# trungnt13/sisua

Hardware: AMD Instinct MI355X
Metric: cells/sec VAE training (pbmc8k_ly, batch=128) (higher is better)
Workload: dtype f32

## Files before the change

include/sisua_hip.h:

```cpp
#ifndef SISUA_HIP_H_
#define SISUA_HIP_H_

#include <stdint.h>

#ifdef __cplusplus
extern "C" {
#endif

#define SMX_ABI_VERSION 18
#define SMX_MAX_LAYERS 8
#define SMX_MAX_LABELS 4

typedef enum {
  SMX_OK = 0,
  SMX_ERR_INVALID = -1,
  SMX_ERR_HIP = -2,
  SMX_ERR_NOMEM = -3,
  SMX_ERR_COMM = -4,
  SMX_ERR_NAN = -5
} smx_status;

typedef enum { SMX_MODEL_VAE = 0, SMX_MODEL_DCA = 1, SMX_MODEL_SCVI = 2, SMX_MODEL_SISUA = 3, SMX_MODEL_SCALE = 4,
               SMX_MODEL_FVAE = 5,
               SMX_MODEL_SCALE_TRIL = 6 ,
// ... 116 lines not shown
                        float* l_samples, float* x_params, float* const* y_params);

int smx_predict(smx_model* m, const float* host_x, const float* host_library, int64_t n_cells, int32_t batch,
                int32_t n_samples, float* z_mean, float* z_scale, float* z_samples, float* l_mean, float* l_scale,
                float* l_samples, float* x_params, float* const* y_params);

int smx_predict_stat(smx_model* m, const float* host_x, const float* host_library, int64_t n_cells, int32_t batch, int32_t n_samples,
                     int32_t stat, int32_t count_only, const float* target, float* out);

int smx_predict_csr(smx_model* m, const int64_t* indptr, const int32_t* cols, const float* vals, const float* host_library,
                    int64_t n_cells, int32_t batch, int32_t n_samples, float* z_mean, float* z_scale, float* z_samples,
                    float* l_mean, float* l_scale, float* l_samples, float* x_params, float* const* y_params);
int smx_predict_stat_csr(smx_model* m, const int64_t* indptr, const int32_t* cols, const float* vals, const float* host_library,
                         int64_t n_cells, int32_t batch, int32_t n_samples, int32_t stat, int32_t count_only, const float* target,
                         const int64_t* t_indptr, const int32_t* t_cols, const float* t_vals, float* out);

int smx_predict_sample(smx_model* m, const float* host_x, const float* host_library, int64_t n_cells, int32_t batch, int32_t n_samples,
                       int32_t count_only, uint64_t seed, int32_t n_k, float* out);
int smx_predict_sample_csr(smx_model* m, const int64_t* indptr, const int32_t* cols, const float* vals, const float* host_library,
                           int64_t n_cells, int32_t batch, int32_t n_samples, int32_t count_only, uint64_t seed, int32_t n_k, float* out);

int smx_predict_stat_cols(smx_model* m, const float* host_x, const float* host_library, int64_t n_cells, int32_t batch, int32_t n_samples,
                          int32_t count_only, const int32_t* genes, int32_t n_sel, float* out);
int smx_predict_stat_cols_csr(smx_model* m, const int64_t* indptr, const int32_t* cols, const float* vals, const float* host_library,
                              int64_t n_cells, int32_t batch, int32_t n_samples, int32_t count_only, const int32_t* genes, int32_t n_sel,
                              float* out);

int smx_predict_impute(smx_model* m, const float* host_x, const float* host_library, int64_t n_cells, int32_t batch, int32_t n_samples,
                       int32_t count_only, const float* original, float* cell_median, int32_t* cell_changed, float* global_lohi);
int smx_predict_impute_csr(smx_model* m, const float* host_x, const int64_t* indptr, const int32_t* cols, const float* vals,
                           const float* host_library, int64_t n_cells, int32_t batch, int32_t n_samples, int32_t count_only,
                           const float* original, const int64_t* o_indptr, const int32_t* o_cols, const float* o_vals, float* cell_median,
                           int32_t* cell_changed, float* global_lohi);

int smx_predict_correlate(smx_model* m, const float* host_x, const float* host_library, int64_t n_cells, int32_t batch, int32_t n_samples,
                          int32_t count_only, const int32_t* genes, int32_t n_sel, const int32_t* prot_rank2, const double* prot_unit, int32_t P,
                          int64_t* sp_Sa, int64_t* sp_Saa, int64_t* sp_Sab, double* pe_mean, double* pe_Sxx, double* pe_Sxy, int32_t* nonfinite);
int smx_predict_correlate_csr(smx_model* m, const int64_t* indptr, const int32_t* cols, const float* vals, const float* host_library,
                              int64_t n_cells, int32_t batch, int32_t n_samples, int32_t count_only, const int32_t* genes, int32_t n_sel,
                              const int32_t* prot_rank2, const double* prot_unit, int32_t P, int64_t* sp_Sa, int64_t* sp_Saa, int64_t* sp_Sab,
                              double* pe_mean, double* pe_Sxx, double* pe_Sxy, int32_t* nonfinite);

int smx_decode(smx_model* m, const float* z, const float* l, int32_t batch, float* x_params, float* const* y_params);

int smx_marginal_llk(smx_model* m, const int32_t* row_ids, const float* host_x, const float* host_library, int32_t batch,
                     int32_t n_samples, float* mllk, float* llk_mean);
int smx_marginal_llk_csr(smx_model* m, const int64_t* indptr, const int32_t* cols, const float* vals, const float* host_library,
                         int32_t batch, int32_t n_samples, float* mllk, float* llk_mean);

int smx_score_llk(smx_model* m, const int32_t* row_ids, const float* host_x, const float* host_library,
                  const float* const* targets, int32_t n_targets, int32_t batch, int32_t n_samples, float* out);

int smx_set_noise(smx_model* m, int32_t stream, const float* data, int32_t batch, int32_t width);
int smx_clear_noise(smx_model* m);

int smx_comm_unique_id(uint8_t id[128]);
int smx_comm_init(smx_model* m, int rank, int world, const uint8_t id[128]);
int smx_comm_world(const smx_model* m);
int smx_comm_rank(const smx_model* m);
int smx_comm_form(const smx_model* m);
int smx_comm_set_form(smx_model* m, int form);
int smx_opt_gather(smx_model* m);
int smx_comm_p2p_export(smx_model* m, int world, uint8_t handles[128]);
int smx_comm_p2p_init(smx_model* m, int rank, int world, const uint8_t* all_handles);
int smx_comm_p2p_error(smx_model* m, int32_t* error);
int smx_comm_time_allreduce(smx_model* m, int iters, float* us_per_call, int64_t* floats);
int smx_comm_library(char* rccl_path, int rccl_cap, char* hip_path, int hip_cap, int32_t* rccl_version);
int smx_comm_set_sync_bn(smx_model* m, int on);
int smx_comm_init_local(smx_model* const* models, int n);

int smx_shuffle_order(int32_t n_obs, int32_t buffer, const int64_t* picks, int32_t* out);

int smx_set_tuning(const char* name, double value);
int smx_clear_tuning(const char* name);

int smx_set_flag(smx_model* m, const char* name, int value);

int smx_timing_enable(smx_model* m, const char* kernel);
int smx_timing_read(smx_model* m, double* total_ms, int64_t* launches);
int64_t smx_loss_bytes_per_cell(const smx_model* m);
int64_t smx_head_fused_bytes(const smx_model* m, int32_t batch);
int32_t smx_head_dw_late(const smx_model* m);
int32_t smx_lazy_adam_steps(const smx_model* m);

int smx_k_count_llk(int likelihood, int direct, const float* x, const float* planes, int32_t B, int32_t G,
                    float* llk, float* grads);
int smx_k_adam(int32_t n_tensors, const int32_t* sizes, float* params, const float* grads, float* m, float* v,
               int32_t step, float lr, float beta1, float beta2, float eps, float clipnorm, float* norms);
int smx_k_opt(int32_t rule, const float* hp, int32_t n_hp, int32_t n_tensors, const int32_t* sizes, float* params, const float* grads,
              float* m, float* v, int32_t step, float lr, float clipnorm, float* norms);
typedef enum { SMX_CARRIER_LAUNCH = 0, SMX_CARRIER_SWEEP = 1, SMX_CARRIER_SHARD = 2, SMX_CARRIER_BODY512 = 3 } smx_opt_carrier;
int smx_k_opt_carrier(const int32_t* ip, const float* fp, const float* hp, int32_t n_hp, const int32_t* sizes, const float* params,
                      const float* grads, const float* m, const float* v, const int32_t* sq_first, const int32_t* sq_count, const float* sq_slots,
                      float* params_out, float* m_out, float* v_out, float* norms, float* lr_t, int32_t* guards_ok, int32_t* unused_ok);
int smx_k_gemm(int transA, int transB, const float* A, const float* B, int32_t M, int32_t N, int32_t K,
               int32_t split_k, int32_t tile_cfg, float* C);
int smx_k_head_fused(int likelihood, int u16, const float* x, const float* d, const float* W, const float* bias, int32_t B, int32_t G,
                     float grad_scale, int32_t reps, float* llk, float* dW, float* db, float* dd, float* sumsq, float* us);
int smx_k_head_fused_stress(int likelihood, int u16, const float* x, const float* d, const float* W, const float* bias, int32_t B, int32_t G,
                            float grad_scale, int32_t launches, int32_t* n_differ, int64_t* first_word);
int smx_k_hiprand(uint64_t seed, int32_t n, const uint32_t* counters, uint32_t* ours, uint32_t* hiprand_words);
int smx_k_noise(uint64_t seed, int32_t stream, int32_t step, int32_t sample, const int64_t* cell_ids, int32_t B,
                int32_t width, float dropout_p, float* dropout_mult, float* normal);
int smx_k_bn_fwd(const int32_t* ip, const float* fp, const float* pre, const float* gamma, const float* beta, const float* bias,
                 const float* moving_mean, const float* moving_var, const float* mask, const int32_t* rows, uint64_t seed, float* out,
                 float* xhat, float* inv_std, float* batch_mean, float* batch_var, float* moving_mean_out, float* moving_var_out,
                 int32_t* guards_ok);
int smx_k_bn_bwd(const int32_t* ip, const float* fp, const float* dout, const float* out, const float* xhat, const float* inv_std,
                 const float* gamma, const float* beta, const float* mask, const int32_t* rows, uint64_t seed, float* dpre, float* dgamma,
                 float* dbeta, float* dbias, int32_t* guards_ok);
int smx_k_scvi_head_train(const int32_t* ip, const float* fp, const float* raw, const void* x, const float* hl, const float* Wl, const float* bl,
                          const float* library, const int32_t* rows, const float* eps_in, uint64_t seed, float* draw, float* llk_part, float* l,
                          float* sig, float* eps, float* kl, float* latl, float* dlatl, float* dl, int32_t* guards_ok);
int smx_k_scvi_head_fwd(const int32_t* ip, const float* fp, const float* raw, const float* l, float* planes, float* rho_raw, int32_t* guards_ok);
int smx_k_scvi_head_bwd(const int32_t* ip, const float* fp, const float* planes, const float* dplanes, const float* rho_raw, const float* l,
                        float* draw, float* dl, int32_t* guards_ok);
int smx_k_plane_sample(int likelihood, int direct, int count_only, const float* planes, int32_t rows, int32_t G, uint64_t seed,
                       int32_t n_k, float* out);
int smx_k_row_select(const float* rows, int32_t n_rows, int32_t G, int32_t ld, float* lo, float* hi);
int smx_k_col_rank2(const float* cols, int32_t n_cols, int64_t n_cells, int32_t* rank2, int32_t* nonfinite);
int smx_k_col_correlate(const float* cols, int32_t n_cols, int64_t n_cells, const int32_t* prot_rank2, const double* prot_unit, int32_t P,
                        int64_t* sp_Sa, int64_t* sp_Saa, int64_t* sp_Sab, double* pe_mean, double* pe_Sxx, double* pe_Sxy, int32_t* nonfinite);

int smx_cluster_silhouette(const float* Z, int64_t n_cells, int32_t D, const int32_t* labels, int32_t n_labels, double* a, double* b);
int smx_cluster_kmeans(const float* Z, int64_t n_cells, int32_t D, int32_t K, const int32_t* init_idx, int32_t n_init, int32_t max_iter,
                       int32_t* labels_best, double* centres_best, double* inertia, int32_t* n_iter, int32_t* best, int32_t* labels_all);

int smx_gmm1d_fit(const float* X, int64_t n_cells, int32_t C, int32_t K, const float* init_raw, int32_t R, int32_t max_iter, double tol,
                  double reg_covar, int32_t remove_zeros, int32_t log_norm, double* lower_bound, int32_t* n_iter, int32_t* converged,
                  int32_t* best, double* weights, double* means, double* variances, int64_t* n_train, double* col_sum, double* params_all,
                  double* stats);
int smx_gmm1d_predict(const float* X, int64_t n_cells, int32_t C, int32_t K, const double* weights, const double* means, const double* variances,
                      const int32_t* order, int32_t positive_component, const double* threshold, int32_t log_norm, double* prob, float* bin,
                      double* score);

int smx_gmm_full_fit(const float* Z, int64_t n_cells, int32_t D, int32_t K, const int32_t* init_labels, int32_t R, int32_t max_iter, double tol,
                     double reg_covar, double* lower_bound, int32_t* n_iter, int32_t* converged, int32_t* status, int32_t* best,
                     double* weights, double* means, double* covariances, double* chol_inv, int32_t* labels, double* params_all);
int smx_gmm_full_predict(const float* Z, int64_t n_cells, int32_t D, int32_t K, const double* weights, const double* means, const double* chol_inv,
                         int32_t* labels, double* resp, double* score);

int smx_prep_stats(const float* x, const int64_t* indptr, const int32_t* cols, const float* vals, int64_t n_cells, int32_t n_genes,
                   int32_t block_rows, int32_t func, const float* row_div, const uint8_t* col_mask, const float* row_thresh,
                   double* cell_total, int32_t* cell_n_genes, double* gene_sum, double* gene_sumsq, int64_t* gene_n_cells,
                   int64_t* gene_n_above);
int smx_prep_apply(const float* x, const int64_t* indptr, const int32_t* cols, const float* vals, int64_t n_cells, int32_t n_genes,
                   int32_t block_rows, int32_t func, const float* row_div, const float* mean, const float* sd, int32_t clip,
                   float max_value, float* out_dense, float* out_vals);

int smx_pca_cov(const float* x, const int64_t* indptr, const int32_t* cols, const float* vals, int64_t n_cells, int32_t n_genes,
                int32_t block_rows, double* mean, double* cov);
int smx_pca_project(const float* x, const int64_t* indptr, const int32_t* cols, const float* vals, int64_t n_cells, int32_t n_genes,
                    int32_t block_rows, const double* mean, const double* components, int32_t n_components, float* out);

int smx_knn(const float* Z, int64_t n_cells, int32_t D, int32_t k, int32_t* idx, double* dist);
int smx_knn_umap(const int32_t* idx, const double* dist, int64_t n_cells, int32_t K, double* rho, double* sigma, double* weight);

int smx_tsne_affinities(const int32_t* idx, const double* dist, int64_t n_cells, int32_t k, double perplexity, double* cond_p, double* beta);
int smx_tsne_gradient(const int64_t* indptr, const int32_t* cols, const double* p, int64_t n_cells, int32_t n_components, const double* Y,
                      double exaggeration, double* grad, double* kl, double* Z);
int smx_tsne_fit(const int64_t* indptr, const int32_t* cols, const double* p, int64_t n_cells, int32_t n_components, const double* Y0,
                 int32_t max_iter, double early_exaggeration, double learning_rate, double min_grad_norm, int32_t n_iter_without_progress,
                 double* Y, double* kl_trace, int32_t* n_iter, double* update_out, double* gains_out);

int smx_mutual_info(const double* xcols, const uint8_t* x_discrete, const double* ycols, const uint8_t* y_discrete, int64_t n_cells,
                    int32_t n_genes, int32_t n_proteins, int32_t n_neighbors, int32_t gene_chunk, const double* psi, const double* logn,
// ... 43 lines not shown
```

sisua_amd/_hip.py:

```python
from __future__ import annotations

import ctypes as C
import os

_HERE = os.path.dirname(os.path.abspath(__file__))
LIB_PATH = os.path.join(_HERE, "libsisua_hip.so")

SMX_ABI_VERSION = 18
SMX_MAX_LAYERS = 8
SMX_MAX_LABELS = 4

MODEL_KINDS = {"vae": 0, "dca": 1, "scvi": 2, "sisua": 3, "scale": 4, "fvae": 5, "scale_tril": 6, "scale_post": 7}
LIKELIHOODS = {"nb": 0, "zinb": 1, "nbd": 2, "zinbd": 3, "mse": 4, "bernoulli": 5, "normal": 6}
LABEL_LIKELIHOODS = {"nb": 0, "onehot": 1, "mixnb": 2, "mixgauss": 3, "mixtril": 4, "mixzinb": 5, "nbd": 6, "zinb": 7, "zinbd": 8,
                     "bernoulli": 9, "normal": 10}
SCVI_PLANE_OPTIONS = {"full": 0, "share": 1, "single": 2}
ACTIVATIONS = {"relu": 0, "linear": 1}
SMX_ACT_RELU, SMX_ACT_LINEAR, SMX_ACT_LEAKY_RELU, SMX_ACT_ELU, SMX_ACT_SELU, SMX_ACT_TANH, SMX_ACT_SIGMOID, SMX_ACT_SOFTPLUS = range(8)
HIDDEN_ACTIVATIONS = {"relu": SMX_ACT_RELU, "linear": SMX_ACT_LINEAR, "leaky_relu": SMX_ACT_LEAKY_RELU, "elu": SMX_ACT_ELU,
                      "selu": SMX_ACT_SELU, "tanh": SMX_ACT_TANH, "sigmoid": SMX_ACT_SIGMOID, "softplus": SMX_ACT_SOFTPLUS}
SMX_NET_ENCODER, SMX_NET_DECODER, SMX_NET_LIBRARY_ENCODER = range(3)


class SmxError(RuntimeError):
# ... 53 lines not shown
    "smx_set_bn": (C.c_int, [_VP, C.c_int, C.c_int, _FP]),
    "smx_get_step": (C.c_int, [_VP, _IP]),
    "smx_set_step": (C.c_int, [_VP, C.c_int32]),
    "smx_dataset_upload": (C.c_int, [_VP, _FP, C.c_int64, C.POINTER(_FP), _FP, C.POINTER(C.c_uint8), C.c_int64]),
    "smx_dataset_upload_u16": (C.c_int, [_VP, C.POINTER(C.c_uint16), C.c_int64, C.POINTER(_FP), _FP, C.POINTER(C.c_uint8), C.c_int64]),
    "smx_dataset_upload_csr": (C.c_int, [_VP, C.POINTER(C.c_int64), C.POINTER(C.c_int32), _FP, C.c_int64, C.POINTER(_FP), _FP,
                                         C.POINTER(C.c_uint8), C.c_int64]),
    "smx_dataset_upload_csr_dense": (C.c_int, [_VP, _LP, _IP, _FP, C.c_int64, C.POINTER(_FP), _FP, C.POINTER(C.c_uint8), C.c_int64,
                                               C.c_int32]),
    "smx_dataset_size": (C.c_int64, [_VP]),
    "smx_dataset_generate_lognormal": (C.c_int, [_VP, C.c_uint64, C.c_int32, C.c_int64, C.c_int32, C.c_double]),
    "smx_train_step": (C.c_int, [_VP, _IP, C.c_int32, C.POINTER(smx_metrics)]),
    "smx_train_step_graph": (C.c_int, [_VP, _IP, C.c_int32, C.POINTER(smx_metrics)]),
    "smx_train_steps": (C.c_int, [_VP, _IP, C.c_int32, C.c_int32, C.c_int, C.POINTER(smx_metrics)]),
    "smx_train_stage": (C.c_int, [_VP, _IP, C.c_int32, C.c_int32]),
    "smx_metrics_history": (C.c_int, [_VP, C.c_int32, _FP]),
    "smx_eval_step": (C.c_int, [_VP, _IP, C.c_int32, C.POINTER(smx_metrics)]),
    "smx_set_train_draws": (C.c_int, [_VP, C.c_int32]),
    "smx_set_optimizer": (C.c_int, [_VP, C.c_int32, _FP, C.c_int32]),
    "smx_set_schedule": (C.c_int, [_VP, C.c_int32, C.c_int32, C.POINTER(C.c_double), C.c_int32]),
    "smx_get_schedule": (C.c_int, [_VP, C.c_int32, _IP, C.POINTER(C.c_double), C.c_int32, _IP]),
    "smx_schedule_eval": (C.c_int, [C.c_int32, C.POINTER(C.c_double), C.c_int32, C.c_int64, C.c_int32, _FP]),
    "smx_get_optimizer": (C.c_int, [_VP, _IP, _FP, _IP]),
    "smx_set_activation": (C.c_int, [_VP, C.c_int32, C.c_int32]),
    "smx_forward": (C.c_int, [_VP, _IP, _FP, _FP, C.c_int32, C.c_int32, C.c_int32, _FP, _FP, _FP, _FP, _FP, _FP, _FP,
                              C.POINTER(_FP)]),
    "smx_forward_samples": (C.c_int, [_VP, _IP, _FP, _FP, C.c_int32, C.c_int32, _FP, _FP, _FP, _FP, _FP, _FP, _FP,
                                      C.POINTER(_FP)]),
    "smx_shuffle_order": (C.c_int, [C.c_int32, C.c_int32, C.POINTER(C.c_int64), C.POINTER(C.c_int32)]),
    "smx_predict": (C.c_int, [_VP, _FP, _FP, C.c_int64, C.c_int32, C.c_int32, _FP, _FP, _FP, _FP, _FP, _FP, _FP,
                              C.POINTER(_FP)]),
    "smx_predict_stat": (C.c_int, [_VP, _FP, _FP, C.c_int64, C.c_int32, C.c_int32, C.c_int32, C.c_int32, _FP, _FP]),
    "smx_predict_csr": (C.c_int, [_VP, _LP, _IP, _FP, _FP, C.c_int64, C.c_int32, C.c_int32, _FP, _FP, _FP, _FP, _FP, _FP, _FP,
                                  C.POINTER(_FP)]),
    "smx_predict_stat_csr": (C.c_int, [_VP, _LP, _IP, _FP, _FP, C.c_int64, C.c_int32, C.c_int32, C.c_int32, C.c_int32, _FP,
                                       _LP, _IP, _FP, _FP]),
    "smx_predict_sample": (C.c_int, [_VP, _FP, _FP, C.c_int64, C.c_int32, C.c_int32, C.c_int32, C.c_uint64, C.c_int32, _FP]),
    "smx_predict_sample_csr": (C.c_int, [_VP, _LP, _IP, _FP, _FP, C.c_int64, C.c_int32, C.c_int32, C.c_int32, C.c_uint64, C.c_int32, _FP]),
    "smx_predict_stat_cols": (C.c_int, [_VP, _FP, _FP, C.c_int64, C.c_int32, C.c_int32, C.c_int32, _IP, C.c_int32, _FP]),
    "smx_predict_stat_cols_csr": (C.c_int, [_VP, _LP, _IP, _FP, _FP, C.c_int64, C.c_int32, C.c_int32, C.c_int32, _IP, C.c_int32, _FP]),
    "smx_predict_impute": (C.c_int, [_VP, _FP, _FP, C.c_int64, C.c_int32, C.c_int32, C.c_int32, _FP, _FP, _IP, _FP]),
    "smx_predict_impute_csr": (C.c_int, [_VP, _FP, _LP, _IP, _FP, _FP, C.c_int64, C.c_int32, C.c_int32, C.c_int32, _FP, _LP, _IP, _FP,
                                         _FP, _IP, _FP]),
    "smx_predict_correlate": (C.c_int, [_VP, _FP, _FP, C.c_int64, C.c_int32, C.c_int32, C.c_int32, _IP, C.c_int32, _IP, _DP, C.c_int32,
                                        _LP, _LP, _LP, _DP, _DP, _DP, _IP]),
    "smx_predict_correlate_csr": (C.c_int, [_VP, _LP, _IP, _FP, _FP, C.c_int64, C.c_int32, C.c_int32, C.c_int32, _IP, C.c_int32, _IP, _DP,
                                            C.c_int32, _LP, _LP, _LP, _DP, _DP, _DP, _IP]),
    "smx_decode": (C.c_int, [_VP, _FP, _FP, C.c_int32, _FP, C.POINTER(_FP)]),
    "smx_dataset_library": (C.c_int, [_VP, _FP]),
    "smx_dataset_corrupt": (C.c_int, [_VP, C.c_double, C.c_double, C.c_uint64, C.POINTER(C.c_int64)]),
    "smx_dataset_read": (C.c_int, [_VP, C.c_int64, C.c_int64, _FP, _FP, _FP]),
    "smx_marginal_llk": (C.c_int, [_VP, _IP, _FP, _FP, C.c_int32, C.c_int32, _FP, _FP]),
    "smx_marginal_llk_csr": (C.c_int, [_VP, _LP, _IP, _FP, _FP, C.c_int32, C.c_int32, _FP, _FP]),
    "smx_score_llk": (C.c_int, [_VP, _IP, _FP, _FP, C.POINTER(_FP), C.c_int32, C.c_int32, C.c_int32, _FP]),
    "smx_set_noise": (C.c_int, [_VP, C.c_int32, _FP, C.c_int32, C.c_int32]),
    "smx_clear_noise": (C.c_int, [_VP]),
    "smx_comm_unique_id": (C.c_int, [C.POINTER(C.c_uint8)]),
    "smx_comm_init": (C.c_int, [_VP, C.c_int, C.c_int, C.POINTER(C.c_uint8)]),
    "smx_comm_p2p_export": (C.c_int, [_VP, C.c_int, C.POINTER(C.c_uint8)]),
    "smx_comm_p2p_init": (C.c_int, [_VP, C.c_int, C.c_int, C.POINTER(C.c_uint8)]),
    "smx_comm_p2p_error": (C.c_int, [_VP, C.POINTER(C.c_int32)]),
    "smx_comm_time_allreduce": (C.c_int, [_VP, C.c_int, C.POINTER(C.c_float), C.POINTER(C.c_int64)]),
    "smx_comm_world": (C.c_int, [_VP]),
    "smx_comm_rank": (C.c_int, [_VP]),
    "smx_comm_form": (C.c_int, [_VP]),
    "smx_comm_set_form": (C.c_int, [_VP, C.c_int]),
    "smx_opt_gather": (C.c_int, [_VP]),
    "smx_comm_library": (C.c_int, [C.c_char_p, C.c_int, C.c_char_p, C.c_int, _IP]),
    "smx_comm_set_sync_bn": (C.c_int, [_VP, C.c_int]),
    "smx_comm_init_local": (C.c_int, [C.POINTER(_VP), C.c_int]),
    "smx_k_adam": (C.c_int, [C.c_int32, _IP, _FP, _FP, _FP, _FP, C.c_int32, C.c_float, C.c_float, C.c_float, C.c_float,
                             C.c_float, _FP]),
    "smx_k_opt": (C.c_int, [C.c_int32, _FP, C.c_int32, C.c_int32, _IP, _FP, _FP, _FP, _FP, C.c_int32, C.c_float, C.c_float, _FP]),
    "smx_k_opt_carrier": (C.c_int, [_IP, _FP, _FP, C.c_int32, _IP, _FP, _FP, _FP, _FP, _IP, _IP, _FP, _FP, _FP, _FP, _FP, _FP, _IP, _IP]),
    "smx_set_flag": (C.c_int, [_VP, C.c_char_p, C.c_int]),
    "smx_set_tuning": (C.c_int, [C.c_char_p, C.c_double]),
    "smx_clear_tuning": (C.c_int, [C.c_char_p]),
    "smx_timing_enable": (C.c_int, [_VP, C.c_char_p]),
    "smx_timing_read": (C.c_int, [_VP, C.POINTER(C.c_double), C.POINTER(C.c_int64)]),
    "smx_loss_bytes_per_cell": (C.c_int64, [_VP]),
    "smx_head_fused_bytes": (C.c_int64, [_VP, C.c_int32]),
    "smx_head_dw_late": (C.c_int32, [_VP]),
    "smx_lazy_adam_steps": (C.c_int32, [_VP]),
    "smx_k_count_llk": (C.c_int, [C.c_int, C.c_int, _FP, _FP, C.c_int32, C.c_int32, _FP, _FP]),
    "smx_k_head_fused": (C.c_int, [C.c_int, C.c_int, _FP, _FP, _FP, _FP, C.c_int32, C.c_int32, C.c_float, C.c_int32, _FP, _FP, _FP, _FP, _FP,
                                   _FP]),
    "smx_k_head_fused_stress": (C.c_int, [C.c_int, C.c_int, _FP, _FP, _FP, _FP, C.c_int32, C.c_int32, C.c_float, C.c_int32, C.POINTER(C.c_int32),
                                          C.POINTER(C.c_int64)]),
    "smx_k_gemm": (C.c_int, [C.c_int, C.c_int, _FP, _FP, C.c_int32, C.c_int32, C.c_int32, C.c_int32, C.c_int32, _FP]),
    "smx_k_hiprand": (C.c_int, [C.c_uint64, C.c_int32, C.POINTER(C.c_uint32), C.POINTER(C.c_uint32), C.POINTER(C.c_uint32)]),
    "smx_k_noise": (C.c_int, [C.c_uint64, C.c_int32, C.c_int32, C.c_int32, C.POINTER(C.c_int64), C.c_int32, C.c_int32,
                              C.c_float, _FP, _FP]),
    "smx_k_bn_fwd": (C.c_int, [_IP, _FP, _FP, _FP, _FP, _FP, _FP, _FP, _FP, _IP, C.c_uint64, _FP, _FP, _FP, _FP, _FP, _FP, _FP, _IP]),
    "smx_k_bn_bwd": (C.c_int, [_IP, _FP, _FP, _FP, _FP, _FP, _FP, _FP, _FP, _IP, C.c_uint64, _FP, _FP, _FP, _FP, _IP]),
    "smx_k_scvi_head_train": (C.c_int, [_IP, _FP, _FP, _VP, _FP, _FP, _FP, _FP, _IP, _FP, C.c_uint64, _FP, _FP, _FP, _FP, _FP, _FP, _FP, _FP, _FP, _IP]),
    "smx_k_scvi_head_fwd": (C.c_int, [_IP, _FP, _FP, _FP, _FP, _FP, _IP]),
    "smx_k_scvi_head_bwd": (C.c_int, [_IP, _FP, _FP, _FP, _FP, _FP, _FP, _FP, _IP]),
    "smx_k_plane_sample": (C.c_int, [C.c_int, C.c_int, C.c_int, _FP, C.c_int32, C.c_int32, C.c_uint64, C.c_int32, _FP]),
    "smx_k_row_select": (C.c_int, [_FP, C.c_int32, C.c_int32, C.c_int32, _FP, _FP]),
    "smx_k_col_rank2": (C.c_int, [_FP, C.c_int32, C.c_int64, _IP, _IP]),
    "smx_k_col_correlate": (C.c_int, [_FP, C.c_int32, C.c_int64, _IP, _DP, C.c_int32, _LP, _LP, _LP, _DP, _DP, _DP, _IP]),
    "smx_cluster_silhouette": (C.c_int, [_FP, C.c_int64, C.c_int32, _IP, C.c_int32, _DP, _DP]),
    "smx_cluster_kmeans": (C.c_int, [_FP, C.c_int64, C.c_int32, C.c_int32, _IP, C.c_int32, C.c_int32, _IP, _DP, _DP, _IP, _IP, _IP]),
    "smx_gmm1d_fit": (C.c_int, [_FP, C.c_int64, C.c_int32, C.c_int32, _FP, C.c_int32, C.c_int32, C.c_double, C.c_double, C.c_int32, C.c_int32, _DP, _IP,
                            _IP, _IP, _DP, _DP, _DP, _LP, _DP, _DP, _DP]),
    "smx_gmm1d_predict": (C.c_int, [_FP, C.c_int64, C.c_int32, C.c_int32, _DP, _DP, _DP, _IP, C.c_int32, _DP, C.c_int32, _DP, _FP, _DP]),
    "smx_gmm_full_fit": (C.c_int, [_FP, C.c_int64, C.c_int32, C.c_int32, _IP, C.c_int32, C.c_int32, C.c_double, C.c_double, _DP, _IP, _IP, _IP, _IP,
                               _DP, _DP, _DP, _DP, _IP, _DP]),
    "smx_gmm_full_predict": (C.c_int, [_FP, C.c_int64, C.c_int32, C.c_int32, _DP, _DP, _DP, _IP, _DP, _DP]),
    "smx_prep_stats": (C.c_int, [_FP, _LP, _IP, _FP, C.c_int64, C.c_int32, C.c_int32, C.c_int32, _FP, C.POINTER(C.c_uint8), _FP, _DP, _IP, _DP, _DP,
                                 _LP, _LP]),
    "smx_prep_apply": (C.c_int, [_FP, _LP, _IP, _FP, C.c_int64, C.c_int32, C.c_int32, C.c_int32, _FP, _FP, _FP, C.c_int32, C.c_float, _FP, _FP]),
    "smx_pca_cov": (C.c_int, [_FP, _LP, _IP, _FP, C.c_int64, C.c_int32, C.c_int32, _DP, _DP]),
    "smx_pca_project": (C.c_int, [_FP, _LP, _IP, _FP, C.c_int64, C.c_int32, C.c_int32, _DP, _DP, C.c_int32, _FP]),
    "smx_knn": (C.c_int, [_FP, C.c_int64, C.c_int32, C.c_int32, _IP, _DP]),
    "smx_knn_umap": (C.c_int, [_IP, _DP, C.c_int64, C.c_int32, _DP, _DP, _DP]),
    "smx_tsne_affinities": (C.c_int, [_IP, _DP, C.c_int64, C.c_int32, C.c_double, _DP, _DP]),
    "smx_tsne_gradient": (C.c_int, [_LP, _IP, _DP, C.c_int64, C.c_int32, _DP, C.c_double, _DP, _DP, _DP]),
    "smx_tsne_fit": (C.c_int, [_LP, _IP, _DP, C.c_int64, C.c_int32, _DP, C.c_int32, C.c_double, C.c_double, C.c_double, C.c_int32, _DP, _DP, _IP,
                               _DP, _DP]),
    "smx_mutual_info": (C.c_int, [_DP, C.POINTER(C.c_uint8), _DP, C.POINTER(C.c_uint8), C.c_int64, C.c_int32, C.c_int32, C.c_int32, C.c_int32, _DP,
                                  _DP, _DP]),
    "smx_k_mi_cells": (C.c_int, [_DP, C.c_int32, _DP, C.c_int32, C.c_int64, C.c_int32, _DP, _DP, _IP, _DP, _DP]),
    "smx_group_moments": (C.c_int, [_FP, _LP, _IP, _FP, C.c_int64, C.c_int32, C.c_int32, _IP, C.c_int32, _LP, _DP, _DP, _LP]),
    "smx_group_ranksums": (C.c_int, [_FP, C.c_int32, C.c_int64, _IP, C.c_int32, C.c_int32, _LP, _LP]),
    "smx_mbkmeans_seed": (C.c_int, [_FP, _LP, _IP, _FP, C.c_int64, C.c_int32, C.c_int32, C.c_int32, C.c_int64, _DP, _IP, _DP, _DP]),
    "smx_mbkmeans_step": (C.c_int, [_FP, _LP, _IP, _FP, C.c_int64, C.c_int32, C.c_int32, _DP, _DP, _IP, _DP]),
    "smx_mbkmeans_predict": (C.c_int, [_FP, _LP, _IP, _FP, C.c_int64, C.c_int32, C.c_int32, C.c_int32, _DP, _IP, _DP]),
    "smx_louvain": (C.c_int, [_LP, _IP, _DP, C.c_int64, C.c_double, C.c_double, C.c_int32, C.c_int32, _IP, _IP, _IP, _DP, _LP, _IP, _IP]),
    "smx_louvain_modularity": (C.c_int, [_LP, _IP, _DP, C.c_int64, _IP, C.c_double, _DP]),
    "smx_louvain_table_degree": (C.c_int32, []),
    "smx_logreg_eval": (C.c_int, [_FP, _LP, _IP, _FP, C.c_int64, C.c_int32, _IP, C.c_int32, C.c_int32, C.c_double, C.c_int32, _DP, _DP, _DP, _DP,
                                  _DP]),
    "smx_logreg_fit": (C.c_int, [_FP, _LP, _IP, _FP, C.c_int64, C.c_int32, _IP, C.c_int32, C.c_int32, C.c_double, C.c_int32, C.c_double, C.c_int32,
                                 _DP, _DP, _DP, _DP, _DP, _DP, _IP, _IP, _IP]),
    "smx_logreg_decision": (C.c_int, [_FP, _LP, _IP, _FP, C.c_int64, C.c_int32, C.c_int32, C.c_int32, C.c_int32, _DP, _DP, _DP]),
    "smx_pad_audit": (C.c_int, [_VP, C.c_int32, _LP, _IP, _LP, C.c_char_p, C.c_int32]),
    "smx_pad_poke": (C.c_int, [_VP, C.c_int32, C.c_int32, C.c_float]),
}

_lib = None


def load():
  global _lib
  if _lib is not None:
    return _lib
  if not os.path.exists(LIB_PATH):
    raise SmxError(f"{LIB_PATH} is missing: build it with `python -m sisua_amd.build` "
                   "(hipcc --offload-arch=gfx950). sisua_amd has no CPU fallback.")
  try:
    lib = C.CDLL(LIB_PATH, mode=C.RTLD_GLOBAL)
  except OSError as e:
    raise SmxError(f"cannot load {LIB_PATH}: {e}") from e
  for name, (res, args) in SIGNATURES.items():
    try:
      fn = getattr(lib, name)
    except AttributeError as e:
      raise SmxError(f"{LIB_PATH} does not export {name}") from e
    fn.restype = res
    fn.argtypes = args
  if lib.smx_abi_version() != SMX_ABI_VERSION:
    raise SmxError("libsisua_hip.so ABI version mismatch; rebuild")
  if int(os.environ.get("WORLD_SIZE", "1")) > 1:
    for cand in ("/opt/rocm/lib/librccl.so.1", "/opt/rocm/lib/librccl.so"):
      if os.path.exists(cand):
# ... 33 lines not shown
```

sisua_amd/build.py:

```python
import os
import subprocess
import sys
from concurrent.futures import ThreadPoolExecutor

HERE = os.path.dirname(os.path.abspath(__file__))
CSRC = os.path.join(HERE, "csrc")
LIB = os.path.join(HERE, "libsisua_hip.so")
SOURCES = ["smx_gemm.hip", "smx_dgemm.hip", "smx_bn.hip", "smx_latent.hip", "smx_adam.hip", "smx_loss.hip", "smx_data.hip", "smx_headloss.hip", "smx_headbwd.hip", "smx_headfused.hip", "smx_bigk.hip", "smx_factor.hip", "smx_scvi.hip", "smx_score.hip", "smx_model.hip", "smx_dataset.hip", "smx_comm.hip", "smx_p2p.hip", "smx_forward.hip", "smx_backward.hip", "smx_step.hip", "smx_predict.hip", "smx_sample.hip", "smx_impute.hip", "smx_correlate.hip", "smx_cluster.hip", "smx_gmm.hip", "smx_gmm_full.hip", "smx_prep.hip", "smx_pca.hip", "smx_knn.hip", "smx_tsne.hip", "smx_mi.hip", "smx_rankgroups.hip", "smx_mbkmeans.hip", "smx_louvain.hip", "smx_logreg.hip", "smx_scoring.hip", "smx_schedule.hip", "smx_kapi.hip"]
HEADERS = ["smx_device.h", "smx_act.h", "smx_internal.h", "smx_loss.h", "smx_model.h", "smx_panel.h", "smx_dgemm.h", "smx_adam.h", "smx_headdw.h", "smx_dist.h", "smx_block.h", "smx_prep.h", os.path.join("..", "..", "include", "sisua_hip.h")]
FLAGS = ["--offload-arch=gfx950", "-O3", "-std=c++17", "-fPIC", "-fno-slp-vectorize", "-Wall", "-Wno-unused-function", "-Wno-unused-value", "-Wno-unused-result"]


def _hipcc():
  for c in (os.environ.get("HIPCC"), "/opt/rocm/bin/hipcc", "hipcc"):
    if c and (os.path.isabs(c) and os.path.exists(c) or not os.path.isabs(c)):
      return c
  raise RuntimeError("hipcc not found")


def _stale(target, deps):
  if not os.path.exists(target):
    return True
  t = os.path.getmtime(target)
  return any(os.path.getmtime(d) > t for d in deps)


def build(force: bool = False, verbose: bool = True) -> str:
  hipcc = _hipcc()
  hdrs = [os.path.normpath(os.path.join(CSRC, h)) for h in HEADERS]
  stamp, flags = os.path.join(CSRC, ".flags"), " ".join(FLAGS)
  if not os.path.exists(stamp) or open(stamp).read() != flags:
    force = True
  objs, jobs = [], []
  for s in SOURCES:
    src = os.path.join(CSRC, s)
    obj = os.path.join(CSRC, s.replace(".hip", ".o"))
    objs.append(obj)
    if force or _stale(obj, [src] + hdrs):
      jobs.append([hipcc] + FLAGS + ["-c", src, "-o", obj])

  def run(cmd):
    if verbose:
      print(" ".join(cmd), flush=True)
    r = subprocess.run(cmd, capture_output=True, text=True)
    if r.returncode != 0:
      raise RuntimeError("build failed:\n" + " ".join(cmd) + "\n" + r.stdout + r.stderr)
    return r.stderr

  with ThreadPoolExecutor(max_workers=7) as ex:
    for err in ex.map(run, jobs):
      if verbose and err.strip():
        print(err)
  with open(stamp, "w") as f:
    f.write(flags)
  if force or jobs or _stale(LIB, objs):
    isa_lint(objs)
    run([hipcc, "--offload-arch=gfx950", "-shared", "-fPIC", "-o", LIB] + objs + ["-ldl"])
  return LIB


def isa_lint(objs):
  tools = os.path.join(os.path.dirname(HERE), "tools")
  if not os.path.exists(os.path.join(tools, "isa_lint.py")) or os.environ.get("SMX_NO_ISA_LINT"):
    return
  sys.path.insert(0, tools)
  try:
    import isa_lint as lint
  finally:
    sys.path.pop(0)
  found = lint.lint_files(objs)
  if found:
    raise RuntimeError("isa_lint: the build contains instruction forms that are wrong on gfx950 (tools/isa_lint.py):\n" +
                       "\n".join("  %s %s: %s" % f for f in found[:20]))


if __name__ == "__main__":
  print(build(force="--force" in sys.argv))
```

sisua_amd/csrc/smx_backward.hip:

```cpp
#include "smx_model.h"

namespace smx {

static void fill_rider_adam(smx_model* m, AdamArgs& a) {
  fill_adam_args(m, a);
  a.use_sq = 1;
  for (size_t t = 0; t < m->tensors.size(); ++t) {
    a.sq_first[t] = m->sq_first[t]; a.sq_count[t] = m->sq_count[t];
    if (m->sq_reduced[t]) { a.sq_first[t] = m->sq_total_first + (int)t * SMX_SQR_PER_TENSOR; a.sq_count[t] = m->sq_reduced[t]; }
  }
  a.master = nullptr; a.with_metrics = 0;
}

static void take_adam_riders(smx_model* m, GemmArgs& h, AdamArgs& store) {
  const int n = std::min(m->adam_ride_b, m->adam_rest_to - m->adam_rest_from);
  m->adam_ride_b = 0;
  if (n <= 0) return;
  fill_rider_adam(m, store);
  h.ride_adam = &store; h.ride_first = m->adam_rest_from; h.ride_count = n;
  if (m->adam_early_from < 0) m->adam_early_from = m->adam_rest_from;
  m->adam_rest_from += n;
  m->adam_early_to = m->adam_rest_from;
}

// ... 77 lines not shown
    if (m->sq_count[t] == 0 && m->tensors[t].count > SMX_SQ_SMALL_TENSOR) return false;
  return true;
}
int head_sweep_prepare(smx_model* m) {
  const int mode = (dp_active(m) || tuning_on("event_system_fence")) ? 1 : 0;
  if (m->st_side && m->ev_mode == mode) return SMX_OK;
  if (!m->st_side) {
    int lo = 0, hi = 0;
    SMX_HIP(hipDeviceGetStreamPriorityRange(&lo, &hi));
    SMX_HIP(hipStreamCreateWithPriority(&m->st_side, hipStreamNonBlocking, lo));
  }
  if (m->ev_sweep) { hipEventDestroy(m->ev_sweep); m->ev_sweep = nullptr; }
  if (m->ev_hf) { hipEventDestroy(m->ev_hf); m->ev_hf = nullptr; }
  const unsigned fl = hipEventDisableTiming | (mode ? 0u : (unsigned)hipEventDisableSystemFence);
  SMX_HIP(hipEventCreateWithFlags(&m->ev_sweep, fl));
  SMX_HIP(hipEventCreateWithFlags(&m->ev_hf, fl));
  m->ev_mode = mode;
  return SMX_OK;
}
static int head_sweep_start(smx_model* m) {
  AdamArgs a;
  fill_rider_adam(m, a);
  static const bool skip = tuning_on("skip_head_adam");
  if (!skip) {
    SMX_HIP(hipStreamWaitEvent(m->st_side, m->ev_hf, 0));
    SMX_CHECK(launch_adam_sweep(m->st_side, a, m->chunk_first_head, head_sweep_end(m) - m->chunk_first_head, head_sweep_wgs(m)));
    SMX_HIP(hipEventRecord(m->ev_sweep, m->st_side));
    m->sweep_pending = true;
  }
  m->adam_early_from = m->chunk_first_head; m->adam_early_to = head_sweep_end(m);
  m->adam_early_pending = false; m->adam_rest_from = m->adam_rest_to = 0; m->adam_ride_b = 0;
  return SMX_OK;
}

int dp_chain_start(smx_model* m) {
  if (m->chain_started) return SMX_OK;
  SMX_CHECK(head_sweep_prepare(m));
  SMX_HIP(hipEventRecord(m->ev_hf, m->st));
  SMX_HIP(hipStreamWaitEvent(m->st_comm, m->ev_hf, 0));
  AdamArgs a;
  fill_adam_args(m, a);
  a.use_sq = 0; a.master = nullptr; a.with_metrics = 0;
  const int first = m->chunk_first_head, count = m->n_chunks - m->chunk_first_head;
  const int forced = (int)tuning("adam_sweep_wgs", 0);
  const int wgs = forced > 0 ? forced : std::min(std::max(count / SMX_HEAD_SWEEP_CHUNKS_PER_WG, 64), 256);
  if (m->flags.opt_shard && (m->world > 1 || m->dp_force) && dp_shard_available(m)) {
    const size_t slice = (((size_t)m->bucket1_count + m->world - 1) / m->world + 63) / 64 * 64;
    SMX_REQUIRE((size_t)m->world * slice <= (size_t)m->bucket1_count + SMX_SHARD_SLACK, "opt_shard: too many ranks for the buffers' slack");
    SMX_CHECK(dp_reduce_scatter(m, m->grads + m->bucket1_off, slice, m->st_comm, true));
    a.partial = m->shard_partial;
    a.shard_lo = (long)(m->bucket1_off + (size_t)m->rank * slice);
    a.shard_hi = (long)std::min(m->bucket1_off + ((size_t)m->rank + 1) * slice, m->bucket1_off + (size_t)m->bucket1_count);
    SMX_CHECK(launch_grad_sqsum_shard(m->st_comm, a, first, count));
    SMX_CHECK(dp_allreduce_buf(m, m->shard_partial + first, (size_t)count, m->st_comm, true));
    SMX_CHECK(launch_head_norms(m->st_comm, a, first, count));
    if (a.shard_hi > a.shard_lo) SMX_CHECK(launch_adam_shard(m->st_comm, a, first, count, wgs));
    SMX_CHECK(dp_all_gather(m, m->params + m->bucket1_off, slice, m->st_comm, true));
    m->opt_stale = true;
  } else {
    SMX_CHECK(dp_allreduce(m, m->bucket1_off, m->bucket1_count, m->st_comm, true));
    SMX_CHECK(launch_grad_sqsum_range(m->st_comm, a, first, count));
    SMX_CHECK(launch_adam_sweep(m->st_comm, a, first, count, wgs));
  }
  SMX_HIP(hipEventRecord(m->ev_sweep, m->st_comm));
  m->sweep_pending = true;
  m->chain_started = true;
  m->adam_early_from = m->chunk_first_head; m->adam_early_to = m->n_chunks;
  m->adam_rest_from = m->adam_rest_to = 0; m->adam_ride_b = 0;
  return SMX_OK;
}

struct MlpBwdOpts {
  bool skip_input_grad = false;
  int* out_slabs = nullptr;
  const char* label = "";
  const EpiLatentBwd* lat_epi = nullptr;
  GemmArgs* defer_dw0 = nullptr;
  const BnBwdArgs* front = nullptr;
  std::vector<GemmArgs>* defer = nullptr;
  std::vector<MlpLayer>* twin = nullptr; const BnBwdArgs* twin_front = nullptr; bool* twin_done = nullptr;
  bool last_bn_done = false;
  const HeadBwdArgs* head_dw = nullptr;
};
static int mlp_backward(smx_model* m, std::vector<MlpLayer>& mlp, const Pass& ps, Mat in0, bool in_is_x, int n_slabs, const MlpBwdOpts& o) {
  auto make_b = [&](MlpLayer& L, int slabs, const BnBwdArgs* front) {
    BnBwdArgs b;
    b.dout = m->slab; b.n_slabs = slabs; b.slab_stride = (long)ps.B * L.out_p; b.ld = L.out_p;
    b.out = L.out_buf; b.xhat = L.xhat; b.inv_std = L.inv_std;
    b.B = ps.B; b.H = L.out; b.Hp = L.out_p; b.batchnorm = L.bn >= 0; b.training = ps.training; b.leak = L.leak;
    b.drop_scale = (ps.training && L.drop_p > 0.f) ? 1.f / (1.f - L.drop_p) : 1.f;
    b.dpre = L.dpre;
    if (L.bn >= 0) { b.gamma = P_(m, L.tGamma); b.dgamma = G_(m, L.tGamma); b.dbeta = G_(m, L.tBeta); }
    else b.dbias = G_(m, L.tBias);
    if (L.act != SMX_ACT_RELU) {
      b.act = L.act;
      if (L.bn >= 0) b.beta = P_(m, L.tBeta);
      b.drop_p = ps.training ? L.drop_p : 0.f;
      b.nk = make_key(m, L.stream, ps.sample, true);
      if (&mlp == &m->dec) b.nk.draw_rows = (uint32_t)ps.draw_rows;
      b.rows = ps.rows; b.cell_base = ps.cell_base;
      if (const Injected* ij = inj(m, L.stream)) { b.inj_mask = ij->d; b.inj_ld = ij->ld; }
    }
    if (front) {
      b.front = 1; b.fD = front->fD; b.fld = front->fld; b.fW = front->fW; b.fldw = front->fldw; b.fK = front->fK;
      b.fold_dz = front->fold_dz; b.zD = front->zD; b.zld = front->zld; b.zW = front->zW; b.zldw = front->zldw; b.zlb = front->zlb;
    }
    if (&mlp == &m->dec && &L == &mlp.back() && m->wide_dd_slabs > 0 && !front) {
      b.dout = m->wide_dd_src; b.n_slabs = m->wide_dd_slabs; b.slab_stride = m->wide_dd_stride; b.wide = 1;
    }
    return b;
  };
  if (o.twin_done) *o.twin_done = false;
  BnBwdArgs carried;
  bool have_carried = false;
  bool dw_carried = false;
  bool dpre_done = false;
  for (int i = (int)mlp.size() - 1; i >= 0; --i) {
    MlpLayer& L = mlp[i];
    const TensorInfo& tw = m->tensors[L.tW];
    const bool last = (i == (int)mlp.size() - 1);
    BnBwdArgs b = make_b(L, n_slabs, (o.front && last) ? o.front : (have_carried ? &carried : nullptr));
    have_carried = false;
    const bool dpre_ready = dpre_done;
    dpre_done = false;
    if ((last && o.last_bn_done) || dpre_ready) {
    } else if (sync_bn_on(m, ps.training) && L.bn >= 0) {
      Timed t(m, "bn_bwd");
      m->adam_early_pending = false;
      const BnSyncArgs y = sync_args(m);
      SMX_CHECK(launch_bn_sync_bwd(m->st, b, y, 0));
      SMX_CHECK(dp_allreduce_buf(m, m->sync_buf, (size_t)y.world * 2 * L.out_p, m->st));
      SMX_CHECK(launch_bn_sync_bwd(m->st, b, y, 1));
    } else {
      if (m->metrics_before_allreduce && m->have_pending_metrics) {
        b.metrics = m->pending_metrics; b.with_metrics = 1; m->have_pending_metrics = false;
      }
      const HeadBwdArgs* hd = (last && o.head_dw && bn_wide_bwd_dw_supported(b, *o.head_dw)) ? o.head_dw : nullptr;
      if (!hd) attach_early_adam(m, b);
      const bool w_rides = hd && b.adam_count == 0 && b.sqr_count == 0 && m->lazy_w_pending && !m->lazy_rest_pending;
      if (w_rides) { b.adam = m->lazy_args; b.adam_first = m->lazy_w_first; b.adam_count = m->lazy_w_n; }
      if (m->lazy_want && m->lazy_l1 && !m->lazy_closed && &mlp == &m->enc && m->have_pending_metrics) {
        b.metrics = m->pending_metrics; b.with_metrics = 1; m->have_pending_metrics = false;
        if (!b.adam.params) fill_adam_args(m, b.adam);
        fill_step_close(m, b.adam);
        b.close = 1; m->lazy_closed = true;
      }
      Timed t(m, "bn_bwd");
      const bool dual = last && b.front && b.fK <= 64 && o.twin && o.twin_front && o.twin_front->fK <= 64 && !o.twin->empty() && m->flags.twin && bn_dual_supported(ps.B) &&
                        bn_bwd_front_supported(ps.B, o.twin_front->fK) && o.twin->back().out_p % 8 == 0 &&
                        !(sync_bn_on(m, ps.training) && o.twin->back().bn >= 0);
      if (hd) {
        SMX_CHECK(launch_bn_wide_bwd_dw(m->st, b, *hd));
        dw_carried = true;
        if (w_rides) m->lazy_w_pending = false;
      } else if (dual) {
        const BnBwdArgs b2 = make_b(o.twin->back(), 0, o.twin_front);
        SMX_CHECK(launch_bn_act_bwd_dual(m->st, b, b2));
        if (o.twin_done) *o.twin_done = true;
      } else {
        SMX_CHECK(launch_bn_act_bwd(m->st, b));
      }
    }
    const bool first_x = (i == 0 && in_is_x);
    const Mat in = (i == 0) ? in0 : Mat{mlp[i - 1].out_buf, mlp[i - 1].out_p};
    GemmArgs g = dense_wgrad(m, in, {L.dpre, L.out_p}, L.tW, dpre_ready ? G_(m, L.tBias) : nullptr, L.in_p, L.out_p, ps.B);
    if (first_x) x_gather(m, ps, g);
    if (i == 0 && o.skip_input_grad) {
      if (o.defer_dw0) *o.defer_dw0 = g;
      else {
        Timed t(m, first_x ? o.label : "gemm_mlp_dw");
        SMX_CHECK(launch_gemm(m->st, g));
      }
      n_slabs = 0;
      break;
    }
    if (o.defer && i > 0 && !(i == 0 && o.lat_epi) && m->flags.bwd_front && (L.out_p == 32 || L.out_p == 64 || L.out_p == 128) && mlp[i - 1].act == SMX_ACT_RELU &&
        bn_bwd_front_supported(ps.B, L.out_p) && mlp[i - 1].out_p % 8 == 0 && (tw.ld % 4) == 0 && (L.out_p % 4) == 0 &&
        !(sync_bn_on(m, ps.training) && mlp[i - 1].bn >= 0)) {
      o.defer->push_back(g);
      carried = BnBwdArgs();
      carried.fD = L.dpre; carried.fld = L.out_p; carried.fW = P_(m, L.tW); carried.fldw = tw.ld; carried.fK = L.out_p;
      have_carried = true;
      n_slabs = 0;
      continue;
    }
    GemmArgs h = dense_dgrad({L.dpre, L.out_p}, {P_(m, L.tW), tw.ld}, m->slab, ps.B, L.in_p, L.out_p);
    h.split_k = suggest_split_k(ps.B, L.in_p, L.out_p);
    SMX_REQUIRE((size_t)h.split_k * (size_t)h.slab_stride <= m->slab_cap, "split-K slabs exceed the slab buffer");
    if (i == 0 && o.lat_epi) {
      h.epi = 2; h.lb = *o.lat_epi; h.split_k = 1; h.tile = TILE_32x32_K4;
    }
    if (i > 0 && m->flags.act_epilogue && mlp[i - 1].bn < 0 && !(ps.training && mlp[i - 1].drop_p > 0.f) && h.split_k <= 1 &&
        mlp[i - 1].act == SMX_ACT_RELU) {
      MlpLayer& Lo = mlp[i - 1];
      h.split_k = 1; h.act = 2; h.leak = Lo.leak; h.act_out = Lo.out_buf; h.act_ld = Lo.out_p;
      h.C = Lo.dpre; h.ldc = Lo.out_p; h.slab_stride = 0;
      dpre_done = true;
    }
    int effs[2] = {1, 1};
    if (o.defer && i == 0 && o.lat_epi && m->fold_dz_now) {
      o.defer->push_back(g);
    } else if (o.defer && i == 0 && o.lat_epi) {
      o.defer->push_back(g);
      AdamArgs riders;
      if (m->adam_ride_b > 0) take_adam_riders(m, h, riders);
      Timed t(m, "gemm_mlp_bwd");
      SMX_CHECK(launch_gemm_group(m->st, &h, 1, effs + 1));
    } else {
      GemmArgs pair[2] = {g, h};
      Timed t(m, "gemm_mlp_bwd");
      SMX_CHECK(launch_gemm_group(m->st, pair, 2, effs));
    }
    const int eff = effs[1];
    n_slabs = eff;
  }
  if (o.out_slabs) *o.out_slabs = n_slabs;
  SMX_REQUIRE(!o.head_dw || dw_carried, "the output head's dW found no launch to carry it");
  return SMX_OK;
}

static int disc_wgrad(smx_model* m, const GemmArgs& g, int rows, bool b3, const GemmArgs* beside = nullptr) {
  if (!(b3 && m->flags.wgrad && wgrad_supported(g, rows))) return launch_gemm(m->st, g);
  if (g.M >= 512 && g.N % 128 == 0 && g.N / 128 <= SMX_GROUP_MAX && g.N > 128 && !tuning_on("no_panel")) {
    GemmArgs part[SMX_GROUP_MAX];
    int counts[SMX_GROUP_MAX];
    const int ng = g.N / 128, per = ((g.M + 31) / 32) * 8;
    for (int k = 0; k < ng; ++k) {
      part[k] = g;
      part[k].B = g.B + 128 * k; part[k].C = g.C + 128 * k; part[k].N = 128; part[k].panel_hint = 1;
      if (g.colsum) part[k].colsum = g.colsum + 128 * k;
      if (g.sq_part) { part[k].sq_part = g.sq_part + (long)per * k; part[k].sq_count = &counts[k]; }
    }
    const int rc = launch_wgrad_group(m->st, part, ng, rows, 1, beside);
    if (rc == SMX_OK && g.sq_part && g.sq_count) *g.sq_count = per * ng;
    return rc;
  }
  return launch_wgrad_group(m->st, &g, 1, rows, 1, beside);
// ... 457 lines not shown
```

sisua_amd/csrc/smx_bn.hip:

```cpp
#include "smx_internal.h"
#include "smx_adam.h"

namespace smx {

SMX_STAMP_TABLE

}
#include "smx_headdw.h"
namespace smx {

#ifndef SMX_BN_COLS
#define SMX_BN_COLS 8
#endif
constexpr int BN_COLS = SMX_BN_COLS;
constexpr int BN_RL = 64;
constexpr int BN_RPT_DEFAULT = 2;
constexpr int BN_THREADS = BN_COLS * BN_RL;
constexpr int BN_WAVES = BN_THREADS / 64;

__device__ inline float bn_col_reduce(float v, float* sh ) {
  const int c = threadIdx.x % BN_COLS, w = threadIdx.x >> 6;
  static_assert(BN_COLS == 8, "bn_col_reduce: the lanes of a column are 8 apart");
  v += __int_as_float(__builtin_amdgcn_update_dpp(0, __float_as_int(v), 0x128, 0xF, 0xF, false));
  v = xor32_add(xor16_add(v));
  __syncthreads();
  if ((threadIdx.x & 63) < BN_COLS) sh[w * BN_COLS + c] = v;
  __syncthreads();
  float t = 0.f;
#pragma unroll
  for (int q = 0; q < BN_WAVES; q += 4)
    t += (sh[q * BN_COLS + c] + sh[(q + 1) * BN_COLS + c]) + (sh[(q + 2) * BN_COLS + c] + sh[(q + 3) * BN_COLS + c]);
  return t;
}

constexpr int SLAB_FLIGHT = 16;
template <int NR>
struct SlabBatch { float t[SLAB_FLIGHT][NR]; };
template <int NR>
__device__ inline void slab_issue(const float* base, int s0, int n_slabs, long slab_stride, int ld, int col, int r0, int rl, int B, SlabBatch<NR>& sb) {
#pragma unroll
  for (int q = 0; q < SLAB_FLIGHT; ++q) {
    const int s = min(s0 + q, n_slabs - 1);
#pragma unroll
    for (int i = 0; i < NR; ++i) {
      const int r = min(r0 + rl + BN_RL * i, B - 1);
      sb.t[q][i] = base[(long)s * slab_stride + (long)r * ld + col];
    }
  }
}
template <int NR>
__device__ inline void slab_accumulate(const SlabBatch<NR>& sb, int s0, int n_slabs, int r0, int rl, int B, float (&acc)[NR]) {
#pragma unroll
  for (int q = 0; q < SLAB_FLIGHT; ++q)
    if (s0 + q < n_slabs) {
#pragma unroll
      for (int i = 0; i < NR; ++i) acc[i] += (r0 + rl + BN_RL * i < B) ? sb.t[q][i] : 0.f;
    }
}
template <int BN_RPT>
__device__ inline void slab_sum(const float* base, int n_slabs, long slab_stride, int ld, int col, int r0, int rl,
                                int B, float (&acc)[BN_RPT]) {
#pragma unroll
  for (int i = 0; i < BN_RPT; ++i) acc[i] = 0.f;
  if (BN_RPT <= 2) {
    for (int s = 0; s < n_slabs; s += SLAB_FLIGHT) {
      SlabBatch<BN_RPT> sb;
      slab_issue<BN_RPT>(base, s, n_slabs, slab_stride, ld, col, r0, rl, B, sb);
      slab_accumulate<BN_RPT>(sb, s, n_slabs, r0, rl, B, acc);
    }
    return;
  }
  constexpr int SU = BN_RPT <= 4 ? 4 : 2;
  int s = 0;
  for (; s + SU <= n_slabs; s += SU) {
    float t[SU][BN_RPT];
#pragma unroll
    for (int q = 0; q < SU; ++q)
#pragma unroll
      for (int i = 0; i < BN_RPT; ++i) {
        const int r = r0 + rl + BN_RL * i;
        t[q][i] = r < B ? base[(long)(s + q) * slab_stride + (long)r * ld + col] : 0.f;
      }
#pragma unroll
    for (int q = 0; q < SU; ++q)
// ... 327 lines not shown

int launch_bn_act_fwd(hipStream_t st, const BnFwdArgs& a_in) {
  BnFwdArgs a = a_in;
  const bool gen = a.act != SMX_ACT_RELU;
  if (gen && (a.act < SMX_ACT_RELU || a.act > SMX_ACT_SOFTPLUS || a.front)) { set_error("bn_act_fwd: activations other than ReLU take no front"); return SMX_ERR_INVALID; }
  if (a.front) {
    if (!bn_front_supported(a.B, a.lat.Dp) || a.n_jobs || !a.W || (a.lat.ld % 4) || (a.lat.inj_eps && (a.lat.inj_ld % 4)) ||
        (a.lat.Dp > 32 && a.lat.Dp != 64 && a.lat.Dp != 128)) {
      set_error("bn_act_fwd: latent front not applicable");
      return SMX_ERR_INVALID;
    }
    if (a.Hp % BN_COLS) { set_error("bn_act_fwd: bad shapes"); return SMX_ERR_INVALID; }
    const size_t lds = ((size_t)a.B * (a.lat.Dp + 4) + (size_t)BN_COLS * (a.lat.Dp + 4)) * sizeof(float);
    static const bool big_ok = hipFuncSetAttribute(reinterpret_cast<const void*>(&bn_act_fwd_kernel<4, 1>),
                                                   hipFuncAttributeMaxDynamicSharedMemorySize, 96 * 1024) == hipSuccess;
    if (lds > 64 * 1024 && !big_ok) { set_error("bn_act_fwd: cannot reserve the dynamic LDS of the latent front"); return SMX_ERR_HIP; }
    if (a.lat.Dp == 128) {
      static const bool big2 = hipFuncSetAttribute(reinterpret_cast<const void*>(&bn_act_fwd_kernel<2, 2>),
                                                   hipFuncAttributeMaxDynamicSharedMemorySize, 96 * 1024) == hipSuccess;
      if (a.B > BN_RL * 2 || a.lat.stochastic || a.lat.relu || a.lat.z || (lds > 64 * 1024 && !big2)) {
        set_error("bn_act_fwd: 128-wide front not applicable");
        return SMX_ERR_INVALID;
      }
      hipLaunchKernelGGL((bn_act_fwd_kernel<2, 2>), dim3(a.Hp / BN_COLS), dim3(BN_THREADS), lds, st, a);
    } else if (a.B <= BN_RL * 2) hipLaunchKernelGGL((bn_act_fwd_kernel<2, 1>), dim3(a.Hp / BN_COLS + (a.lat.z ? 1 : 0)), dim3(BN_THREADS), lds, st, a);
    else hipLaunchKernelGGL((bn_act_fwd_kernel<4, 1>), dim3(a.Hp / BN_COLS + (a.lat.z ? 1 : 0)), dim3(BN_THREADS), lds, st, a);
    SMX_HIP(hipGetLastError());
    return SMX_OK;
  }
  if (a.Hp % BN_COLS || a.B <= 0) { set_error("bn_act_fwd: bad shapes"); return SMX_ERR_INVALID; }
  if (a.wide) {
    if (a.B > 128 || a.Hp > 128 || !a.pre || !a.xhat || a.slab_stride < (long)a.Hp * 128 || (a.slab_stride % 4)) { set_error("bn_act_fwd: wide slabs take at most 128 x 128"); return SMX_ERR_INVALID; }
    if (gen) hipLaunchKernelGGL(bn_wide_fwd_gen_kernel, dim3(a.Hp + a.n_jobs * SMX_NOISE_BLOCKS_PER_JOB), dim3(BN_THREADS), 0, st, a);
    else hipLaunchKernelGGL(bn_wide_fwd_kernel, dim3(a.Hp + a.n_jobs * SMX_NOISE_BLOCKS_PER_JOB), dim3(BN_THREADS), 0, st, a);
    SMX_HIP(hipGetLastError());
    return SMX_OK;
  }
  const int grid = a.Hp / BN_COLS + a.n_jobs * SMX_NOISE_BLOCKS_PER_JOB;
  if (gen) {
    if (a.B <= BN_RL * 2) hipLaunchKernelGGL(bn_act_fwd_gen_kernel<2>, dim3(grid), dim3(BN_THREADS), 0, st, a);
    else if (a.B <= BN_RL * 4) hipLaunchKernelGGL(bn_act_fwd_gen_kernel<4>, dim3(grid), dim3(BN_THREADS), 0, st, a);
    else if (a.B <= BN_RL * 8) hipLaunchKernelGGL(bn_act_fwd_gen_kernel<8>, dim3(grid), dim3(BN_THREADS), 0, st, a);
    else if (a.B <= BN_RL * 16) hipLaunchKernelGGL(bn_act_fwd_gen_kernel<16>, dim3(grid), dim3(BN_THREADS), 0, st, a);
    else hipLaunchKernelGGL(bn_act_fwd_gen_kernel<0>, dim3(grid), dim3(BN_THREADS), 0, st, a);
    SMX_HIP(hipGetLastError());
    return SMX_OK;
  }
  if (a.B <= BN_RL * 2) hipLaunchKernelGGL(bn_act_fwd_kernel<2>, dim3(grid), dim3(BN_THREADS), 0, st, a);
  else if (a.B <= BN_RL * 4) hipLaunchKernelGGL(bn_act_fwd_kernel<4>, dim3(grid), dim3(BN_THREADS), 0, st, a);
  else if (a.B <= BN_RL * 8) hipLaunchKernelGGL(bn_act_fwd_kernel<8>, dim3(grid), dim3(BN_THREADS), 0, st, a);
  else if (a.B <= BN_RL * 16) hipLaunchKernelGGL(bn_act_fwd_kernel<16>, dim3(grid), dim3(BN_THREADS), 0, st, a);
  else hipLaunchKernelGGL(bn_act_fwd_kernel<0>, dim3(grid), dim3(BN_THREADS), 0, st, a);
  SMX_HIP(hipGetLastError());
  return SMX_OK;
}

bool bn_dual_supported(int B) { return B > 0 && B <= BN_RL * 4; }
int launch_bn_act_fwd_dual(hipStream_t st, const BnFwdArgs& a, const BnFwdArgs& b) {
  if (a.front || b.front || b.n_jobs || a.B != b.B || !bn_dual_supported(a.B) || a.Hp % BN_COLS || b.Hp % BN_COLS || a.act != SMX_ACT_RELU ||
      b.act != SMX_ACT_RELU) {
    set_error("bn_act_fwd_dual: bad shapes (or an activation other than ReLU)");
    return SMX_ERR_INVALID;
  }
  const int na = a.Hp / BN_COLS + a.n_jobs * SMX_NOISE_BLOCKS_PER_JOB;
  const int grid = na + b.Hp / BN_COLS;
  if (a.B <= BN_RL * 2) hipLaunchKernelGGL(bn_act_fwd_dual_kernel<2>, dim3(grid), dim3(BN_THREADS), 0, st, a, b, na);
  else hipLaunchKernelGGL(bn_act_fwd_dual_kernel<4>, dim3(grid), dim3(BN_THREADS), 0, st, a, b, na);
  SMX_HIP(hipGetLastError());
  return SMX_OK;
}

typedef float bnf_f32x4 __attribute__((ext_vector_type(4)));
__device__ inline bnf_f32x4 bnf_mfma16x3(const Split8& a, const Split8& b, bnf_f32x4 acc) {
  acc = __builtin_amdgcn_mfma_f32_16x16x32_bf16(a.t2, b.t0, acc, 0, 0, 0);
  acc = __builtin_amdgcn_mfma_f32_16x16x32_bf16(a.t0, b.t2, acc, 0, 0, 0);
  acc = __builtin_amdgcn_mfma_f32_16x16x32_bf16(a.t1, b.t1, acc, 0, 0, 0);
  acc = __builtin_amdgcn_mfma_f32_16x16x32_bf16(a.t1, b.t0, acc, 0, 0, 0);
  acc = __builtin_amdgcn_mfma_f32_16x16x32_bf16(a.t0, b.t1, acc, 0, 0, 0);
  acc = __builtin_amdgcn_mfma_f32_16x16x32_bf16(a.t0, b.t0, acc, 0, 0, 0);
  return acc;
}
#define SMX_FOLD_WROW 136
#define SMX_FOLD_WIMG_BYTES (3 * 32 * SMX_FOLD_WROW * 2)
__device__ inline void fold_dz_tile(const BnBwdArgs& a, const int bid, float* tile, const int ldd, unsigned char* wimg) {
  const EpiLatentBwd& e = a.zlb;
  const int tid = threadIdx.x, lane = tid & 63, w = tid >> 6, li = lane & 15, kg = lane >> 4;
  float e_mu[2][4], e_sr[2][4], e_sg[2][4], e_ep[2][4];
  const float kls = kl_scale_of(e.klw);
#pragma unroll
  for (int nb = 0; nb < 2; ++nb)
#pragma unroll
    for (int r = 0; r < 4; ++r) {
      const long b = min(16 * w + 4 * kg + r, a.B - 1);
      const int d = 16 * nb + li;
      e_mu[nb][r] = e.lat[b * e.ld + d];
      e_sr[nb][r] = e.lat[b * e.ld + e.Dp + d];
      e_sg[nb][r] = e.sig[b * e.Dp + d];
      e_ep[nb][r] = e.eps[b * e.Dp + d];
    }
  {
    const int d = tid >> 4, k0 = (tid & 15) * 8;
    const float4 lo = *reinterpret_cast<const float4*>(a.zW + (long)d * a.zldw + k0), hi = *reinterpret_cast<const float4*>(a.zW + (long)d * a.zldw + k0 + 4);
    const float x[8] = {lo.x, lo.y, lo.z, lo.w, hi.x, hi.y, hi.z, hi.w};
    const Split8 sp = split3x8(x);
    smx_bf16x8* row = reinterpret_cast<smx_bf16x8*>(wimg + ((long)d * SMX_FOLD_WROW + k0) * 2);
    row[0] = sp.t0;
    row[(32 * SMX_FOLD_WROW * 2) / 16] = sp.t1;
    row[(2 * 32 * SMX_FOLD_WROW * 2) / 16] = sp.t2;
  }
  Split8 A[4];
  {
    const float* zr = a.zD + (long)min(16 * w + li, a.B - 1) * a.zld + 8 * kg;
    float4 v[8];
#pragma unroll
    for (int ks = 0; ks < 4; ++ks) { v[2 * ks] = *reinterpret_cast<const float4*>(zr + 32 * ks); v[2 * ks + 1] = *reinterpret_cast<const float4*>(zr + 32 * ks + 4); }
#pragma unroll
    for (int ks = 0; ks < 4; ++ks) {
      const float x[8] = {v[2 * ks].x, v[2 * ks].y, v[2 * ks].z, v[2 * ks].w, v[2 * ks + 1].x, v[2 * ks + 1].y, v[2 * ks + 1].z, v[2 * ks + 1].w};
      A[ks] = split3x8(x);
    }
  }
  __syncthreads();
  bnf_f32x4 acc[2] = {{0.f, 0.f, 0.f, 0.f}, {0.f, 0.f, 0.f, 0.f}};
#pragma unroll
  for (int ks = 0; ks < 4; ++ks)
#pragma unroll
    for (int nb = 0; nb < 2; ++nb) {
      const smx_bf16x8* row = reinterpret_cast<const smx_bf16x8*>(wimg + ((long)(16 * nb + li) * SMX_FOLD_WROW + 32 * ks + 8 * kg) * 2);
      Split8 Bq;
      Bq.t0 = row[0]; Bq.t1 = row[(32 * SMX_FOLD_WROW * 2) / 16]; Bq.t2 = row[(2 * 32 * SMX_FOLD_WROW * 2) / 16];
      acc[nb] = bnf_mfma16x3(A[ks], Bq, acc[nb]);
    }
#pragma unroll
  for (int nb = 0; nb < 2; ++nb)
#pragma unroll
    for (int r = 0; r < 4; ++r) {
      const int b = 16 * w + 4 * kg + r, d = 16 * nb + li;
      const bool live = d < e.D;
      const float dz = acc[nb][r];
      const float o0 = live ? dz + kls * e_mu[nb][r] : 0.f;
      const float o1 = live ? (dz * e_ep[nb][r] + kls * (e_sg[nb][r] - frcp(e_sg[nb][r]))) * sigmoidf(e_sr[nb][r] + SMX_SOFTPLUS_INV_1) : 0.f;
      if (b < a.B) {
        tile[b * ldd + d] = o0;
        tile[b * ldd + e.Dp + d] = o1;
        if (bid == 0) { e.dlat[(long)b * e.ld + d] = o0; e.dlat[(long)b * e.ld + e.Dp + d] = o1; }
      }
    }
}

__device__ inline float bn_keep(const BnBwdArgs& a, int r, int col) {
  if (!(a.drop_p > 0.f)) return a.drop_scale;
  if (a.inj_mask) return a.inj_mask[(long)r * a.inj_ld + col];
  const uint32_t cell = a.cell_base + (uint32_t)(a.rows ? a.rows[r] : r);
  return dropout_mult1(philox_row(a.nk, (uint32_t)r, cell, (uint32_t)(col >> 2)), col & 3, a.drop_p, a.drop_scale);
}
__device__ inline float bn_gen_dy(const BnBwdArgs& a, int r, int col, float dout, float xv, float gamma, float beta) {
  const float y = a.batchnorm ? __builtin_fmaf(gamma, xv, beta) : xv;
  return dout * bn_keep(a, r, col) * act_grad(a.act, act_fwd(a.act, y));
}

template <int RPT, int FRONT, bool GEN_ACT = false>
__device__ inline void bn_act_bwd_body(const BnBwdArgs& a, const int bid) {
  constexpr bool SMALL = RPT > 0;
  constexpr int BN_RPT = SMALL ? RPT : BN_RPT_DEFAULT;
  extern __shared__ __attribute__((aligned(16))) float ds[];
  {
    const int nb = a.Hp / BN_COLS, extra = bid - nb;
    if (extra >= 0) {
      const int e = extra - (a.with_metrics ? 1 : 0);
      if (e >= 0 && e < a.adam_count) { adam_chunk_body<BN_THREADS>(a.adam, a.adam_first + e); return; }
      if (threadIdx.x >= 256) return;
      if (e < 0) metrics_body(a.metrics);
      else {
        const int i = e - a.adam_count;
        if (i < a.sqr_count) sq_reduce_body(a.adam.sq_slots + a.sqr_first[i], a.sqr_n[i], a.sq_total + a.sqr_dst[i]);
        else step_close_body<false>(a.adam);
      }
      return;
    }
  }
  __shared__ float sh[BN_WAVES * BN_COLS];
  SMX_STAMP(FRONT ? 3 : 2, 0);
  if (FRONT) preload(a.fD, a.fld, a.fW, a.fldw, a.fK, a.diag, a.out, a.xhat, a.inv_std, a.gamma, a.B, a.H, a.Hp, a.batchnorm, a.training, a.drop_scale);
  else preload(a.dout, a.n_slabs, a.slab_stride, a.ld, a.out, a.xhat, a.inv_std, a.gamma, a.B, a.H, a.Hp, a.batchnorm, a.training, a.drop_scale, a.dpre, a.leak);
  const int c = threadIdx.x % BN_COLS, rl = threadIdx.x / BN_COLS;
  const int col = bid * BN_COLS + c;
  const bool live = col < a.H;
  constexpr int CH = BN_RL * BN_RPT;
  float dyreg[BN_RPT], xhreg[BN_RPT];
  float s1 = 0.f, s2 = 0.f;
  float outpre[BN_RPT], xhpre[BN_RPT];
  float gamma_pre = 0.f, inv_pre = 0.f;
  if (SMALL) {
#pragma unroll
    for (int i = 0; i < BN_RPT; ++i) {
      const long o = (long)min(rl + BN_RL * i, a.B - 1) * a.Hp + col;
      if constexpr (!GEN_ACT) outpre[i] = a.out[o];
      xhpre[i] = (GEN_ACT || a.batchnorm) ? a.xhat[o] : 0.f;
    }
    if (a.batchnorm) { gamma_pre = live ? a.gamma[col] : 0.f; inv_pre = a.inv_std[col]; }
  }
  float gamma_g = 0.f, beta_g = 0.f;
  if constexpr (GEN_ACT) {
    if (a.batchnorm && live) { gamma_g = a.gamma[col]; beta_g = a.beta[col]; }
  }
  constexpr int FK = FRONT == 2 ? 128 : 64;
  float wrow[FRONT ? FK : 1];
  if (FRONT) {
    const int ldd = a.fK + 4, kq = a.fK >> 2;
    const int ksh = __builtin_ctz((unsigned)kq), kmask = kq - 1;
    float* ws = ds + a.B * ldd;
    const int ldw_s = a.fK + 4;
    float4 wl = make_float4(0.f, 0.f, 0.f, 0.f);
    const bool wl_on = (int)threadIdx.x < BN_COLS * kq && !(a.diag & 64);
    if (wl_on) wl = *reinterpret_cast<const float4*>(a.fW + (long)(bid * BN_COLS + ((int)threadIdx.x >> ksh)) * a.fldw + ((int)threadIdx.x & kmask) * 4);
    if (FRONT == 1 && a.fold_dz) {
      fold_dz_tile(a, bid, ds, ldd, reinterpret_cast<unsigned char*>(ws + BN_COLS * ldw_s));
      if ((int)threadIdx.x < BN_COLS * kq) *reinterpret_cast<float4*>(&ws[((int)threadIdx.x >> ksh) * ldw_s + ((int)threadIdx.x & kmask) * 4]) = wl;
    } else
    {
      constexpr int MAXIT = BN_RPT * (FK / 32);
      float4 tl[MAXIT];
#pragma unroll
      for (int it = 0; it < MAXIT; ++it) {
        const int idx = threadIdx.x + it * BN_THREADS;
        tl[it] = (idx < a.B * kq && !(a.diag & 32)) ? *reinterpret_cast<const float4*>(a.fD + (long)(idx >> ksh) * a.fld + (idx & kmask) * 4)
                                  : make_float4(0.f, 0.f, 0.f, 0.f);
      }
#pragma unroll
      for (int it = 0; it < MAXIT; ++it) {
        const int idx = threadIdx.x + it * BN_THREADS;
        if (idx < a.B * kq) {
          *reinterpret_cast<float4*>(ds + (idx >> ksh) * ldd + (idx & kmask) * 4) = tl[it];
        }
      }
      if ((int)threadIdx.x < BN_COLS * kq) *reinterpret_cast<float4*>(&ws[((int)threadIdx.x >> ksh) * ldw_s + ((int)threadIdx.x & kmask) * 4]) = wl;
    }
    __syncthreads();
    SMX_STAMP(3, 1);
#pragma unroll
    for (int v = 0; v < FK / 4; ++v) {
      const float4 t = (4 * v < a.fK) ? *reinterpret_cast<const float4*>(&ws[c * ldw_s + 4 * v]) : make_float4(0.f, 0.f, 0.f, 0.f);
      wrow[4 * v] = t.x; wrow[4 * v + 1] = t.y; wrow[4 * v + 2] = t.z; wrow[4 * v + 3] = t.w;
    }
    SMX_STAMP(3, 2);
  }
  for (int r0 = 0; r0 < a.B; r0 += CH) {
    float acc[BN_RPT];
    if (FRONT) {
      const int ldd = a.fK + 4;
#pragma unroll
      for (int i = 0; i < BN_RPT; ++i) {
        const int r = min(r0 + rl + BN_RL * i, a.B - 1);
        const float4* d4 = reinterpret_cast<const float4*>(ds + r * ldd);
        float t = 0.f;
        auto dots = [&](auto nv) {
#pragma unroll
          for (int v = 0; v < decltype(nv)::value; ++v) {
            const float4 d = d4[v];
            t = fmaf(d.x, wrow[4 * v], t); t = fmaf(d.y, wrow[4 * v + 1], t); t = fmaf(d.z, wrow[4 * v + 2], t); t = fmaf(d.w, wrow[4 * v + 3], t);
          }
        };
        if (a.diag & 16) t = ds[r * ldd] + wrow[0] + wrow[63];
        else if (FRONT == 2) dots(std::integral_constant<int, FK / 4>());
        else if (a.fK <= 32) dots(std::integral_constant<int, 8>());
        else dots(std::integral_constant<int, 16>());
        acc[i] = t;
      }
    } else
    slab_sum(a.dout, a.n_slabs, a.slab_stride, a.ld, col, r0, rl, a.B, acc);
#pragma unroll
    for (int i = 0; i < BN_RPT; ++i) {
      const int r = r0 + rl + BN_RL * i;
      float dy = 0.f, xh = 0.f;
      if (r < a.B) {
        const long o = (long)r * a.Hp + col;
        if constexpr (GEN_ACT) {
          const float xv = SMALL ? xhpre[i] : a.xhat[o];
          dy = live ? bn_gen_dy(a, r, col, acc[i], xv, gamma_g, beta_g) : 0.f;
          if (a.batchnorm) xh = xv;
        } else {
        const float ov = SMALL ? outpre[i] : a.out[o];
        dy = (live && ov > 0.f) ? acc[i] * a.drop_scale : 0.f;
        if (a.leak != 0.f && live && !(ov > 0.f)) dy = acc[i] * a.leak;
        if (a.batchnorm) xh = SMALL ? xhpre[i] : a.xhat[o];
        }
        if (!SMALL) a.dpre[o] = dy;
        s1 += dy;
        {
#pragma clang fp contract(off)
          s2 += dy * xh;
        }
      }
      if (SMALL) { dyreg[i] = dy; xhreg[i] = xh; }
    }
  }
  SMX_STAMP(FRONT ? 3 : 2, 3);
  s1 = bn_col_reduce(s1, sh);
  SMX_STAMP(FRONT ? 3 : 2, 4);
// ... 166 lines not shown
          a.batch_mean, a.batch_var, a.moving_mean, a.moving_var, a.inv_std, a.update_moving, a.rows, a.leak);
  const int col = bid, r = (int)threadIdx.x;
  const bool live = col < a.H, rowt = r < 128, on = rowt && r < a.B;
  const float bias = (!a.batchnorm && a.bias && live) ? a.bias[col] : 0.f;
  const float gamma = (a.batchnorm && live) ? a.gamma[col] : 0.f, beta = (a.batchnorm && live) ? a.beta[col] : 0.f;
  const bool drop = a.training && a.drop_p > 0.f;
  float mpre = 0.f;
  if (drop && a.inj_mask && on) mpre = a.inj_mask[(long)r * a.inj_ld + col];
  float mm_pre = 0.f, mv_pre = 0.f;
  if (a.batchnorm && a.training && a.update_moving && live && r == 0) { mm_pre = a.moving_mean[col]; mv_pre = a.moving_var[col]; }
  SMX_STAMP(0, 0);
  wide_slab_column(a.pre, a.slab_stride, a.n_slabs, col, sh);
  SMX_STAMP(0, 3);
  __syncthreads();
  float v = 0.f;
  if (rowt) { v = wide_row_value(sh, r) + bias; vs[r] = v; }
  float mean = 0.f, inv = 1.f;
  if (a.batchnorm) {
    float var;
    if (a.training) {
      __syncthreads();
      if (r < 64) {
        const float v0 = vs[r], v1 = vs[r + 64];
        float s1 = 0.f;
        if (r < a.B) s1 += v0;
        if (r + 64 < a.B) s1 += v1;
        s1 = wide_tree64(s1);
        const float mu = s1 / (float)a.B;
        float s2 = 0.f;
        if (r < a.B) { const float d = v0 - mu; s2 = d * d; }
        if (r + 64 < a.B) { const float d = v1 - mu; s2 = __builtin_fmaf(d, d, s2); }
        s2 = wide_tree64(s2);
        if (r == 0) { st[0] = mu; st[1] = s2 / (float)a.B; }
      }
      __syncthreads();
      mean = st[0];
      var = st[1];
      if (r == 0) {
        if (a.batch_mean) { a.batch_mean[col] = mean; a.batch_var[col] = var; }
        if (a.update_moving && live) {
          a.moving_mean[col] = mm_pre * a.momentum + mean * (1.f - a.momentum);
          a.moving_var[col] = mv_pre * a.momentum + var * (1.f - a.momentum);
        }
      }
    } else {
      mean = live ? a.moving_mean[col] : 0.f;
      var = live ? a.moving_var[col] : 1.f;
    }
    inv = rsqrtf(var + a.eps);
    if (r == 0 && a.inv_std) a.inv_std[col] = inv;
  }
  SMX_STAMP(0, 5);
  if (!on) return;
  const float scale = drop ? 1.f / (1.f - a.drop_p) : 1.f;
  const long o = (long)r * a.Hp + col;
  float y = v;
  if (a.batchnorm) {
    v = (v - mean) * inv;
    y = __builtin_fmaf(gamma, v, beta);
  }
  a.xhat[o] = v;
  float h;
  if constexpr (GEN_ACT) h = act_fwd(a.act, y);
  else {
    h = fmaxf(y, 0.f);
    if (a.leak != 0.f) h += a.leak * fminf(y, 0.f);
  }
  if (drop) {
    float mult = mpre;
    if (!a.inj_mask) {
      const uint32_t cell = a.cell_base + (uint32_t)(a.rows ? a.rows[r] : r);
      const U4 w = philox_row(a.nk, (uint32_t)r, cell, (uint32_t)(col >> 2));
      mult = dropout_mult1(w, col & 3, a.drop_p, scale);
    }
    h *= mult;
  }
  a.out[o] = live ? h : 0.f;
  SMX_STAMP(0, 6);
}
__global__ __launch_bounds__(BN_THREADS) void bn_wide_fwd_kernel(BnFwdArgs a) { bn_wide_fwd_body<false>(a); }
__global__ __launch_bounds__(BN_THREADS) void bn_wide_fwd_gen_kernel(BnFwdArgs a) { bn_wide_fwd_body<true>(a); }

constexpr int BN_WIDE_BWD_SMEM_FLOATS = 16 * 128 + 128 + 128 + 4;
template <bool GEN_ACT>
__device__ inline void bn_wide_bwd_body(const BnBwdArgs& a, float* lds) {
#pragma clang fp contract(off)
  const int bid = (int)blockIdx.x;
  {
    const int extra = bid - a.Hp;
    if (extra >= 0) {
      const int e = extra - (a.with_metrics ? 1 : 0);
      if (e >= 0 && e < a.adam_count) { adam_chunk_body<BN_THREADS>(a.adam, a.adam_first + e); return; }
      if (threadIdx.x >= 256) return;
      if (e < 0) metrics_body(a.metrics);
      else {
        const int i = e - a.adam_count;
        if (i < a.sqr_count) sq_reduce_body(a.adam.sq_slots + a.sqr_first[i], a.sqr_n[i], a.sq_total + a.sqr_dst[i]);
        else step_close_body<false>(a.adam);
      }
      return;
    }
  }
  float* const sh = lds;
  float* const vs = lds + 16 * 128; float* const xs = vs + 128; float* const st = xs + 128;
  preload(a.dout, a.n_slabs, a.slab_stride, a.out, a.xhat, a.inv_std, a.gamma, a.B, a.H, a.Hp, a.batchnorm, a.training, a.drop_scale, a.dpre, a.dgamma, a.dbeta);
  const int col = bid, r = (int)threadIdx.x;
  const bool live = col < a.H, rowt = r < 128, on = rowt && r < a.B;
  float ov = 0.f, xh = 0.f, gamma = 0.f, inv = 0.f;
  float xv = 0.f, beta = 0.f;
  if (on) {
    const long o = (long)r * a.Hp + col;
    if constexpr (GEN_ACT) {
      xv = a.xhat[o];
      if (a.batchnorm) xh = xv;
    } else {
      ov = a.out[o];
      if (a.batchnorm) xh = a.xhat[o];
    }
  }
  if (a.batchnorm) { gamma = live ? a.gamma[col] : 0.f; inv = a.inv_std[col]; }
  if constexpr (GEN_ACT) {
    if (a.batchnorm && live) beta = a.beta[col];
  }
  SMX_STAMP(2, 0);
  wide_slab_column(a.dout, a.slab_stride, a.n_slabs, col, sh);
  SMX_STAMP(2, 3);
  __syncthreads();
  float dy = 0.f;
  if (on) {
    const float acc = wide_row_value(sh, r);
    if constexpr (GEN_ACT) dy = live ? bn_gen_dy(a, r, col, acc, xv, gamma, beta) : 0.f;
    else {
      dy = (live && ov > 0.f) ? acc * a.drop_scale : 0.f;
      if (a.leak != 0.f && live && !(ov > 0.f)) dy = acc * a.leak;
    }
  }
  if (rowt) { vs[r] = dy; xs[r] = xh; }
  __syncthreads();
  if (r < 64) {
    float s1 = 0.f, s2 = 0.f;
    if (r < a.B) { const float d0 = vs[r]; s1 += d0; s2 += d0 * xs[r]; }
    if (r + 64 < a.B) { const float d1 = vs[r + 64]; s1 += d1; s2 += d1 * xs[r + 64]; }
    s1 = wide_tree64(s1);
    if (a.batchnorm) s2 = wide_tree64(s2);
    if (r == 0) { st[0] = s1; st[1] = s2; }
  }
  __syncthreads();
  const float s1 = st[0], s2 = st[1];
  SMX_STAMP(2, 5);
  if (!a.batchnorm) {
    if (r == 0 && a.dbias && live) a.dbias[col] = s1;
    if (on) a.dpre[(long)r * a.Hp + col] = dy;
    return;
  }
  if (r == 0) { a.dgamma[col] = live ? s2 : 0.f; a.dbeta[col] = live ? s1 : 0.f; }
  if (!on) return;
  const float invB = 1.f / (float)a.B;
  float d;
  if (a.training) d = (gamma * inv) * __builtin_fmaf(-__builtin_fmaf(xh, s2, s1), invB, dy);
  else d = dy * gamma * inv;
  a.dpre[(long)r * a.Hp + col] = d;
  SMX_STAMP(2, 6);
}
__global__ __launch_bounds__(BN_THREADS) void bn_wide_bwd_kernel(BnBwdArgs a) {
  __shared__ __attribute__((aligned(16))) float lds[BN_WIDE_BWD_SMEM_FLOATS];
  bn_wide_bwd_body<false>(a, lds);
}
__global__ __launch_bounds__(BN_THREADS) void bn_wide_bwd_gen_kernel(BnBwdArgs a) {
  __shared__ __attribute__((aligned(16))) float lds[BN_WIDE_BWD_SMEM_FLOATS];
  bn_wide_bwd_body<true>(a, lds);
}

template <int NP>
__global__ __launch_bounds__(BN_THREADS) void bn_wide_bwd_dw_kernel(BnBwdArgs a, HeadBwdArgs h) {
  static_assert(SMX_HEAD_DW_SMEM_FLOATS >= BN_WIDE_BWD_SMEM_FLOATS && BN_THREADS == 512, "bn_wide_bwd_dw: role 0 is a 512-thread body with the larger LDS need");
  __shared__ __attribute__((aligned(16))) float lds[SMX_HEAD_DW_SMEM_FLOATS];
  const int first_dw = (int)gridDim.x - h.n_w;
  if ((int)blockIdx.x >= first_dw) {
    preload(h.D, h.ldd, h.dP, h.ldp, h.dW, h.ldw, h.db, h.B, h.Gp, h.sq_part, h.n_w, h.n_ht, h.n_gt, h.diag, h.Hp, h.n_planes);
    head_dw_body<NP, 0, 1>(h, (int)blockIdx.x - first_dw, lds);
    return;
  }
  bn_wide_bwd_body<false>(a, lds);
}

bool bn_wide_bwd_dw_supported(const BnBwdArgs& a, const HeadBwdArgs& h) {
  return a.wide && !a.front && a.act == SMX_ACT_RELU && a.Hp % BN_COLS == 0 && a.B > 0 && a.B <= 128 && a.Hp <= 128 &&
         !h.sep && h.bf16x3 && h.n_extra == 0 && (h.n_planes == 2 || h.n_planes == 3) && h.B == a.B && h.B > 0 && h.Hp % 32 == 0 && h.Gp % 32 == 0;
}
int launch_bn_wide_bwd_dw(hipStream_t st, const BnBwdArgs& a, const HeadBwdArgs& h_in) {
  HeadBwdArgs h = h_in;
  if (!bn_wide_bwd_dw_supported(a, h) || !a.dout || a.slab_stride < (long)a.Hp * 128 || (a.slab_stride % 4) || !h.D || !h.dP || !h.dW || !h.db || h.ldd < h.Hp ||
      h.ldp < (long)h.n_planes * h.Gp || h.ldw < (long)h.n_planes * h.Gp) {
    set_error("bn_wide_bwd_dw: bad shapes");
    return SMX_ERR_INVALID;
  }
  h.n_ht = h.Hp / 32; h.n_gt = h.Gp / 32; h.n_ct = (h.B + 31) / 32;
  h.n_w = h.n_ht * ((h.n_gt + 7) / 8 * 8);
  h.skip_dd = 1; h.skip_dw = 0; h.diag = 0;
  { static const int dg = (int)tuning("head_bwd_diag", 0); if (dg) h.diag = dg; }
  if (h.sq_count) *h.sq_count = h.n_ht * h.n_gt * 8;
  const dim3 grid((unsigned)(a.Hp + (a.with_metrics ? 1 : 0) + a.adam_count + a.sqr_count + (a.close ? 1 : 0) + h.n_w));
  if (h.n_planes == 3) hipLaunchKernelGGL(bn_wide_bwd_dw_kernel<3>, grid, dim3(BN_THREADS), 0, st, a, h);
  else hipLaunchKernelGGL(bn_wide_bwd_dw_kernel<2>, grid, dim3(BN_THREADS), 0, st, a, h);
  SMX_HIP(hipGetLastError());
  return SMX_OK;
}

bool bn_wide_supported(int B, int Hp, int n_slabs) { return B > 0 && B <= 128 && Hp > 0 && Hp <= 128 && n_slabs > 0 && !tuning_on("no_bn_wide"); }

__global__ __launch_bounds__(BN_THREADS) void bn_sync_stats_fwd_kernel(BnFwdArgs a, BnSyncArgs y) {
  __shared__ float sh[BN_WAVES * BN_COLS];
  const int c = threadIdx.x % BN_COLS, rl = threadIdx.x / BN_COLS;
  const int col = blockIdx.x * BN_COLS + c;
  float s1 = 0.f;
  for (int r0 = 0; r0 < a.B; r0 += BN_RL * 2) {
    float acc[2];
    slab_sum<2>(a.pre, a.n_slabs, a.slab_stride, a.ld, col, r0, rl, a.B, acc);
#pragma unroll
    for (int i = 0; i < 2; ++i) {
      const int r = r0 + rl + BN_RL * i;
      if (r < a.B) { a.xhat[(long)r * a.Hp + col] = acc[i]; s1 += acc[i]; }
    }
  }
  s1 = bn_col_reduce(s1, sh);
  const float mean = s1 / (float)a.B;
  float s2 = 0.f;
  for (int r = rl; r < a.B; r += BN_RL) { const float d = a.xhat[(long)r * a.Hp + col] - mean; s2 += d * d; }
  s2 = bn_col_reduce(s2, sh);
  if (rl == 0)
    for (int r = 0; r < y.world; ++r) {
      y.gather[((long)r * 2 + 0) * a.Hp + col] = r == y.rank ? mean : 0.f;
      y.gather[((long)r * 2 + 1) * a.Hp + col] = r == y.rank ? s2 : 0.f;
    }
}

template <bool GEN_ACT>
__device__ inline void bn_sync_apply_fwd_body(const BnFwdArgs& a, const BnSyncArgs& y) {
  const int c = threadIdx.x % BN_COLS, rl = threadIdx.x / BN_COLS;
  const int col = blockIdx.x * BN_COLS + c;
  const bool live = col < a.H;
  float mean = 0.f;
  for (int r = 0; r < y.world; ++r) mean += y.gather[((long)r * 2) * a.Hp + col];
  mean /= (float)y.world;
  float m2 = 0.f;
  for (int r = 0; r < y.world; ++r) {
    const float d = y.gather[((long)r * 2) * a.Hp + col] - mean;
    m2 += y.gather[((long)r * 2 + 1) * a.Hp + col] + (float)a.B * d * d;
  }
  const float var = m2 / ((float)a.B * (float)y.world);
  const float inv = rsqrtf(var + a.eps);
  const float gamma = live ? a.gamma[col] : 0.f, beta = live ? a.beta[col] : 0.f;
  if (rl == 0) {
    if (a.batch_mean) { a.batch_mean[col] = mean; a.batch_var[col] = var; }
    if (a.inv_std) a.inv_std[col] = inv;
  }
  const bool drop = a.training && a.drop_p > 0.f;
  const float scale = drop ? 1.f / (1.f - a.drop_p) : 1.f;
  for (int r = rl; r < a.B; r += BN_RL) {
    const long o = (long)r * a.Hp + col;
    const float v = (a.xhat[o] - mean) * inv;
    a.xhat[o] = v;
    float h;
    if constexpr (GEN_ACT) h = act_fwd(a.act, __builtin_fmaf(gamma, v, beta));
    else h = fmaxf(gamma * v + beta, 0.f);
    if (drop) {
      float mult;
      if (a.inj_mask) mult = a.inj_mask[(long)r * a.inj_ld + col];
      else {
        const uint32_t cell = a.cell_base + (uint32_t)(a.rows ? a.rows[r] : r);
        mult = dropout_mult1(philox_row(a.nk, (uint32_t)r, cell, (uint32_t)(col >> 2)), col & 3, a.drop_p, scale);
      }
      h *= mult;
    }
    a.out[o] = live ? h : 0.f;
  }
}
__global__ __launch_bounds__(BN_THREADS) void bn_sync_apply_fwd_kernel(BnFwdArgs a, BnSyncArgs y) { bn_sync_apply_fwd_body<false>(a, y); }
__global__ __launch_bounds__(BN_THREADS) void bn_sync_apply_fwd_gen_kernel(BnFwdArgs a, BnSyncArgs y) { bn_sync_apply_fwd_body<true>(a, y); }

template <bool GEN_ACT>
__device__ inline void bn_sync_stats_bwd_body(const BnBwdArgs& a, const BnSyncArgs& y) {
  __shared__ float sh[BN_WAVES * BN_COLS];
  const int c = threadIdx.x % BN_COLS, rl = threadIdx.x / BN_COLS;
  const int col = blockIdx.x * BN_COLS + c;
  const bool live = col < a.H;
  float gamma_g = 0.f, beta_g = 0.f;
// ... 81 lines not shown
```

sisua_amd/csrc/smx_internal.h:

```cpp
#pragma once
#include <hip/hip_runtime.h>
#include <stdint.h>

#include <string>

#include "smx_device.h"
#include "smx_act.h"
#include "../../include/sisua_hip.h"

namespace smx {

void set_error(const std::string& msg);
#define SMX_HIP(call)                                                                          \
  do {                                                                                         \
    hipError_t e_ = (call);                                                                    \
    if (e_ != hipSuccess) {                                                                    \
      smx::set_error(std::string(#call) + " failed: " + hipGetErrorString(e_) + " (" __FILE__ ":" + \
                     std::to_string(__LINE__) + ")");                                          \
      return SMX_ERR_HIP;                                                                      \
    }                                                                                          \
  } while (0)

inline int round_up(int v, int m) { return (v + m - 1) / m * m; }

enum GemmTile { TILE_AUTO = 0, TILE_128x32 = 1, TILE_64x64 = 2, TILE_32x128 = 3, TILE_32x32_K4 = 4, TILE_64x32_K2 = 5 };

struct AXform {
  const int32_t* rows = nullptr;
  int log1p = 0;
  float drop_p = 0.f, drop_scale = 1.f;
  NoiseKey nk{0, 0, 0, 0, nullptr};
  uint32_t cell_base = 0;
  const float* inj_mask = nullptr;
  int inj_ld = 0;
  int u16 = 0;
};

struct EpiLatentBwd {
  const float* lat = nullptr; int ld = 0;
  const float* sig = nullptr; const float* eps = nullptr;
  KlWeight klw{nullptr, 0.f, 0.f, 0}; int D = 0, Dp = 0, stochastic = 1, relu = 0;
  float* dlat = nullptr;
  const float* dklz = nullptr;
  const float* dz_add = nullptr;
};

struct AdamArgs;
struct GemmArgs {
  const float* A = nullptr; int lda = 0; int a_kmajor = 0;
  const float* B = nullptr; int ldb = 0; int b_nmajor = 0;
  float* C = nullptr; int ldc = 0; long slab_stride = 0;
  int M = 0, N = 0, K = 0;
  int split_k = 1;
  int k_chunk = 0;
  const float* bias = nullptr;
  float* colsum = nullptr;
  int use_xform = 0;
  AXform xf;
  int tile = TILE_AUTO;
  float* sq_part = nullptr; int sq_gx = 0; int* sq_count = nullptr;
  int wide_store = 0;
  int c_colmajor = 0;
  int epi = 0;
  EpiLatentBwd lb;
  int act = 0; float leak = 0.f; const float* act_out = nullptr; int act_ld = 0;
  int act_wrap = 0;
  int panel_hint = 0;
  const AdamArgs* ride_adam = nullptr; int ride_first = 0, ride_count = 0;
};
double tuning(const char* name, double dflt);
unsigned long long tuning_epoch();
inline bool tuning_on(const char* name) { return tuning(name, 0.0) != 0.0; }
struct GemmRide;
bool gemm_ride_tile_supported(const GemmArgs& g);
int launch_gemm(hipStream_t st, const GemmArgs& g, int* eff_split = nullptr, const GemmRide* ride = nullptr);
#define SMX_GROUP_MAX 8
int launch_gemm_group(hipStream_t st, const GemmArgs* list, int n, int* eff_splits = nullptr);
int launch_gemm_dual(hipStream_t st, const GemmArgs& g1, const GemmArgs& g2, int* eff_split = nullptr);
bool dgemm_supported(const GemmArgs& g);
int launch_dgemm(hipStream_t st, const GemmArgs& g);
int suggest_split_k(int M, int N, int K);

struct LossArgs {
  int likelihood = 0;
  int direct = 0;
  int backward = 1;
  const float* X = nullptr; int ldx = 0;
  int x_u16 = 0;
  const int32_t* rows = nullptr;
  const float* P = nullptr;
// ... 321 lines not shown
int launch_score_draws(hipStream_t st, const ScoreDrawArgs& a);
struct ScoreBnArgs {
  float* h = nullptr; long R = 0; int H = 0, Hp = 0;
  const float* gamma = nullptr; const float* beta = nullptr; const float* moving_mean = nullptr; const float* moving_var = nullptr;
  float eps = 1e-3f, leak = 0.f;
  float* out_t = nullptr; long ldt = 0;
  __bf16* out3 = nullptr;
  int act = SMX_ACT_RELU;
};
struct ScoreDec1Args {
  ScoreDrawArgs d;
  const float* W = nullptr; int ldw = 0;
  int H = 0, Hp = 0;
  const float* gamma = nullptr; const float* beta = nullptr; const float* moving_mean = nullptr; const float* moving_var = nullptr;
  float eps = 1e-3f, leak = 0.f;
  __bf16* out3 = nullptr;
};
bool score_decoder1_supported(int Dp, int Hp);
int launch_score_decoder1(hipStream_t st, const ScoreDec1Args& a);
struct ScoreSplitWArgs {
  const float* W = nullptr; int ldw = 0, Gp = 0;
  int n_gt = 0, nslab = 0, NP = 0;
  __bf16* img = nullptr;
};
int launch_score_split_w(hipStream_t st, const ScoreSplitWArgs& a);
int launch_score_bn_act(hipStream_t st, const ScoreBnArgs& a);
struct ScoreHeadArgs {
  const __bf16* A3 = nullptr;
  const __bf16* Wimg = nullptr;
  const float* bias = nullptr;
  const float* X = nullptr; int ldx = 0; const int32_t* rows = nullptr; int x_u16 = 0;
  float* llk_part = nullptr;
  int R = 0, row_mod = 0, G = 0, Gp = 0, Hp = 0, likelihood = 0;
  int n_rb = 0, n_gt = 0, rb_group = 0, gt_per_xcd = 0;
  int no_queue = 0;
  int n_split = 0, wg_per_xcd = 0;
};
bool score_head_supported(int Hp, int Gp);
int launch_score_head(hipStream_t st, const ScoreHeadArgs& a);
struct ScviScoreArgs {
  const float* raw = nullptr; long ld = 0; long plane_stride = 0;
  int R = 0, G = 0, Gp = 0, k = 2, likelihood = 0, row_mod = 0;
  const float* l = nullptr; float clip_library = 1e3f;
  const float* X = nullptr; int ldx = 0; const int32_t* rows = nullptr; int x_u16 = 0;
  float* llk = nullptr;
};
bool scvi_score_supported(int Gp);
int launch_scvi_score_rows(hipStream_t st, const ScviScoreArgs& a);
struct IwStackArgs {
  const float* llk_part = nullptr; int n_chunks = 0;
  const float* lw = nullptr;
  const float* lgx1 = nullptr; const int32_t* rows = nullptr;
  float* run_max = nullptr; float* run_sum = nullptr; float* llk_sum = nullptr;
  int B = 0, S = 0, first = 1;
};
int launch_iw_stack(hipStream_t st, const IwStackArgs& a);

struct HeadBwdArgs {
  const float* D = nullptr; int ldd = 0;
  const float* dP = nullptr; long ldp = 0;
  const float* W = nullptr; int ldw = 0;
  float* dW = nullptr; float* db = nullptr;
  float* slab = nullptr; long slab_stride = 0;
  int dd_colmajor = 0;
  int B = 0, Hp = 0, Gp = 0, n_planes = 0;
  int n_slices = 0, k_chunk = 0;
  float* sq_part = nullptr; int* sq_count = nullptr;
  int sep = 0; const float* Wp[3] = {nullptr, nullptr, nullptr}; float* dWp[3] = {nullptr, nullptr, nullptr};
  float* dbp[3] = {nullptr, nullptr, nullptr}; float* sqp[3] = {nullptr, nullptr, nullptr}; int* sq_countp[3] = {nullptr, nullptr, nullptr};
  int n_extra = 0; const float* xA[SMX_MAX_LABELS] = {nullptr, nullptr, nullptr, nullptr}; int xlda[SMX_MAX_LABELS] = {0, 0, 0, 0};
  const float* xW[SMX_MAX_LABELS] = {nullptr, nullptr, nullptr, nullptr}; int xldw[SMX_MAX_LABELS] = {0, 0, 0, 0}; int xK[SMX_MAX_LABELS] = {0, 0, 0, 0};
  int n_ht = 0, n_gt = 0, n_ct = 0, n_w = 0;
  int diag = 0;
  int bf16x3 = 0;
  int skip_dw = 0;
  int skip_dd = 0;
};
bool head_bwd_supported(int B, int Hp, int Gp);
int head_bwd_slices(long ldp, int max_slabs, int* k_chunk);
int launch_out_head_bwd(hipStream_t st, const HeadBwdArgs& a);
bool bn_wide_bwd_dw_supported(const BnBwdArgs& a, const HeadBwdArgs& h);
int launch_bn_wide_bwd_dw(hipStream_t st, const BnBwdArgs& a, const HeadBwdArgs& h);
#define SMX_ADAM_SPLIT_LATE_DEFAULT 1.0f

struct BigKArgs {
  const float* A = nullptr; long lda = 0;
  int a_u16 = 0, log1p = 0; const int32_t* rows = nullptr;
  const float* Bm = nullptr; long ldb = 0; int b_kmajor = 0;
  float* part = nullptr; long slab_stride = 0;
  float* out = nullptr; int ldc = 0;
  int M = 0, N = 0, K = 0;
  int n_slices = 0, k_chunk = 0;
  int stages = 0;
  int colmajor = 0;
};
#define SMX_BIGK_STAGES_DEFAULT 2
int bigk_slices(long K, int max_slices, int* k_chunk);
bool bigk_supported(const BigKArgs& a);
int launch_bigk(hipStream_t st, const BigKArgs& a);

int launch_grad_sqsum_shard(hipStream_t st, const AdamArgs& a, int first, int count);
int launch_head_norms(hipStream_t st, const AdamArgs& a, int first, int count);
int launch_adam_shard(hipStream_t st, const AdamArgs& a, int first, int count, int wgs);
int launch_bigk_reduce(hipStream_t st, const float* part, long slab_stride, int n_slices, long n4, float* out);

#define SMX_HEAD_FUSED_TAB_BYTES (8 * 12 * 64 * 16)
#define SMX_SHARD_SLACK 4096
#define SMX_DP_BUCKETS_MIN_BYTES 3000000
#define SMX_HEAD_FUSED_MIN_GENES 4096
int head_fused_min_genes();
#define SMX_HEAD_FUSED_MAX_CELLS 256
#define SMX_HEAD_SWEEP_MIN_CHUNKS 1536
#define SMX_HEAD_SWEEP_CHUNKS_PER_WG 18
struct HeadFusedArgs {
  const float* D = nullptr; int ldd = 0;
  const float* W = nullptr; long ldw = 0;
  const float* bias = nullptr;
  const void* X = nullptr; long ldx = 0; const int32_t* rows = nullptr; int x_u16 = 0;
  float* dW = nullptr; float* db = nullptr;
  float* part = nullptr; long slab_stride = 0;
  int part_colmajor = 0;
  float* llk_part = nullptr;
  float* sq_part = nullptr;
  void* dtab = nullptr;
  int B = 0, G = 0, Gp = 0, likelihood = 0;
  float grad_scale = 1.f;
  int n_gt = 0, per_wg = 0, n_chunks = 0;
  long long* dbg = nullptr;
};
bool head_fused_supported(int B, int Hp, int Gp, int k);
int head_fused_grid(int Gp);
int head_fused_chunks(int Gp);
int launch_head_fused(hipStream_t st, const HeadFusedArgs& a, int* n_slabs, int* n_sq, hipEvent_t stop = nullptr);
int launch_head_fused_reduce(hipStream_t st, const HeadFusedArgs& a, int n_slabs, float* dd_out);
long head_fused_bytes(int B, int G, int Gp, int k);
int head_fused_prepare();

struct WgradProblem {
  const float* A; int lda; int a_mode; int log1p;
  const int32_t* rows;
  const float* Bm; int ldb;
  float* C; int ldc; int M, N;
  float* colsum; float* sq_part;
  int start, n_mt, n_nt;
  int panel;
};
struct WgradGroup { int n; int B; int b3; int pad; int starts[SMX_GROUP_MAX]; WgradProblem p[SMX_GROUP_MAX]; };
bool wgrad_supported(const GemmArgs& g, int B);

#define SMX_PANEL_MIN_WIDE 4096
struct PanelProblem {
  const void* big = nullptr; long ld_big = 0;
  int big_mode = 0, log1p = 0; const int32_t* rows = nullptr;
  long sub_stride = 0; int n_sub = 1;
  const float* S = nullptr; int ldS = 0; int n_st = 0;
  float* out = nullptr; long ld_out = 0;
  float* big_colsum = nullptr;
  float* s_colsum = nullptr;
  float* sq_part = nullptr;
  int n_wt = 0; int B = 0;
};
int panel_grid(int units);
bool panel_dw_supported(const HeadBwdArgs& a);
int launch_panel_dw(hipStream_t st, const HeadBwdArgs& a);
int launch_wgrad_group(hipStream_t st, const GemmArgs* list, int n, int B, int bf16x3 = 0, const GemmArgs* beside = nullptr);

// ... 61 lines not shown
```

sisua_amd/csrc/smx_model.h:

```cpp
#pragma once
#include <dlfcn.h>
#include <limits.h>
#include <math.h>
#include <rccl/rccl.h>
#include <stdio.h>
#include <stdlib.h>
#include <string.h>
#include <unistd.h>

#include <algorithm>
#include <condition_variable>
#include <memory>
#include <mutex>
#include <chrono>
#include <map>
#include <string>
#include <vector>

#include "../../include/sisua_hip.h"
#include "smx_internal.h"

using namespace smx;

#define SMX_CHECK(expr)            \
// ... 156 lines not shown
  std::vector<TensorInfo> tensors;
  size_t flat_count = 0, tail_off_bn = 0, tail_off_metrics = 0, grads_count = 0;
  float *params = nullptr, *grads = nullptr, *adam_m = nullptr, *adam_v = nullptr;
  int opt_rule = 0; float opt_hp[4] = {0.f, 0.f, 0.f, 0.f}; uint32_t opt_t0 = 0;
  int sched_kind[2] = {0, 0}; std::vector<double> sched_p[2];
  std::vector<MlpLayer> enc, encl, dec;
  int t_latW = -1, t_latb = -1, t_latlW = -1, t_latlb = -1;
  int t_outW[3] = {-1, -1, -1}, t_outb[3] = {-1, -1, -1};
  int t_labW[SMX_MAX_LABELS], t_labb[SMX_MAX_LABELS];
  int lab_ky[SMX_MAX_LABELS], lab_Pp[SMX_MAX_LABELS];
  std::vector<int> bn_w, bn_wp;
  std::vector<size_t> bn_off;
  float* bn_moving = nullptr;
  size_t bn_total = 0;
  float* X = nullptr; int64_t N = 0; int64_t cell_base = 0;
  float* Y[SMX_MAX_LABELS] = {nullptr, nullptr, nullptr, nullptr};
  float* library = nullptr; uint8_t* mask = nullptr; float* lgx1 = nullptr;
  float* hostX = nullptr; float* hostLib = nullptr; float* hostLgx1 = nullptr;
  float* zero_rows = nullptr;
  int32_t* rows2[2] = {nullptr, nullptr}; int32_t* order = nullptr; size_t order_cap = 0;
  float2* sched_tab = nullptr; size_t sched_cap = 0;
  int32_t* order_pin = nullptr; size_t order_pin_cap = 0; hipEvent_t ev_order = nullptr; bool order_pin_busy = false;
  int32_t* pred_ids = nullptr; int pred_ids_batch = 0;
  char* csr_host = nullptr; size_t csr_host_bytes = 0;
  float* pred_target = nullptr; size_t pred_target_floats = 0;
  float* imp_d = nullptr; size_t imp_d_floats = 0;
  unsigned long long* imp_hist = nullptr;
  int32_t* pred_sel = nullptr; size_t pred_sel_n = 0;
  char* cor_keep = nullptr; size_t cor_keep_bytes = 0;
  char* cor_ops = nullptr; size_t cor_ops_bytes = 0;
  float* metrics_pin = nullptr;
  float* score_pin = nullptr; size_t score_pin_floats = 0;
  float* mhist = nullptr; size_t mhist_cap = 0; int32_t mhist_steps = 0;
  int32_t staged_steps = 0, staged_batch = 0, staged_draws = 1;
  StepState* state3 = nullptr;
  int par = 0; uint32_t h_next = 0;
  MetricsArgs pending_metrics; bool have_pending_metrics = false, metrics_before_allreduce = false;
  int seq_batch = 0, seq_prepare_next = 0;
  bool lazy_want = false;
  bool lazy_l1 = false;
  bool lazy_closed = false;
  bool lazy_rest_pending = false, lazy_w_pending = false;
  AdamArgs lazy_args;
  int lazy_w_first = 0, lazy_w_n = 0;
  int32_t lazy_steps = 0;
  bool ahead_front_eps = false, ahead_front_drop = false;
  bool scvi_fused = false;
  bool encl_twinned = false;
  float* noise_eps = nullptr;
  float *latbuf = nullptr, *dlat = nullptr, *z = nullptr, *sig = nullptr, *eps = nullptr, *kl = nullptr;
  float *latlbuf = nullptr, *dlatl = nullptr, *lsmp = nullptr, *lsig = nullptr, *leps = nullptr, *kl_l = nullptr, *dl = nullptr;
  float *P = nullptr, *dP = nullptr, *raw = nullptr, *draw = nullptr, *rho = nullptr, *llk_part = nullptr;
  float* laby_raw[SMX_MAX_LABELS] = {nullptr, nullptr, nullptr, nullptr};
  float* laby_draw[SMX_MAX_LABELS] = {nullptr, nullptr, nullptr, nullptr};
  float* llk_y = nullptr;
  float* llk_o = nullptr;
  int n_observed = 0;
  bool out_single[3] = {false, false, false};
  bool out_has_W[3] = {true, true, true};
  float* slab = nullptr; size_t slab_cap = 0; int max_feat_p = 0;
  void* hf_tab = nullptr;
  float* shard_partial = nullptr;
  bool opt_stale = false;
  unsigned long long params_epoch = 1, wimg_epoch = 0, wimg_tuning = 0; int wimg_key = 0;
  long wide_dd_stride = 0;
  const float* wide_dd_src = nullptr;
  int wide_dd_slabs = 0;
  bool head_fused = false; int head_fused_sq = 0;
  float* bigk_part = nullptr; size_t bigk_floats = 0;
  OptChunk* chunks = nullptr; int n_chunks = 0; int chunks_floats = 4096; float* partial = nullptr; float* tensor_norm = nullptr;
  std::map<int, Injected> injected; bool use_injected = false;
  ncclComm_t comm = nullptr; int rank = 0, world = 1;
  ncclComm_t comm2 = nullptr;
  std::shared_ptr<LocalGroup> local; float* local_scratch = nullptr; size_t local_scratch_cap = 0;
  std::shared_ptr<P2PState> p2p;
  bool sync_bn = false; float* sync_buf = nullptr; size_t sync_cap = 0;
  bool dp_force = false, dp_two_buckets = false;
  int dp_form = 0;
  hipStream_t st_comm = nullptr; hipEvent_t ev_c1 = nullptr, ev_c2 = nullptr, ev_c3 = nullptr;
  size_t bucket1_off = 0, bucket1_count = 0;
  bool bucket1_in_flight = false;
  bool fold_dz_now = false;
  bool dw_late_now = false;
  bool chain_started = false;
  int audit_rows = 0, audit_disc_rows = 0; AuditStacked audit_stk;
  std::map<int, hipGraphExec_t> graphs;
  bool capturing = false;
  bool graph_comm_failed = false;
  std::string timing_label; int timing_reps = SMX_LOSS_TIMING_REPEAT; std::vector<std::pair<hipEvent_t, hipEvent_t>> timing_events; size_t timing_used = 0;
};

namespace smx {

struct Timed {
  smx_model* m; hipEvent_t stop = nullptr;
  Timed(smx_model* m_, const char* label) : m(m_) {
    if (m->capturing || m->timing_label.empty() || m->timing_label != label) return;
    if (m->timing_used == m->timing_events.size()) {
      hipEvent_t a, b;
      if (hipEventCreate(&a) != hipSuccess || hipEventCreate(&b) != hipSuccess) return;
      m->timing_events.push_back({a, b});
    }
    auto& ev = m->timing_events[m->timing_used++];
    hipEventRecord(ev.first, m->st);
    stop = ev.second;
  }
  ~Timed() { if (stop) hipEventRecord(stop, m->st); }
};

template <typename T>
int dmalloc(T** p, size_t n) {
  if (n == 0) n = 1;
  hipError_t e = hipMalloc((void**)p, n * sizeof(T));
  if (e != hipSuccess) { set_error(std::string("hipMalloc failed: ") + hipGetErrorString(e)); return SMX_ERR_NOMEM; }
  e = hipMemset(*p, 0, n * sizeof(T));
  if (e != hipSuccess) { set_error(std::string("hipMemset failed: ") + hipGetErrorString(e)); return SMX_ERR_HIP; }
  return SMX_OK;
}
struct DeviceScratch {
  std::vector<void*> p;
  DeviceScratch() = default;
  DeviceScratch(const DeviceScratch&) = delete;
  DeviceScratch& operator=(const DeviceScratch&) = delete;
  ~DeviceScratch() { for (void* q : p) hipFree(q); }
  template <class T>
  int get(T** d, size_t n) {
    *d = nullptr;
    const int rc = dmalloc(d, n);
    if (*d) p.push_back(*d);
    return rc;
  }
  template <class T>
  int put(T** d, const T* host, size_t n) {
    *d = nullptr;
    if (!host) return SMX_OK;
    SMX_CHECK(get(d, n));
    SMX_HIP(hipMemcpy(*d, host, n * sizeof(T), hipMemcpyHostToDevice));
    return SMX_OK;
  }
};
template <typename T>
int dgrow(smx_model* m, T** p, size_t* cap, size_t need, size_t want = 0) {
  if (need <= *cap) return SMX_OK;
  if (*p) { SMX_HIP(hipStreamSynchronize(m->st)); hipFree(*p); }
  *p = nullptr; *cap = 0;
  SMX_CHECK(dmalloc(p, std::max(need, want)));
  *cap = std::max(need, want);
  return SMX_OK;
}
inline int hgrow(smx_model* m, float** p, size_t* cap, size_t need, size_t want = 0) {
  if (need <= *cap) return SMX_OK;
  if (*p) { SMX_HIP(hipStreamSynchronize(m->st)); hipHostFree(*p); }
  *p = nullptr; *cap = 0;
  SMX_HIP(hipHostMalloc((void**)p, std::max(need, want) * sizeof(float), hipHostMallocDefault));
  *cap = std::max(need, want);
  return SMX_OK;
}

inline int32_t* cur_rows(smx_model* m) { return m->rows2[m->par]; }
inline StepState* cur_state(smx_model* m) { return m->state3 + m->par; }
inline StepState* master_state(smx_model* m) { return m->state3 + 2; }
inline float* P_(smx_model* m, int t) { return m->params + m->tensors[t].offset; }
inline float* G_(smx_model* m, int t) { return m->grads + m->tensors[t].offset; }

struct Pass {
  int B = 0;
// ... 41 lines not shown
inline BnSyncArgs sync_args(smx_model* m) { BnSyncArgs y; y.gather = m->sync_buf; y.rank = m->rank; y.world = m->world; return y; }
inline KlWeight kl_weight(smx_model* m, const Pass& ps, float scale, int div) {
  KlWeight w{nullptr, 0.f, scale, div};
  if (ps.training) w.beta_ptr = &cur_state(m)->beta;
  else w.beta = sched_beta(m, m->h_next);
  return w;
}
inline NoiseKey draw_key(smx_model* m, int stream, const Pass& ps) {
  NoiseKey nk = make_key(m, stream, ps.sample, ps.training != 0);
  nk.draw_rows = (uint32_t)ps.draw_rows;
  return nk;
}
template <typename A>
inline void latent_noise(smx_model* m, const Pass& ps, A& a) {
  a.nk = draw_key(m, ST_EPS_Z, ps); a.rows = ps.rows; a.cell_base = ps.cell_base;
  if (const Injected* ij = inj(m, ST_EPS_Z)) { a.inj_eps = ij->d; a.inj_ld = ij->ld; }
}
inline bool b3_on(const smx_model* m, int B) {
  return m->flags.bf16x3 < 0 ? use_bf16x3((long)B * m->Gp * m->k) : m->flags.bf16x3 != 0;
}
inline float* sq_part_of(smx_model* m, int t) {
  return (m->sq_slots && !tuning_on("no_sq_partials")) ? m->sq_slots + m->sq_first[(size_t)t] : nullptr;
}
inline void want_sq(smx_model* m, GemmArgs& g, int t) {
  if (!(g.sq_part = sq_part_of(m, t))) return;
  g.sq_count = &m->sq_count[(size_t)t];
}
struct Mat { const float* p; int ld; Mat(const float* p_, long ld_) : p(p_), ld((int)ld_) {} };
inline GemmArgs dense_fwd(Mat H, Mat W, float* Y, int ldy, const float* bias, int M, int N, int K) {
  GemmArgs g;
  g.A = H.p; g.lda = H.ld; g.B = W.p; g.ldb = W.ld; g.C = Y; g.ldc = ldy; g.bias = bias; g.M = M; g.N = N; g.K = K;
  return g;
}
inline GemmArgs dense_wgrad(smx_model* m, Mat H, Mat dY, int tW, float* db, int M, int N, int K) {
  GemmArgs g;
  g.A = H.p; g.lda = H.ld; g.a_kmajor = 1; g.B = dY.p; g.ldb = dY.ld; g.C = G_(m, tW); g.ldc = m->tensors[tW].ld; g.colsum = db;
  g.M = M; g.N = N; g.K = K;
  want_sq(m, g, tW);
  return g;
}
inline GemmArgs dense_dgrad(Mat dY, Mat W, float* slabs, int M, int N, int K) {
  GemmArgs g;
  g.A = dY.p; g.lda = dY.ld; g.B = W.p; g.ldb = W.ld; g.b_nmajor = 1; g.C = slabs; g.ldc = N; g.slab_stride = (long)M * N;
  g.M = M; g.N = N; g.K = K;
  return g;
}
inline void x_gather(smx_model* m, const Pass& ps, GemmArgs& g) {
  g.use_xform = 1;
  g.xf.rows = ps.xrows; g.xf.u16 = ps.x_u16; g.xf.log1p = m->cfg.log_norm; g.xf.cell_base = ps.cell_base;
  if (ps.training && m->cfg.input_dropout > 0.f) {
    g.xf.drop_p = m->cfg.input_dropout; g.xf.drop_scale = 1.f / (1.f - m->cfg.input_dropout);
    g.xf.nk = make_key(m, ST_INPUT_DROPOUT, ps.sample, true);
    if (const Injected* ij = inj(m, ST_INPUT_DROPOUT)) { g.xf.inj_mask = ij->d; g.xf.inj_ld = ij->ld; }
  }
}
inline ScviHeadArgs scvi_head_args(smx_model* m, const Pass& ps) {
  ScviHeadArgs sh;
  sh.raw = m->raw; sh.planes = m->P; sh.ld = (long)m->k * m->Gp; sh.plane_stride = m->Gp; sh.B = ps.B; sh.G = m->G; sh.Gp = m->Gp;
  sh.k = m->k; sh.l = m->lsmp; sh.clip_library = m->cfg.clip_library; sh.rho_raw = m->rho;
  return sh;
}

enum class Fwd { Full, DecodeOnly, Resample, EncodeOnly, EncodeRaw };
enum class Loss { None, Eval, Train };
int forward_pass(smx_model* m, const Pass& ps, Loss loss, Fwd mode = Fwd::Full);
int factor_forward(smx_model* m, const Pass& ps, bool backward);
bool use_head_loss(const smx_model* m, int B);
int backward_pass(smx_model* m, const Pass& ps);
int factor_backward(smx_model* m, const Pass& ps);
bool head_sweep_ok(smx_model* m);
int head_sweep_prepare(smx_model* m);
int head_sweep_join(smx_model* m);
int dp_chain_start(smx_model* m);
void fill_adam_args(smx_model* m, AdamArgs& a);
void fill_step_close(smx_model* m, AdamArgs& a);
bool lazy_adam_wanted(smx_model* m, bool prepare_next);
int lazy_flush(smx_model* m);
bool lazy_ride_tile(smx_model* m, const GemmArgs& g, GemmRide& r);
bool lazy_ride_w(smx_model* m, GemmRide& r);
int optimizer_pass(smx_model* m);
int csr_stage(smx_model* m, Pass& ps);
int check_rows(smx_model* m, const int32_t* ids, size_t n);
int read_metrics(smx_model* m, smx_metrics* out);
struct CsrRows { const int64_t* indptr; const int32_t* cols; const float* vals; };
int check_csr_rows(const CsrRows& c, size_t n, int G);
int csr_host_rows(smx_model* m, const CsrRows& c, size_t r0, size_t n, void* out, float* lgx1, int u16 = 0);
struct CellSrc { const int32_t* row_ids; const float* host_x; const float* host_library; };
int setup_pass(smx_model* m, Pass& ps, const CellSrc& src, int32_t batch, int training, int sample, int draw_rows = 0);
bool stacked_scoring_ok(const smx_model* m);
bool head_fused_ok(const smx_model* m, int B);
int stacked_decoder(smx_model* m, const float* z, long rows, float* const* hb, int last_form, float* ht, const float** out, int* out_ld);
#define SMX_IMP_L1_BINS 2048
#define SMX_IMP_LN_BINS 1024
#define SMX_IMP_HIST_WORDS (SMX_IMP_L1_BINS + 2 * SMX_IMP_LN_BINS + 1)
struct ImputeRowArgs {
  const float* mean; long ldm;
  const float* orig; long ldo;
  const float* cor; long ldc;
  int G, d_only;
  float* d;
  float* median; int32_t* changed;
  unsigned long long* hist;
};
int launch_impute_rows(hipStream_t st, const ImputeRowArgs& a, int rows);
int launch_impute_level(hipStream_t st, const float* d, long n, const unsigned* prefix, unsigned mask, int shift, unsigned long long* hist);
int launch_gather_cols(hipStream_t st, const float* src, long ld, long rows, const int32_t* idx, int n_sel, float* dst);
#define SMX_COR_MAX_CELLS (1l << 20)
struct CorrelateArgs {
  const float* cols; const int32_t* rank2; int N, P;
  const int32_t* prot_rank2; const double* prot_unit;
  long long *sp_Sa, *sp_Saa, *sp_Sab;
  double *pe_mean, *pe_Sxx, *pe_Sxy;
};
struct CorrelateWork {
  float* cols; int32_t* rank2; unsigned *sortA, *sortB; const int32_t* prot_rank2; const double* prot_unit; char* sums;
};
struct CorrelateOut { long long *sp_Sa, *sp_Saa, *sp_Sab; double *pe_mean, *pe_Sxx, *pe_Sxy; int32_t* nonfinite; };
inline size_t correlate_sums_bytes(size_t n, size_t P) { return n * ((2 + P) * 16 + 4); }
int launch_keep_cols(hipStream_t st, const float* src, long ld, long rows, const int32_t* idx, int n_sel, float* dst, long N, long c0);
int launch_col_rank2(hipStream_t st, const float* cols, int n_cols, long N, unsigned* sortA, unsigned* sortB, int32_t* rank2, int32_t* nonfinite);
int launch_col_correlate(hipStream_t st, const CorrelateArgs& a, int n_cols);
int correlate_kept(hipStream_t st, const CorrelateWork& w, int n, long N, int P, const CorrelateOut& o);

}
```

sisua_amd/csrc/smx_model.hip:

```cpp
#include <atomic>
#include <cfloat>
#include "smx_model.h"

namespace smx {

static thread_local std::string g_err;
void set_error(const std::string& msg) { g_err = msg; }
const char* last_error_cstr() { return g_err.c_str(); }

int add_tensor(smx_model* m, const std::string& name, int rows, int cols, int chunks, bool vec) {
  TensorInfo t;
  t.name = name; t.rows = vec ? 1 : rows; t.cols = cols; t.chunks = chunks;
  t.chunk_w = cols / chunks; t.chunk_wp = round_up(t.chunk_w, 32);
  t.rows_p = vec ? 1 : round_up(rows, 32);
  t.ld = chunks * t.chunk_wp;
  t.offset = m->flat_count;
  t.count = (size_t)t.rows_p * t.ld;
  m->flat_count += (t.count + 63) / 64 * 64;
  m->tensors.push_back(t);
  return (int)m->tensors.size() - 1;
}

int build_mlp(smx_model* m, std::vector<MlpLayer>& mlp, const char* prefix, int n_in, int n, const int32_t* units,
              int stream0, float drop_p, bool batchnorm, float leak) {
// ... 445 lines not shown
    if ((rc = dmalloc(&m->zero_rows, B))) return fail(rc);
    if (hipMemset(m->zero_rows, 0, B * sizeof(float)) != hipSuccess) { set_error("zero_rows: hipMemset failed"); return fail(SMX_ERR_HIP); }
  }
  set_row_caps(m, B);
  std::vector<OptChunk> chunks;
  const int CH = 4096;
  for (size_t t = 0; t < m->tensors.size(); ++t) {
    const TensorInfo& ti = m->tensors[t];
    const int first = (int)chunks.size();
    const int n = (int)((ti.count + CH - 1) / CH);
    for (int i = 0; i < n; ++i) {
      OptChunk c;
      memset(&c, 0, sizeof(c));
      c.tensor = (int)t; c.offset = (int)(ti.offset + (size_t)i * CH);
      c.count = (int)((size_t)(i + 1) * CH <= ti.count ? CH : ti.count - (size_t)i * CH);
      c.first_chunk = first; c.n_chunks = n; c.tensor_count = (int32_t)ti.count;
      chunks.push_back(c);
    }
  }
  m->n_chunks = (int)chunks.size();
  m->chunks_floats = CH;
  m->chunk_first_head = m->n_chunks;
  for (size_t i = 0; i < chunks.size(); ++i)
    if (chunks[i].tensor == m->t_outW[0]) { m->chunk_first_head = (int)i; break; }
  m->chunk_first_label = m->n_chunks;
  if (m->n_heads > 0)
    for (size_t i = 0; i < chunks.size(); ++i)
      if (chunks[i].tensor == m->t_labW[0]) { m->chunk_first_label = (int)i; break; }
  if (m->tensors.size() <= SMX_MAX_TENSORS) {
    size_t total = 0;
    m->sq_first.assign(m->tensors.size(), 0);
    m->sq_count.assign(m->tensors.size(), 0);
    for (size_t t = 0; t < m->tensors.size(); ++t) {
      const TensorInfo& ti = m->tensors[t];
      m->sq_first[t] = (int)total;
      total += (size_t)((ti.rows_p + 31) / 32) * (size_t)((ti.ld + 31) / 32) * 8;
    }
    m->sq_total_first = (int)total;
    m->sq_reduced.assign(m->tensors.size(), 0);
    if ((rc = dmalloc(&m->sq_slots, total + m->tensors.size() * SMX_SQR_PER_TENSOR))) return fail(rc);
  }
  if ((rc = dmalloc(&m->chunks, chunks.size())) || (rc = dmalloc(&m->partial, chunks.size())) || (rc = dmalloc(&m->shard_partial, chunks.size())) ||
      (rc = dmalloc(&m->tensor_norm, m->tensors.size())))
    return fail(rc);
  if (hipMemcpy(m->chunks, chunks.data(), chunks.size() * sizeof(OptChunk), hipMemcpyHostToDevice) != hipSuccess) {
    set_error("chunk table copy failed"); return fail(SMX_ERR_HIP);
  }
  *out = m;
  return SMX_OK;
}

int smx_model_destroy(smx_model* m) {
  if (!m) return SMX_OK;
  if (m->st) hipStreamSynchronize(m->st);
  for (auto& kv : m->graphs) hipGraphExecDestroy(kv.second);
  for (auto& ev : m->timing_events) { hipEventDestroy(ev.first); hipEventDestroy(ev.second); }
  if (m->bigk_part) hipFree(m->bigk_part);
  if (m->hf_tab) hipFree(m->hf_tab);
  p2p_release(m);
  if (m->comm2 && g_rccl.CommDestroy) g_rccl.CommDestroy(m->comm2);
  m->comm2 = nullptr;
  if (m->comm && g_rccl.CommDestroy) g_rccl.CommDestroy(m->comm);
  m->comm = nullptr;
  m->local.reset();
  auto fr = [](void* p) { if (p) hipFree(p); };
  fr(m->local_scratch); fr(m->sync_buf);
  fr(m->params); fr(m->grads); fr(m->adam_m); fr(m->adam_v); fr(m->bn_moving);
  for (auto* mlp : {&m->enc, &m->encl, &m->dec})
    for (auto& L : *mlp) { fr(L.xhat); fr(L.out_buf); fr(L.dpre); fr(L.inv_std); fr(L.noise); }
  release_dataset(m);
  fr(m->hostX); fr(m->hostLib); fr(m->hostLgx1); fr(m->zero_rows);
  for (int j = 0; j < SMX_MAX_LABELS; ++j) { fr(m->laby_raw[j]); fr(m->laby_draw[j]); }
  fr(m->rows2[0]); fr(m->rows2[1]); fr(m->order); fr(m->sched_tab); fr(m->state3); fr(m->mhist);
  fr(m->resp); fr(m->dklz); fr(m->zmean); fr(m->zpick); fr(m->tril_part); fr(m->ltril);
  for (auto& L : m->disc) { fr(L.xhat); fr(L.out_buf); fr(L.dpre); }
  fr(m->zz); fr(m->u_d); fr(m->tc_cell); fr(m->dl_cell); fr(m->dz_tc); fr(m->disc_dpre); fr(m->disc_db);
  fr(m->noise_eps); fr(m->latbuf); fr(m->dlat); fr(m->z); fr(m->sig); fr(m->eps); fr(m->kl);
  fr(m->latlbuf); fr(m->dlatl); fr(m->lsmp); fr(m->lsig); fr(m->leps); fr(m->kl_l); fr(m->dl);
  fr(m->P); fr(m->dP); fr(m->raw); fr(m->draw); fr(m->rho); fr(m->llk_part); fr(m->llk_y); fr(m->llk_o); fr(m->slab);
  fr(m->chunks); fr(m->partial); fr(m->shard_partial); fr(m->tensor_norm); fr(m->sq_slots);
  if (m->pinned) hipHostFree(m->pinned);
  if (m->order_pin) hipHostFree(m->order_pin);
  if (m->metrics_pin) hipHostFree(m->metrics_pin);
  if (m->score_pin) hipHostFree(m->score_pin);
  if (m->ev_order) hipEventDestroy(m->ev_order);
  if (m->pred_stage) hipFree(m->pred_stage);
  if (m->pred_target) hipFree(m->pred_target);
  if (m->csr_host) hipFree(m->csr_host);
  if (m->pred_ids) hipFree(m->pred_ids);
  if (m->imp_d) hipFree(m->imp_d);
  if (m->imp_hist) hipFree(m->imp_hist);
  if (m->pred_sel) hipFree(m->pred_sel);
  if (m->cor_keep) hipFree(m->cor_keep);
  if (m->cor_ops) hipFree(m->cor_ops);
  if (m->score_buf) hipFree(m->score_buf);
  if (m->score_wimg) hipFree(m->score_wimg);
  if (m->score_aux) hipFree(m->score_aux);
  for (auto& kv : m->injected) fr(kv.second.d);
  if (m->st_comm) { hipStreamSynchronize(m->st_comm); hipStreamDestroy(m->st_comm); }
  if (m->st_side) { hipStreamSynchronize(m->st_side); hipStreamDestroy(m->st_side); }
  if (m->ev_hf) hipEventDestroy(m->ev_hf);
  if (m->ev_sweep) hipEventDestroy(m->ev_sweep);
  if (m->ev_c1) hipEventDestroy(m->ev_c1);
  if (m->ev_c2) hipEventDestroy(m->ev_c2);
  if (m->ev_c3) hipEventDestroy(m->ev_c3);
  if (m->st) hipStreamDestroy(m->st);
  delete m;
  return SMX_OK;
}

int smx_num_tensors(const smx_model* m) { return m ? (int)m->tensors.size() : 0; }

int smx_tensor_info(const smx_model* m, int index, char* name, int name_cap, int32_t* rows, int32_t* cols) {
  SMX_REQUIRE(m && index >= 0 && index < (int)m->tensors.size(), "tensor index out of range");
  const TensorInfo& t = m->tensors[index];
  if (name && name_cap > 0) { strncpy(name, t.name.c_str(), name_cap - 1); name[name_cap - 1] = 0; }
  if (rows) *rows = t.rows;
  if (cols) *cols = t.cols;
  return SMX_OK;
}

static float* which_buf(smx_model* m, int which) {
  switch (which) { case 0: return m->params; case 1: return m->grads; case 2: return m->adam_m; case 3: return m->adam_v; }
  return nullptr;
}

int smx_get_tensor(smx_model* m, int which, int index, float* host) {
  SMX_REQUIRE(m && host && index >= 0 && index < (int)m->tensors.size(), "bad tensor index");
  float* base = which_buf(m, which);
  SMX_REQUIRE(base, "which must be 0..3");
  const TensorInfo& t = m->tensors[index];
  SMX_REQUIRE(!(m->opt_stale && (which == 2 || which == 3) && t.offset >= m->bucket1_off),
              "the heads' Adam moments are sharded over the ranks (flag opt_shard): call smx_opt_gather on every rank first");
  std::vector<float> dev(t.count);
  SMX_HIP(hipStreamSynchronize(m->st));
  SMX_HIP(hipMemcpy(dev.data(), base + t.offset, t.count * sizeof(float), hipMemcpyDeviceToHost));
  unpack(t, dev, host, 1.f);
  return SMX_OK;
}

int smx_set_tensor(smx_model* m, int which, int index, const float* host) {
  SMX_REQUIRE(m && host && index >= 0 && index < (int)m->tensors.size(), "bad tensor index");
  float* base = which_buf(m, which);
  SMX_REQUIRE(base, "which must be 0..3");
  const TensorInfo& t = m->tensors[index];
  std::vector<float> dev;
  pack(t, host, dev);
  SMX_HIP(hipStreamSynchronize(m->st));
  SMX_HIP(hipMemcpy(base + t.offset, dev.data(), t.count * sizeof(float), hipMemcpyHostToDevice));
  if (which == 0) ++m->params_epoch;
  return SMX_OK;
}

namespace smx {
struct AuditBuf { std::string name; const void* p = nullptr; long rows = 0; int ld = 0, width = 0, wp = 0, form = 0; };
static inline bool pad_nonzero(float v) { uint32_t b; memcpy(&b, &v, 4); return (b & 0x7fffffffu) != 0u; }
static inline bool pad_element(const TensorInfo& t, size_t i) {
  const size_t r = i / (size_t)t.ld, c = i % (size_t)t.ld;
  return (int)r >= t.rows || (int)(c % (size_t)t.chunk_wp) >= t.chunk_w;
}
struct PadTally {
  int64_t n_bad = 0, first_offset = -1; int first = -1; std::string first_name;
  void hit(int index, const std::string& name, int64_t off) {
    if (n_bad++ == 0) { first = index; first_name = name; first_offset = off; }
  }
};
// ... 155 lines not shown
  SMX_HIP(hipMemset(ij.d, 0, (size_t)m->Bmax * ld * sizeof(float)));
  SMX_HIP(hipMemcpy2D(ij.d, (size_t)ld * sizeof(float), data, (size_t)width * sizeof(float), (size_t)width * sizeof(float),
                      (size_t)batch, hipMemcpyHostToDevice));
  m->use_injected = true;
  return SMX_OK;
}

int smx_clear_noise(smx_model* m) {
  SMX_REQUIRE(m, "null model");
  SMX_HIP(hipStreamSynchronize(m->st));
  for (auto& kv : m->injected) if (kv.second.d) hipFree(kv.second.d);
  m->injected.clear();
  m->use_injected = false;
  return SMX_OK;
}

int smx_set_flag(smx_model* m, const char* name, int value) {
  SMX_REQUIRE(m && name, "null argument");
  SMX_HIP(hipStreamSynchronize(m->st));
  const std::string n(name);
  int* f = n == "head_loss" ? &m->flags.head_loss : n == "head_fused" ? &m->flags.head_fused : n == "head_sweep" ? &m->flags.head_sweep : n == "front" ? &m->flags.front : n == "bwd_front" ? &m->flags.bwd_front
         : n == "head_bwd" ? &m->flags.head_bwd : n == "wgrad" ? &m->flags.wgrad : n == "scvi_fused" ? &m->flags.scvi_fused
         : n == "twin" ? &m->flags.twin : n == "label_ride" ? &m->flags.label_ride : n == "act_epilogue" ? &m->flags.act_epilogue
         : n == "stacked_scoring" ? &m->flags.stacked_scoring : n == "bf16x3" ? &m->flags.bf16x3 : n == "opt_shard" ? &m->flags.opt_shard
         : n == "tie_mixtures" ? &m->flags.tie_mixtures : n == "tie_loc" ? &m->flags.tie_loc : n == "tie_scale" ? &m->flags.tie_scale : nullptr;
  SMX_REQUIRE(f, "unknown flag (head_loss, head_fused, head_sweep, front, bwd_front, head_bwd, wgrad, scvi_fused, twin, label_ride, act_epilogue, stacked_scoring, bf16x3, opt_shard; SCALE: tie_mixtures, tie_loc, tie_scale)");
  *f = (f == &m->flags.bf16x3 && value < 0) ? -1 : (value ? 1 : 0);
  drop_graphs(m);
  return SMX_OK;
}

int smx_set_activation(smx_model* m, int32_t net, int32_t act) {
  SMX_REQUIRE(m, "null model");
  SMX_REQUIRE(act >= SMX_ACT_RELU && act <= SMX_ACT_SOFTPLUS, "smx_set_activation: unknown activation");
  std::vector<MlpLayer>* mlp = net == SMX_NET_ENCODER ? &m->enc : net == SMX_NET_DECODER ? &m->dec : net == SMX_NET_LIBRARY_ENCODER ? &m->encl : nullptr;
  SMX_REQUIRE(mlp, "smx_set_activation: unknown network (encoder 0, decoder 1, library encoder 2)");
  SMX_REQUIRE(net != SMX_NET_LIBRARY_ENCODER || !m->encl.empty(), "smx_set_activation: the model has no library encoder");
  SMX_HIP(hipStreamSynchronize(m->st));
  for (auto& L : *mlp) L.act = act;
  drop_graphs(m);
  return SMX_OK;
}

int smx_timing_enable(smx_model* m, const char* kernel) {
  SMX_REQUIRE(m, "null model");
  SMX_HIP(hipStreamSynchronize(m->st));
  m->timing_label = kernel ? kernel : "";
  m->timing_reps = SMX_LOSS_TIMING_REPEAT;
  const size_t at = m->timing_label.find('@');
  if (at != std::string::npos) {
    m->timing_reps = std::max(1, atoi(m->timing_label.c_str() + at + 1));
    m->timing_label.resize(at);
  }
  m->timing_used = 0;
  return SMX_OK;
}

int smx_timing_read(smx_model* m, double* total_ms, int64_t* launches) {
  SMX_REQUIRE(m && total_ms && launches, "null argument");
  SMX_HIP(hipStreamSynchronize(m->st));
  double tot = 0.0;
  for (size_t i = 0; i < m->timing_used; ++i) {
    float ms = 0.f;
    SMX_HIP(hipEventElapsedTime(&ms, m->timing_events[i].first, m->timing_events[i].second));
    tot += ms;
  }
  *total_ms = tot; *launches = (int64_t)m->timing_used;
  m->timing_used = 0;
  return SMX_OK;
}

int64_t smx_loss_bytes_per_cell(const smx_model* m) {
  if (!m) return 0;
  return (int64_t)(4 + 8 * m->k) * m->G + 16 * (int64_t)m->D + 4;
}

int64_t smx_head_fused_bytes(const smx_model* m, int32_t batch) {
  if (!m || batch <= 0 || m->dec.empty()) return 0;
  return head_fused_ok(m, batch) ? (int64_t)head_fused_bytes(batch, m->G, m->Gp, m->k) : 0;
}

int32_t smx_head_dw_late(const smx_model* m) { return (m && m->dw_late_now) ? 1 : 0; }
int32_t smx_lazy_adam_steps(const smx_model* m) { return m ? m->lazy_steps : 0; }

}
```

sisua_amd/csrc/smx_step.hip:

```cpp
#include "smx_model.h"

namespace smx {

__global__ void bn_moving_update_kernel(float* moving, const float* batch_sum, int n, float inv_world, float momentum) {
  const int i = blockIdx.x * blockDim.x + threadIdx.x;
  if (i < n) moving[i] = moving[i] * momentum + batch_sum[i] * inv_world * (1.f - momentum);
}

void fill_adam_args(smx_model* m, AdamArgs& a) {
  const smx_config& c = m->cfg;
  a.params = m->params; a.grads = m->grads; a.m = m->adam_m; a.v = m->adam_v;
  a.chunks = m->chunks; a.n_chunks = m->n_chunks; a.n_launch = m->n_chunks; a.gap_from = m->n_chunks; a.gap_len = 0;
  a.partial = m->partial; a.tensor_norm = m->tensor_norm;
  a.use_sq = (m->sq_slots != nullptr && !dp_active(m) && !tuning_on("no_sq_partials")) ? 1 : 0;
  for (size_t t = 0; t < m->tensors.size() && a.use_sq; ++t) {
    a.sq_first[t] = m->sq_first[t]; a.sq_count[t] = m->sq_count[t];
    if (m->sq_count[t] == 0 && m->tensors[t].count > SMX_SQ_SMALL_TENSOR) a.use_sq = 0;
    if (m->sq_reduced[t]) { a.sq_first[t] = m->sq_total_first + (int)t * SMX_SQR_PER_TENSOR; a.sq_count[t] = m->sq_reduced[t]; }
  }
  a.sq_slots = m->sq_slots;
  a.state = cur_state(m); a.clipnorm = c.clipnorm;
  opt_scalars(m->opt_rule, m->opt_hp, a); a.t0 = m->opt_t0;
  a.grad_scale = 1.f;
  if (m->scale && (m->flags.tie_loc || m->flags.tie_scale)) {
// ... 74 lines not shown
    SMX_CHECK(launch_metrics(m->st, m->pending_metrics));
    m->have_pending_metrics = false;
  }
  const bool chain = dp_chain_ok(m);
  if (chain) {
    Timed t(m, "allreduce");
    SMX_CHECK(dp_chain_start(m));
    SMX_CHECK(dp_allreduce(m, 0, m->bucket1_off, m->st));
  } else if (dp_active(m)) {
    Timed t(m, "allreduce");
    if (m->bucket1_in_flight) {
      SMX_HIP(hipEventRecord(m->ev_c2, m->st));
      SMX_HIP(hipStreamWaitEvent(m->st_comm, m->ev_c2, 0));
      SMX_CHECK(dp_allreduce(m, 0, m->bucket1_off, m->st_comm));
      SMX_HIP(hipEventRecord(m->ev_c3, m->st_comm));
      SMX_HIP(hipStreamWaitEvent(m->st, m->ev_c3, 0));
      m->bucket1_in_flight = false;
    } else {
      SMX_CHECK(dp_allreduce(m, 0, m->grads_count, m->st));
    }
  }
  AdamArgs a;
  fill_adam_args(m, a);
  if (chain) a.sq_chunks = m->chunk_first_head;
  m->chain_started = false;
  if (dp_active(m) && m->bn_total && m->world > 1) {
    if (!a.use_sq) {
      a.bn_moving = m->bn_moving; a.bn_batch = m->grads + m->tail_off_bn; a.bn_total = (int)m->bn_total;
      a.bn_inv_world = 1.f / (float)m->world; a.bn_momentum = c.bn_momentum;
    } else {
      hipLaunchKernelGGL(bn_moving_update_kernel, dim3((unsigned)((m->bn_total + 255) / 256)), dim3(256), 0, m->st,
                         m->bn_moving, m->grads + m->tail_off_bn, (int)m->bn_total, 1.f / (float)m->world,
                         c.bn_momentum);
    }
  }
  if (m->adam_early_from >= 0) {
    a.gap_from = m->adam_early_from; a.gap_len = m->adam_early_to - m->adam_early_from;
    a.n_launch = m->n_chunks - a.gap_len;
  } else {
    a.gap_from = m->n_chunks; a.gap_len = 0; a.n_launch = m->n_chunks;
  }
  m->adam_early_from = -1;
  if (m->have_pending_metrics) { a.metrics = m->pending_metrics; a.with_metrics = 1; m->have_pending_metrics = false; }
  fill_step_close(m, a);
  if (m->lazy_closed) a.master = nullptr;
  if (lazy_defer(m, a)) return SMX_OK;
  Timed t(m, "adam");
  SMX_CHECK(launch_adam(m->st, a));
  return SMX_OK;
}

int csr_stage(smx_model* m, Pass& ps) {
  if (!m->x_csr || ps.Xsrc != m->X) return SMX_OK;
  SMX_REQUIRE(ps.rows != nullptr && ps.B <= m->Rmax, "sparse store: resident rows only");
  SMX_REQUIRE(!(ps.training && m->cfg.input_dropout > 0.f), "sparse store: input dropout is keyed by the dense store's rows (use the float32 / uint16 store)");
  SMX_CHECK(launch_csr_expand(m->st, m->csr_indptr, m->csr_cols, m->csr_vals, ps.rows, 0, ps.B, m->Gp, m->xbatch));
  ps.Xsrc = m->xbatch; ps.xrows = nullptr; ps.x_u16 = 0;
  return SMX_OK;
}

int train_sequence(smx_model* m, int B, bool with_begin, bool begin_from_master, uint32_t cursor, bool prepare_next) {
  Pass ps;
  ps.B = B; ps.rows = cur_rows(m); ps.xrows = ps.rows; ps.Xsrc = m->X; ps.x_u16 = m->x_u16; ps.lib = m->library; ps.lgx1 = m->lgx1;
  ps.cell_base = (uint32_t)m->cell_base; ps.training = 1; ps.sample = 0; ps.global_batch = B * m->world;
  ps.draw_rows = m->train_draws > 1 ? B / m->train_draws : 0;
  m->seq_batch = B; m->seq_prepare_next = prepare_next ? 1 : 0;
  m->lazy_want = lazy_adam_wanted(m, prepare_next); m->lazy_l1 = false; m->lazy_closed = false;
  Timed t(m, "step");
  if (with_begin) {
    AdamArgs o;
    opt_scalars(m->opt_rule, m->opt_hp, o);
    SMX_CHECK(launch_step_begin(m->st, master_state(m), cur_state(m), m->order, cur_rows(m), B, begin_from_master ? 1 : 0,
                                cursor, m->sched_tab, o.b1, o.b2, o.form, m->opt_t0));
  }
  m->chain_started = false;
  { Timed null_pair(m, "null"); }
  SMX_CHECK(csr_stage(m, ps));
  SMX_CHECK(forward_pass(m, ps, Loss::Train));
  SMX_CHECK(backward_pass(m, ps));
  SMX_CHECK(optimizer_pass(m));
  return SMX_OK;
}

int read_metrics(smx_model* m, smx_metrics* out) {
  if (!out) return SMX_OK;
  const size_t nt = m->tensors.size();
  if (!m->metrics_pin) SMX_HIP(hipHostMalloc((void**)&m->metrics_pin, (8 + nt + 1) * sizeof(float), hipHostMallocDefault));
  float* h = m->metrics_pin;
  float* norms_p = m->metrics_pin + 8;
  unsigned* p2p_err = reinterpret_cast<unsigned*>(m->metrics_pin + 8 + nt);
  *p2p_err = 0u;
  SMX_HIP(hipMemcpyAsync(h, m->grads + m->tail_off_metrics, 8 * sizeof(float), hipMemcpyDeviceToHost, m->st));
  SMX_HIP(hipMemcpyAsync(norms_p, m->tensor_norm, nt * sizeof(float), hipMemcpyDeviceToHost, m->st));
  if (m->p2p && m->p2p->error) SMX_HIP(hipMemcpyAsync(p2p_err, m->p2p->error, sizeof(unsigned), hipMemcpyDeviceToHost, m->st));
  SMX_HIP(hipStreamSynchronize(m->st));
  if (*p2p_err) {
    set_error(*p2p_err == 1u ? "peer-to-peer all-reduce: a wait on a peer's flag timed out (SMX_P2P_TIMEOUT_S)" :
                               "peer-to-peer all-reduce: a peer reported a timed-out wait");
    return SMX_ERR_COMM;
  }
  std::vector<float> norms(norms_p, norms_p + nt);
  out->loss = h[0]; out->nllk_x = h[1]; out->nllk_y = h[2]; out->kl = h[3]; out->kl_l = h[4];
  float mx = 0.f;
  for (float v : norms) mx = (v > mx || v != v) ? v : mx;
  out->grad_norm_max = mx;
  out->nan_flag = !(isfinite(h[0]) && isfinite(h[1]) && isfinite(h[3]) && isfinite(mx));
  out->step = (int32_t)m->h_next;
  out->tc = h[5]; out->dtc_loss = h[6]; out->nllk_o = h[7];
  if (m->n_observed && !isfinite(h[7])) out->nan_flag = 1;
  if (m->fvae && !(isfinite(h[5]) && isfinite(h[6]))) out->nan_flag = 1;
  return SMX_OK;
}

int upload_order(smx_model* m, const int32_t* order, size_t n, size_t n_steps) {
  if (n_steps > m->mhist_cap) {
    SMX_HIP(hipStreamSynchronize(m->st));
    drop_graphs(m);
    if (m->mhist) hipFree(m->mhist);
    m->mhist = nullptr; m->mhist_cap = 0;
    SMX_CHECK(dmalloc(&m->mhist, (n_steps * 2 + 64) * 8));
    m->mhist_cap = n_steps * 2 + 64;
  }
  m->mhist_steps = (int32_t)n_steps;
  if (n > m->order_cap) {
    SMX_HIP(hipStreamSynchronize(m->st));
    drop_graphs(m);
    if (m->order) hipFree(m->order);
    m->order = nullptr;
    m->order_cap = n * 2 + (size_t)m->Bmax;
    SMX_CHECK(dmalloc(&m->order, m->order_cap));
  }
  if (n_steps > m->sched_cap) {
    SMX_HIP(hipStreamSynchronize(m->st));
    drop_graphs(m);
    if (m->sched_tab) hipFree(m->sched_tab);
    m->sched_tab = nullptr;
    m->sched_cap = n_steps * 2 + 64;
    SMX_CHECK(dmalloc(&m->sched_tab, m->sched_cap));
  }
  const size_t need = n + 2 * n_steps;
  if (need > m->order_pin_cap) {
    if (m->order_pin_busy) { SMX_HIP(hipEventSynchronize(m->ev_order)); m->order_pin_busy = false; }
    if (m->order_pin) hipHostFree(m->order_pin);
    m->order_pin = nullptr; m->order_pin_cap = 0;
    SMX_HIP(hipHostMalloc((void**)&m->order_pin, (need * 2 + (size_t)m->Bmax) * sizeof(int32_t), hipHostMallocDefault));
    m->order_pin_cap = need * 2 + (size_t)m->Bmax;
  }
  if (!m->ev_order) SMX_HIP(hipEventCreateWithFlags(&m->ev_order, hipEventDisableTiming));
  if (m->order_pin_busy) { SMX_HIP(hipEventSynchronize(m->ev_order)); m->order_pin_busy = false; }
  memcpy(m->order_pin, order, n * sizeof(int32_t));
  float* tab = reinterpret_cast<float*>(m->order_pin + n);
  sched_fill(m, tab, n_steps);
  SMX_HIP(hipMemcpyAsync(m->order, m->order_pin, n * sizeof(int32_t), hipMemcpyHostToDevice, m->st));
  SMX_HIP(hipMemcpyAsync(m->sched_tab, tab, n_steps * sizeof(float2), hipMemcpyHostToDevice, m->st));
  SMX_HIP(hipEventRecord(m->ev_order, m->st));
  m->order_pin_busy = true;
  SMX_HIP(hipMemsetAsync(&master_state(m)->cursor, 0, sizeof(uint32_t), m->st));
  return SMX_OK;
}

int check_rows(smx_model* m, const int32_t* ids, size_t n) {
  SMX_REQUIRE(m->X != nullptr, "no dataset uploaded (smx_dataset_upload)");
  for (size_t i = 0; i < n; ++i)
    if (ids[i] < 0 || (int64_t)ids[i] >= m->N) { set_error("row id out of range"); return SMX_ERR_INVALID; }
  return SMX_OK;
}

int launch_train(smx_model* m, int B, bool use_graph, int s_idx, int n_steps) {
  static const bool no_graph_comm = tuning_on("no_graph_comm");
  if (use_graph && !m->local && !m->p2p && !(m->comm && (no_graph_comm || m->graph_comm_failed)) && !m->use_injected && m->timing_label.empty()) {
    auto it = m->graphs.find(B);
    if (it == m->graphs.end()) {
      hipGraph_t graph = nullptr;
      SMX_HIP(hipStreamBeginCapture(m->st, hipStreamCaptureModeThreadLocal));
      m->capturing = true;
      m->par = 0;
      int rc = train_sequence(m, B, true, true, 0, false);
      m->capturing = false;
// ... 80 lines not shown
}

}

extern "C" {

int smx_set_train_draws(smx_model* m, int32_t n_draws) {
  SMX_REQUIRE(m, "null model");
  SMX_REQUIRE(n_draws >= 1, "smx_set_train_draws: the number of draws must be >= 1");
  SMX_REQUIRE(n_draws == 1 || !m->fvae, "smx_set_train_draws: FactorVAE / SemiFVAE train with one draw (permute_dims over stacked draws has no agreed reading)");
  SMX_REQUIRE(n_draws == 1 || m->world == 1, "smx_set_train_draws: several draws per cell are single-GPU only (data parallel world > 1)");
  SMX_REQUIRE((int64_t)n_draws * m->Bmax <= (int64_t)1 << 20, "smx_set_train_draws: draws x max_batch exceeds 2^20 stacked rows");
  if (n_draws == m->train_draws) return SMX_OK;
  SMX_CHECK(smx::head_sweep_join(m));
  SMX_HIP(hipStreamSynchronize(m->st));
  smx::drop_graphs(m);
  if ((int64_t)n_draws * m->Bmax > m->Rmax) SMX_CHECK(smx::alloc_rows(m, (size_t)n_draws * m->Bmax));
  m->train_draws = n_draws;
  m->staged_steps = 0;
  return SMX_OK;
}

int smx_set_optimizer(smx_model* m, int32_t rule, const float* hp, int32_t n_hp) {
  SMX_REQUIRE(m, "null model");
  const float adam_hp[3] = {m->cfg.adam_beta1, m->cfg.adam_beta2, m->cfg.adam_eps};
  float res[4];
  SMX_CHECK(smx::opt_resolve(rule, hp, n_hp, adam_hp, res));
  SMX_CHECK(smx::head_sweep_join(m));
  SMX_HIP(hipStreamSynchronize(m->st));
  smx::drop_graphs(m);
  const long n = (long)(m->flat_count + SMX_SHARD_SLACK);
  SMX_CHECK(smx::launch_opt_fill(m->st, m->adam_m, n, 0.f));
  SMX_CHECK(smx::launch_opt_fill(m->st, m->adam_v, n, 0.f));
  if (rule == SMX_OPT_ADAGRAD && res[0] != 0.f) {
    std::vector<float> h((size_t)n, 0.f);
    for (const TensorInfo& t : m->tensors)
      for (int r = 0; r < t.rows; ++r)
        for (int ch = 0; ch < t.chunks; ++ch)
          std::fill_n(h.begin() + (long)(t.offset + (size_t)r * t.ld + (size_t)ch * t.chunk_wp), t.chunk_w, res[0]);
    SMX_HIP(hipStreamSynchronize(m->st));
    SMX_HIP(hipMemcpy(m->adam_v, h.data(), h.size() * sizeof(float), hipMemcpyHostToDevice));
  }
  SMX_HIP(hipStreamSynchronize(m->st));
  m->opt_stale = false;
  m->opt_rule = rule;
  for (int i = 0; i < 4; ++i) m->opt_hp[i] = res[i];
  m->opt_t0 = m->h_next;
  return SMX_OK;
}

int smx_get_optimizer(const smx_model* m, int32_t* rule, float* hp, int32_t* t0) {
  SMX_REQUIRE(m, "null model");
  if (rule) *rule = m->opt_rule;
  if (hp) for (int i = 0; i < SMX_OPT_MAX_HP; ++i) hp[i] = m->opt_hp[i];
  if (t0) *t0 = (int32_t)m->opt_t0;
  return SMX_OK;
}

int smx_train_step(smx_model* m, const int32_t* row_ids, int32_t batch, smx_metrics* out) {
  return smx_train_steps(m, row_ids, 1, batch, 0, out);
}
int smx_train_step_graph(smx_model* m, const int32_t* row_ids, int32_t batch, smx_metrics* out) {
  return smx_train_steps(m, row_ids, 1, batch, 1, out);
}

int smx_train_steps(smx_model* m, const int32_t* order, int32_t n_steps, int32_t batch, int use_graph, smx_metrics* out) {
  SMX_REQUIRE(m && n_steps > 0, "bad arguments");
  SMX_REQUIRE(batch > 0 && batch <= m->Bmax, "batch must be in 1..max_batch");
  SMX_CHECK(smx::check_draws(m));
  if (order) {
    SMX_CHECK(check_rows(m, order, (size_t)n_steps * batch));
    const std::vector<int32_t> tiled = smx::tile_draws(m, order, n_steps, batch);
    SMX_CHECK(upload_order(m, tiled.empty() ? order : tiled.data(), (size_t)n_steps * batch * m->train_draws, (size_t)n_steps));
  } else {
    SMX_REQUIRE(m->staged_steps == n_steps && m->staged_batch == batch && m->staged_draws == m->train_draws,
              "order = NULL: no ids staged for this n_steps x batch (smx_train_stage) and draw count");
  }
  m->staged_steps = 0;
  if (m->opt_stale && (use_graph || !(m->flags.opt_shard && smx::dp_chain_ok(m) && smx::dp_shard_available(m)))) SMX_CHECK(smx_opt_gather(m));
  int rc = SMX_OK;
  ++m->params_epoch;
  smx::DrawCaps caps(m);
  m->lazy_steps = 0;
  for (int s = 0; s < n_steps && rc == SMX_OK; ++s) rc = launch_train(m, batch * m->train_draws, use_graph != 0, s, n_steps);
  { const int rf = smx::lazy_flush(m); if (rc == SMX_OK) rc = rf; }
  { const int rj = smx::head_sweep_join(m); if (rc == SMX_OK) rc = rj; }
  if (rc != SMX_OK) return rc;
  if (m->use_injected) { m->use_injected = false; }
  SMX_CHECK(read_metrics(m, out));
  return SMX_OK;
}

int smx_train_stage(smx_model* m, const int32_t* order, int32_t n_steps, int32_t batch) {
  SMX_REQUIRE(m && order && n_steps > 0, "bad arguments");
  SMX_REQUIRE(batch > 0 && batch <= m->Bmax, "batch must be in 1..max_batch");
  SMX_CHECK(smx::check_draws(m));
  SMX_CHECK(check_rows(m, order, (size_t)n_steps * batch));
  const std::vector<int32_t> tiled = smx::tile_draws(m, order, n_steps, batch);
  SMX_CHECK(upload_order(m, tiled.empty() ? order : tiled.data(), (size_t)n_steps * batch * m->train_draws, (size_t)n_steps));
  m->staged_steps = n_steps; m->staged_batch = batch; m->staged_draws = m->train_draws;
  return SMX_OK;
}

int smx_metrics_history(smx_model* m, int32_t n_steps, float* host) {
  SMX_REQUIRE(m && host && n_steps > 0 && n_steps <= m->mhist_steps, "no such history (steps of the last smx_train_steps call)");
  SMX_HIP(hipStreamSynchronize(m->st));
  SMX_HIP(hipMemcpy(host, m->mhist, (size_t)n_steps * 8 * sizeof(float), hipMemcpyDeviceToHost));
  return SMX_OK;
}

int smx_eval_step(smx_model* m, const int32_t* row_ids, int32_t batch, smx_metrics* out) {
  SMX_REQUIRE(m && row_ids, "bad arguments");
  SMX_CHECK(smx::check_draws(m));
  Pass ps;
  smx::DrawCaps caps(m);
  if (m->train_draws > 1) {
    SMX_REQUIRE(batch > 0 && batch <= m->Bmax, "batch must be in 1..max_batch");
    SMX_CHECK(check_rows(m, row_ids, (size_t)batch));
    const std::vector<int32_t> tiled = smx::tile_draws(m, row_ids, 1, batch);
    SMX_CHECK(setup_pass(m, ps, {tiled.data(), nullptr, nullptr}, batch * m->train_draws, 0, 0, batch));
    SMX_HIP(hipStreamSynchronize(m->st));
  } else {
    SMX_CHECK(setup_pass(m, ps, {row_ids, nullptr, nullptr}, batch, 0, 0));
  }
  SMX_CHECK(forward_pass(m, ps, Loss::Eval));
  SMX_CHECK(read_metrics(m, out));
  return SMX_OK;
}

}
```

sisua_amd/engine.py:

```python
from __future__ import annotations

import ctypes as C
from typing import Dict, Optional, Sequence

import numpy as np

from sisua_amd import _hip, interpolation, optimizers
from sisua_amd._hip import SmxError, check, smx_config, smx_metrics
from sisua_amd.config import ModelConfig, init_params, label_planes, manifest

STREAM_INPUT_DROPOUT = 0
STREAM_ENC_DROPOUT = 16
STREAM_ENCL_DROPOUT = 32
STREAM_DEC_DROPOUT = 48
STREAM_EPS_Z = 64
STREAM_EPS_L = 65


def _fp(a: Optional[np.ndarray]):
  return None if a is None else a.ctypes.data_as(C.POINTER(C.c_float))


def _f32(a, shape=None):
  a = np.ascontiguousarray(a, dtype=np.float32)
# ... 598 lines not shown
  def comm_p2p_init(self, rank: int, world: int, all_handles: bytes):
    if len(all_handles) != 128 * world:
      raise ValueError("all_handles must hold world x 128 bytes in rank order")
    buf = (C.c_uint8 * len(all_handles)).from_buffer_copy(all_handles)
    check(self.lib.smx_comm_p2p_init(self._h, int(rank), int(world), buf))

  def comm_p2p_error(self) -> int:
    e = C.c_int32(0)
    check(self.lib.smx_comm_p2p_error(self._h, C.byref(e)))
    return int(e.value)

  def comm_time_allreduce(self, iters: int = 50):
    us, n = C.c_float(0.0), C.c_int64(0)
    check(self.lib.smx_comm_time_allreduce(self._h, int(iters), C.byref(us), C.byref(n)))
    return float(us.value), 4 * int(n.value)

  @property
  def world(self) -> int:
    return self.lib.smx_comm_world(self._h)

  @property
  def rank(self) -> int:
    return self.lib.smx_comm_rank(self._h)

  @property
  def comm_form(self) -> int:
    return self.lib.smx_comm_form(self._h)

  FORM_NAMES = {0: "none", 1: "one all-reduce", 2: "two-bucket chain", 3: "hand-written exchange", 4: "hand-written exchange, two buckets"}

  def comm_set_form(self, form: int):
    check(self.lib.smx_comm_set_form(self._h, int(form)))

  def opt_gather(self):
    check(self.lib.smx_opt_gather(self._h))

  def set_sync_bn(self, on: bool = True):
    check(self.lib.smx_comm_set_sync_bn(self._h, int(bool(on))))

  @staticmethod
  def comm_library() -> dict:
    lib = _hip.load()
    a, b, v = C.create_string_buffer(4096), C.create_string_buffer(4096), C.c_int32()
    check(lib.smx_comm_library(a, 4096, b, 4096, C.byref(v)))
    return dict(rccl=a.value.decode(), hip=b.value.decode(), rccl_version=int(v.value))

  @staticmethod
  def comm_init_local(engines: Sequence["Engine"]):
    lib = _hip.load()
    arr = (C.c_void_p * len(engines))(*[e._h for e in engines])
    check(lib.smx_comm_init_local(arr, len(engines)))

  def set_flag(self, name: str, value: bool):
    v = -1 if (name == "bf16x3" and not isinstance(value, bool) and int(value) < 0) else int(bool(value))
    check(self.lib.smx_set_flag(self._h, name.encode(), v))

  def pad_audit(self, which: int):
    n, t, off = C.c_int64(0), C.c_int32(-1), C.c_int64(-1)
    name = C.create_string_buffer(64)
    check(self.lib.smx_pad_audit(self._h, int(which), C.byref(n), C.byref(t), C.byref(off), name, 64))
    return int(n.value), (name.value.decode() if n.value else None), int(off.value)

  def pad_poke(self, which: int, tensor, value: float = 1.0):
    index = self.index[tensor] if isinstance(tensor, str) else int(tensor)
    check(self.lib.smx_pad_poke(self._h, int(which), index, float(value)))

  def timing_enable(self, kernel: Optional[str]):
    check(self.lib.smx_timing_enable(self._h, kernel.encode() if kernel else None))

  def timing_read(self):
    ms, n = C.c_double(), C.c_int64()
    check(self.lib.smx_timing_read(self._h, C.byref(ms), C.byref(n)))
    return ms.value, n.value

  def loss_bytes_per_cell(self) -> int:
    return int(self.lib.smx_loss_bytes_per_cell(self._h))

  def head_fused_bytes(self, batch: int) -> int:
    return int(self.lib.smx_head_fused_bytes(self._h, int(batch)))

  def head_dw_late(self) -> bool:
    return bool(self.lib.smx_head_dw_late(self._h))

  def lazy_adam_steps(self) -> int:
    return int(self.lib.smx_lazy_adam_steps(self._h))

  def synchronize(self):
    check(self.lib.smx_synchronize())


def k_count_llk(likelihood: str, x, planes, direct: bool = False, want_grads: bool = True):
  lib = _hip.require_gpu()
  x = _f32(x)
  B, G = x.shape
  pl = _f32(planes)
  k = pl.shape[0]
  llk = np.empty(B, np.float32)
  grads = np.empty((k, B, G), np.float32) if want_grads else None
  check(lib.smx_k_count_llk(_hip.LIKELIHOODS[likelihood], int(direct), _fp(x), _fp(pl), B, G, _fp(llk), _fp(grads)))
  return llk, grads


def k_head_fused(likelihood: str, x, d, W, bias, grad_scale: float = 1.0, u16: bool = False, reps: int = 0):
  lib = _hip.require_gpu()
  x, d, W, bias = _f32(x), _f32(d), _f32(W), _f32(bias)
  B, G = x.shape
  k = W.shape[1]
  assert d.shape == (B, 128) and W.shape == (128, k, G) and bias.shape == (k, G)
  llk = np.empty(B, np.float32)
  dW, db, dd = np.empty((128, k, G), np.float32), np.empty((k, G), np.float32), np.empty((B, 128), np.float32)
  sumsq, us = np.zeros(1, np.float32), np.zeros(1, np.float32)
  check(lib.smx_k_head_fused(_hip.LIKELIHOODS[likelihood], int(u16), _fp(x), _fp(d), _fp(W), _fp(bias), B, G, float(grad_scale), int(reps),
                             _fp(llk), _fp(dW), _fp(db), _fp(dd), _fp(sumsq), _fp(us)))
  return dict(llk=llk, dW=dW, db=db, dd=dd, sumsq=float(sumsq[0]), us=float(us[0]))


def k_head_fused_stress(likelihood: str, x, d, W, bias, launches: int, grad_scale: float = 1.0, u16: bool = False):
  lib = _hip.require_gpu()
  x, d, W, bias = _f32(x), _f32(d), _f32(W), _f32(bias)
  B, G = x.shape
  k = W.shape[1]
  assert d.shape == (B, 128) and W.shape == (128, k, G) and bias.shape == (k, G)
  n, first = C.c_int32(0), C.c_int64(-1)
  check(lib.smx_k_head_fused_stress(_hip.LIKELIHOODS[likelihood], int(u16), _fp(x), _fp(d), _fp(W), _fp(bias), B, G, float(grad_scale), int(launches),
                                    C.byref(n), C.byref(first)))
  return int(n.value), int(first.value)


def k_adam(params, grads, m, v, step: int, lr=1e-3, beta1=0.9, beta2=0.999, eps=1e-7, clipnorm=100.0):
  lib = _hip.require_gpu()
  sizes = np.array([int(np.size(p)) for p in params], dtype=np.int32)
  cat = lambda xs: np.ascontiguousarray(np.concatenate([np.asarray(x, np.float32).ravel() for x in xs]))
  P, G, M, V = cat(params), cat(grads), cat(m), cat(v)
  norms = np.empty(len(sizes), np.float32)
  check(lib.smx_k_adam(len(sizes), sizes.ctypes.data_as(C.POINTER(C.c_int32)), _fp(P), _fp(G), _fp(M), _fp(V), int(step),
                       float(lr), float(beta1), float(beta2), float(eps), float(clipnorm), _fp(norms)))
  cut = np.cumsum(sizes)[:-1]
  shp = [np.shape(p) for p in params]
  un = lambda flat: [a.reshape(sh) for a, sh in zip(np.split(flat, cut), shp)]
  return un(P), un(M), un(V), norms


def k_opt(rule: str, params, grads, m, v, step: int, lr=1e-3, clipnorm=100.0, **hp):
  lib = _hip.require_gpu()
  name, full = optimizers.canonical(rule, **hp)
  hv = optimizers.hp_vector(name, full)
  sizes = np.array([int(np.size(p)) for p in params], dtype=np.int32)
  cat = lambda xs: np.ascontiguousarray(np.concatenate([np.asarray(x, np.float32).ravel() for x in xs]))
  P, G, M, V = cat(params), cat(grads), cat(m), cat(v)
  norms = np.empty(len(sizes), np.float32)
  check(lib.smx_k_opt(optimizers.RULES[name][0], _fp(hv), len(hv), len(sizes), sizes.ctypes.data_as(C.POINTER(C.c_int32)), _fp(P), _fp(G),
                      _fp(M), _fp(V), int(step), float(lr), float(clipnorm), _fp(norms)))
  cut = np.cumsum(sizes)[:-1]
  shp = [np.shape(p) for p in params]
  un = lambda flat: [a.reshape(sh) for a, sh in zip(np.split(flat, cut), shp)]
  return un(P), un(M), un(V), norms


OPT_CARRIERS = {"launch": 0, "sweep": 1, "shard": 2, "body512": 3}


def k_opt_carrier(rule: str, params, grads, m, v, step: int, carrier="launch", wgs=0, world=0, use_sq=False, sq=None, lr=1e-3, clipnorm=100.0,
                  grad_scale=1.0, t0=0, tied=(), tied_inv=1.0, hp_raw=None, **hp):
  lib = _hip.require_gpu()
  if hp_raw is None:
    name, full = optimizers.canonical(rule, **hp)
# ... 964 lines not shown
```

Measured before the change: 2.130 million.

## Fuse decoder BN backward and encoder front backward into one launch with in-kernel handoff

The decoder's wide BN-backward-with-head-dW launch is deferred and merged with the encoder's last-layer fold_dz backward into a single kernel. Encoder workgroups spin on sharded device-scope counters until decoder column workgroups have published d pre-activation, so the two launches and the gap between them collapse into one grid. This brings a persistent handoff-state buffer, a timeout error path checked when metrics are read, and a deadlock risk if consumer blocks occupy the GPU before producers are scheduled. Spin-waiting and extra LDS may also reduce occupancy.

```diff
diff --git a/include/sisua_hip.h b/include/sisua_hip.h
--- a/include/sisua_hip.h
+++ b/include/sisua_hip.h
@@ -222,6 +222,7 @@
 int64_t smx_head_fused_bytes(const smx_model* m, int32_t batch);
 int32_t smx_head_dw_late(const smx_model* m);
 int32_t smx_lazy_adam_steps(const smx_model* m);
+int32_t smx_bwd_seam_steps(const smx_model* m);
 
 int smx_k_count_llk(int likelihood, int direct, const float* x, const float* planes, int32_t B, int32_t G,
                     float* llk, float* grads);
diff --git a/sisua_amd/_hip.py b/sisua_amd/_hip.py
--- a/sisua_amd/_hip.py
+++ b/sisua_amd/_hip.py
@@ -159,6 +159,7 @@
     "smx_head_fused_bytes": (C.c_int64, [_VP, C.c_int32]),
     "smx_head_dw_late": (C.c_int32, [_VP]),
     "smx_lazy_adam_steps": (C.c_int32, [_VP]),
+    "smx_bwd_seam_steps": (C.c_int32, [_VP]),
     "smx_k_count_llk": (C.c_int, [C.c_int, C.c_int, _FP, _FP, C.c_int32, C.c_int32, _FP, _FP]),
     "smx_k_head_fused": (C.c_int, [C.c_int, C.c_int, _FP, _FP, _FP, _FP, C.c_int32, C.c_int32, C.c_float, C.c_int32, _FP, _FP, _FP, _FP, _FP,
                                    _FP]),
diff --git a/sisua_amd/build.py b/sisua_amd/build.py
--- a/sisua_amd/build.py
+++ b/sisua_amd/build.py
@@ -7,7 +7,7 @@
 CSRC = os.path.join(HERE, "csrc")
 LIB = os.path.join(HERE, "libsisua_hip.so")
 SOURCES = ["smx_gemm.hip", "smx_dgemm.hip", "smx_bn.hip", "smx_latent.hip", "smx_adam.hip", "smx_loss.hip", "smx_data.hip", "smx_headloss.hip", "smx_headbwd.hip", "smx_headfused.hip", "smx_bigk.hip", "smx_factor.hip", "smx_scvi.hip", "smx_score.hip", "smx_model.hip", "smx_dataset.hip", "smx_comm.hip", "smx_p2p.hip", "smx_forward.hip", "smx_backward.hip", "smx_step.hip", "smx_predict.hip", "smx_sample.hip", "smx_impute.hip", "smx_correlate.hip", "smx_cluster.hip", "smx_gmm.hip", "smx_gmm_full.hip", "smx_prep.hip", "smx_pca.hip", "smx_knn.hip", "smx_tsne.hip", "smx_mi.hip", "smx_rankgroups.hip", "smx_mbkmeans.hip", "smx_louvain.hip", "smx_logreg.hip", "smx_scoring.hip", "smx_schedule.hip", "smx_kapi.hip"]
-HEADERS = ["smx_device.h", "smx_act.h", "smx_internal.h", "smx_loss.h", "smx_model.h", "smx_panel.h", "smx_dgemm.h", "smx_adam.h", "smx_headdw.h", "smx_dist.h", "smx_block.h", "smx_prep.h", os.path.join("..", "..", "include", "sisua_hip.h")]
+HEADERS = ["smx_device.h", "smx_act.h", "smx_internal.h", "smx_loss.h", "smx_model.h", "smx_panel.h", "smx_dgemm.h", "smx_adam.h", "smx_headdw.h", "smx_handoff.h", "smx_dist.h", "smx_block.h", "smx_prep.h", os.path.join("..", "..", "include", "sisua_hip.h")]
 FLAGS = ["--offload-arch=gfx950", "-O3", "-std=c++17", "-fPIC", "-fno-slp-vectorize", "-Wall", "-Wno-unused-function", "-Wno-unused-value", "-Wno-unused-result"]
 
 
diff --git a/sisua_amd/csrc/smx_backward.hip b/sisua_amd/csrc/smx_backward.hip
--- a/sisua_amd/csrc/smx_backward.hip
+++ b/sisua_amd/csrc/smx_backward.hip
@@ -183,6 +183,34 @@
   bool last_bn_done = false;
   const HeadBwdArgs* head_dw = nullptr;
 };
+static bool seam_wanted(const smx_model* m, const Pass& ps) {
+  return m->dw_late_now && m->fold_dz_now && m->dec.size() == 1 && !dp_active(m) && !m->comm && !m->local && !m->p2p && m->world == 1 && !m->sync_bn && !sync_bn_on(m, ps.training) &&
+         m->timing_label.empty() && !m->capturing && !m->lazy_rest_pending && m->enc.back().out_p / 8 <= HANDOFF_MAX_WAITERS && !tuning_on("no_bwd_seam");
+}
+static int seam_flush(smx_model* m) {
+  if (!m->seam_pending) return SMX_OK;
+  m->seam_pending = false;
+  return launch_bn_wide_bwd_dw(m->st, m->seam_dec, m->seam_head);
+}
+static int seam_launch(smx_model* m, const BnBwdArgs& enc) {
+  m->seam_pending = false;
+  if (!m->seam_state) {
+    SMX_HIP(hipMalloc((void**)&m->seam_state, HANDOFF_STATE_BYTES));
+    m->seam_epochs = 0;
+  }
+  if (m->seam_epochs == 0) SMX_HIP(hipMemsetAsync(m->seam_state, 0, HANDOFF_STATE_BYTES, m->st));
+  BwdSeamArgs sm;
+  sm.seam.counter = m->seam_state; sm.seam.error = m->seam_state + HANDOFF_MAX_SHARDS * HANDOFF_SHARD_STRIDE;
+  sm.seam.shards = HANDOFF_MAX_SHARDS;
+  sm.seam.target = (unsigned)m->seam_dec.Hp * (m->seam_epochs + 1);
+  sm.seam.timeout_ticks = (long long)(std::min(std::max((double)tuning("bwd_seam_timeout_s", 2.0), 0.01), 60.0) * 1e8);
+  sm.preread = tuning_on("bwd_seam_preread") ? 1 : 0;
+  sm.cons_first = tuning_on("bwd_seam_cons_first") ? 1 : 0;
+  SMX_CHECK(launch_bn_bwd_seam(m->st, m->seam_dec, enc, m->seam_head, sm));
+  ++m->seam_epochs; ++m->seam_steps;
+  return SMX_OK;
+}
+
 static int mlp_backward(smx_model* m, std::vector<MlpLayer>& mlp, const Pass& ps, Mat in0, bool in_is_x, int n_slabs, const MlpBwdOpts& o) {
   auto make_b = [&](MlpLayer& L, int slabs, const BnBwdArgs* front) {
     BnBwdArgs b;
@@ -224,6 +252,9 @@
     have_carried = false;
     const bool dpre_ready = dpre_done;
     dpre_done = false;
+    const bool seam = m->seam_pending && &mlp == &m->enc && last && b.front && b.fold_dz && !o.last_bn_done && !dpre_ready && !(sync_bn_on(m, ps.training) && L.bn >= 0) &&
+                      !(m->metrics_before_allreduce && m->have_pending_metrics) && bn_bwd_seam_supported(m->seam_dec, b, m->seam_head);
+    if (m->seam_pending && &mlp != &m->dec && !seam) SMX_CHECK(seam_flush(m));
     if ((last && o.last_bn_done) || dpre_ready) {
     } else if (sync_bn_on(m, ps.training) && L.bn >= 0) {
       Timed t(m, "bn_bwd");
@@ -237,7 +268,8 @@
         b.metrics = m->pending_metrics; b.with_metrics = 1; m->have_pending_metrics = false;
       }
       const HeadBwdArgs* hd = (last && o.head_dw && bn_wide_bwd_dw_supported(b, *o.head_dw)) ? o.head_dw : nullptr;
-      if (!hd) attach_early_adam(m, b);
+      if (seam) m->adam_early_pending = false;
+      else if (!hd) attach_early_adam(m, b);
       const bool w_rides = hd && b.adam_count == 0 && b.sqr_count == 0 && m->lazy_w_pending && !m->lazy_rest_pending;
       if (w_rides) { b.adam = m->lazy_args; b.adam_first = m->lazy_w_first; b.adam_count = m->lazy_w_n; }
       if (m->lazy_want && m->lazy_l1 && !m->lazy_closed && &mlp == &m->enc && m->have_pending_metrics) {
@@ -250,10 +282,16 @@
       const bool dual = last && b.front && b.fK <= 64 && o.twin && o.twin_front && o.twin_front->fK <= 64 && !o.twin->empty() && m->flags.twin && bn_dual_supported(ps.B) &&
                         bn_bwd_front_supported(ps.B, o.twin_front->fK) && o.twin->back().out_p % 8 == 0 &&
                         !(sync_bn_on(m, ps.training) && o.twin->back().bn >= 0);
-      if (hd) {
+      if (hd && &mlp == &m->dec && (w_rides || !m->lazy_w_pending) && seam_wanted(m, ps)) {
+        m->seam_dec = b; m->seam_head = *hd; m->seam_pending = true;
+        dw_carried = true;
+        if (w_rides) m->lazy_w_pending = false;
+      } else if (hd) {
         SMX_CHECK(launch_bn_wide_bwd_dw(m->st, b, *hd));
         dw_carried = true;
         if (w_rides) m->lazy_w_pending = false;
+      } else if (seam) {
+        SMX_CHECK(seam_launch(m, b));
       } else if (dual) {
         const BnBwdArgs b2 = make_b(o.twin->back(), 0, o.twin_front);
         SMX_CHECK(launch_bn_act_bwd_dual(m->st, b, b2));
diff --git a/sisua_amd/csrc/smx_bn.hip b/sisua_amd/csrc/smx_bn.hip
--- a/sisua_amd/csrc/smx_bn.hip
+++ b/sisua_amd/csrc/smx_bn.hip
@@ -1,5 +1,6 @@
 #include "smx_internal.h"
 #include "smx_adam.h"
+#include "smx_handoff.h"
 
 namespace smx {
 
@@ -493,7 +494,8 @@
 }
 #define SMX_FOLD_WROW 136
 #define SMX_FOLD_WIMG_BYTES (3 * 32 * SMX_FOLD_WROW * 2)
-__device__ inline void fold_dz_tile(const BnBwdArgs& a, const int bid, float* tile, const int ldd, unsigned char* wimg) {
+template <bool SEAM = false>
+__device__ inline bool fold_dz_tile(const BnBwdArgs& a, const int bid, float* tile, const int ldd, unsigned char* wimg, const BwdSeamArgs* sm = nullptr, int* seam_ok = nullptr) {
   const EpiLatentBwd& e = a.zlb;
   const int tid = threadIdx.x, lane = tid & 63, w = tid >> 6, li = lane & 15, kg = lane >> 4;
   float e_mu[2][4], e_sr[2][4], e_sg[2][4], e_ep[2][4];
@@ -518,6 +520,12 @@
     row[0] = sp.t0;
     row[(32 * SMX_FOLD_WROW * 2) / 16] = sp.t1;
     row[(2 * 32 * SMX_FOLD_WROW * 2) / 16] = sp.t2;
+  }
+  if constexpr (SEAM) {
+    if (sm->preread) {
+      for (int i = tid; i < a.B * 4; i += BN_THREADS) { const float t = a.zD[(long)(i >> 2) * a.zld + (i & 3) * 32]; asm volatile("" ::"v"(t)); }
+    }
+    if (!handoff_wait<true>(sm->seam, seam_ok)) return false;
   }
   Split8 A[4];
   {
@@ -557,6 +565,7 @@
         if (bid == 0) { e.dlat[(long)b * e.ld + d] = o0; e.dlat[(long)b * e.ld + e.Dp + d] = o1; }
       }
     }
+  return true;
 }
 
 __device__ inline float bn_keep(const BnBwdArgs& a, int r, int col) {
@@ -570,12 +579,13 @@
   return dout * bn_keep(a, r, col) * act_grad(a.act, act_fwd(a.act, y));
 }
 
-template <int RPT, int FRONT, bool GEN_ACT = false>
-__device__ inline void bn_act_bwd_body(const BnBwdArgs& a, const int bid) {
+template <int RPT, int FRONT, bool GEN_ACT = false, bool SEAM = false>
+__device__ inline void bn_act_bwd_body(const BnBwdArgs& a, const int bid, const BwdSeamArgs* sm = nullptr) {
   constexpr bool SMALL = RPT > 0;
   constexpr int BN_RPT = SMALL ? RPT : BN_RPT_DEFAULT;
+  static_assert(!SEAM || (FRONT == 1 && !GEN_ACT), "the seam form is the fold_dz front's");
   extern __shared__ __attribute__((aligned(16))) float ds[];
-  {
+  if constexpr (!SEAM) {
     const int nb = a.Hp / BN_COLS, extra = bid - nb;
     if (extra >= 0) {
       const int e = extra - (a.with_metrics ? 1 : 0);
@@ -626,6 +636,10 @@
     const bool wl_on = (int)threadIdx.x < BN_COLS * kq && !(a.diag & 64);
     if (wl_on) wl = *reinterpret_cast<const float4*>(a.fW + (long)(bid * BN_COLS + ((int)threadIdx.x >> ksh)) * a.fldw + ((int)threadIdx.x & kmask) * 4);
     if (FRONT == 1 && a.fold_dz) {
+      if constexpr (SEAM) {
+        __shared__ int seam_ok;
+        if (!fold_dz_tile<true>(a, bid, ds, ldd, reinterpret_cast<unsigned char*>(ws + BN_COLS * ldw_s), sm, &seam_ok)) return;
+      } else
       fold_dz_tile(a, bid, ds, ldd, reinterpret_cast<unsigned char*>(ws + BN_COLS * ldw_s));
       if ((int)threadIdx.x < BN_COLS * kq) *reinterpret_cast<float4*>(&ws[((int)threadIdx.x >> ksh) * ldw_s + ((int)threadIdx.x & kmask) * 4]) = wl;
     } else
@@ -958,11 +972,10 @@
 __global__ __launch_bounds__(BN_THREADS) void bn_wide_fwd_gen_kernel(BnFwdArgs a) { bn_wide_fwd_body<true>(a); }
 
 constexpr int BN_WIDE_BWD_SMEM_FLOATS = 16 * 128 + 128 + 128 + 4;
-template <bool GEN_ACT>
-__device__ inline void bn_wide_bwd_body(const BnBwdArgs& a, float* lds) {
+template <bool GEN_ACT, bool SEAM = false>
+__device__ inline void bn_wide_bwd_body(const BnBwdArgs& a, float* lds, const int bid, const BwdSeamArgs* sm = nullptr) {
 #pragma clang fp contract(off)
-  const int bid = (int)blockIdx.x;
-  {
+  if constexpr (!SEAM) {
     const int extra = bid - a.Hp;
     if (extra >= 0) {
       const int e = extra - (a.with_metrics ? 1 : 0);
@@ -1026,10 +1039,25 @@
   SMX_STAMP(2, 5);
   if (!a.batchnorm) {
     if (r == 0 && a.dbias && live) a.dbias[col] = s1;
+    if constexpr (SEAM) {
+      if (on) handoff_store(a.dpre + (long)r * a.Hp + col, dy);
+      handoff_publish(sm->seam, col);
+    } else
     if (on) a.dpre[(long)r * a.Hp + col] = dy;
     return;
   }
   if (r == 0) { a.dgamma[col] = live ? s2 : 0.f; a.dbeta[col] = live ? s1 : 0.f; }
+  if constexpr (SEAM) {
+    if (on) {
+      const float invB = 1.f / (float)a.B;
+      float d;
+      if (a.training) d = (gamma * inv) * __builtin_fmaf(-__builtin_fmaf(xh, s2, s1), invB, dy);
+      else d = dy * gamma * inv;
+      handoff_store(a.dpre + (long)r * a.Hp + col, d);
+    }
+    handoff_publish(sm->seam, col);
+    return;
+  }
   if (!on) return;
   const float invB = 1.f / (float)a.B;
   float d;
@@ -1040,11 +1068,11 @@
 }
 __global__ __launch_bounds__(BN_THREADS) void bn_wide_bwd_kernel(BnBwdArgs a) {
   __shared__ __attribute__((aligned(16))) float lds[BN_WIDE_BWD_SMEM_FLOATS];
-  bn_wide_bwd_body<false>(a, lds);
+  bn_wide_bwd_body<false>(a, lds, (int)blockIdx.x);
 }
 __global__ __launch_bounds__(BN_THREADS) void bn_wide_bwd_gen_kernel(BnBwdArgs a) {
   __shared__ __attribute__((aligned(16))) float lds[BN_WIDE_BWD_SMEM_FLOATS];
-  bn_wide_bwd_body<true>(a, lds);
+  bn_wide_bwd_body<true>(a, lds, (int)blockIdx.x);
 }
 
 template <int NP>
@@ -1057,7 +1085,7 @@
     head_dw_body<NP, 0, 1>(h, (int)blockIdx.x - first_dw, lds);
     return;
   }
-  bn_wide_bwd_body<false>(a, lds);
+  bn_wide_bwd_body<false>(a, lds, (int)blockIdx.x);
 }
 
 bool bn_wide_bwd_dw_supported(const BnBwdArgs& a, const HeadBwdArgs& h) {
@@ -1079,6 +1107,66 @@
   const dim3 grid((unsigned)(a.Hp + (a.with_metrics ? 1 : 0) + a.adam_count + a.sqr_count + (a.close ? 1 : 0) + h.n_w));
   if (h.n_planes == 3) hipLaunchKernelGGL(bn_wide_bwd_dw_kernel<3>, grid, dim3(BN_THREADS), 0, st, a, h);
   else hipLaunchKernelGGL(bn_wide_bwd_dw_kernel<2>, grid, dim3(BN_THREADS), 0, st, a, h);
+  SMX_HIP(hipGetLastError());
+  return SMX_OK;
+}
+
+template <int NP>
+__global__ __launch_bounds__(BN_THREADS) void bn_bwd_seam_kernel(BnBwdArgs dec, BnBwdArgs enc, HeadBwdArgs h, BwdSeamArgs sm) {
+  extern __shared__ __attribute__((aligned(16))) float ds[];
+  const int b = (int)blockIdx.x, np = dec.Hp, nc = enc.Hp / BN_COLS;
+  const int first_dw = (int)gridDim.x - h.n_w;
+  if (b >= first_dw) {
+    preload(h.D, h.ldd, h.dP, h.ldp, h.dW, h.ldw, h.db, h.B, h.Gp, h.sq_part, h.n_w, h.n_ht, h.n_gt, h.diag, h.Hp, h.n_planes);
+    head_dw_body<NP, 0, 1>(h, b - first_dw, ds);
+    return;
+  }
+  if (b < np + nc) {
+    const bool cons = sm.cons_first ? b < nc : b >= np;
+    if (cons) bn_act_bwd_body<2, 1, false, true>(enc, sm.cons_first ? b : b - np, &sm);
+    else bn_wide_bwd_body<false, true>(dec, ds, sm.cons_first ? b - nc : b, &sm);
+    return;
+  }
+  int e = b - np - nc;
+  if (enc.with_metrics) {
+    if (e == 0) { if (threadIdx.x < 256) metrics_body(enc.metrics); return; }
+    --e;
+  }
+  if (e < dec.adam_count) { adam_chunk_body<BN_THREADS>(dec.adam, dec.adam_first + e); return; }
+  if (enc.close && threadIdx.x < 256) step_close_body<false>(enc.adam);
+}
+
+bool bn_bwd_seam_supported(const BnBwdArgs& dec, const BnBwdArgs& enc, const HeadBwdArgs& h) {
+  return bn_wide_bwd_dw_supported(dec, h) && !dec.with_metrics && !dec.close && dec.sqr_count == 0 && dec.dpre &&
+         enc.front && enc.fold_dz && enc.act == SMX_ACT_RELU && enc.B == dec.B && enc.B <= BN_RL * 2 && enc.Hp % BN_COLS == 0 &&
+         enc.Hp / BN_COLS <= HANDOFF_MAX_WAITERS && enc.adam_count == 0 && enc.sqr_count == 0 && enc.zD == dec.dpre && enc.zld == dec.Hp && dec.Hp == 128 &&
+         bn_bwd_front_supported(enc.B, enc.fK) && bn_bwd_fold_supported(enc.B, enc.fK, enc.zlb.Dp);
+}
+int launch_bn_bwd_seam(hipStream_t st, const BnBwdArgs& dec, const BnBwdArgs& enc_in, const HeadBwdArgs& h_in, const BwdSeamArgs& sm) {
+  HeadBwdArgs h = h_in;
+  BnBwdArgs enc = enc_in;
+  enc.diag = 0;
+  const EpiLatentBwd& e = enc.zlb;
+  if (!bn_bwd_seam_supported(dec, enc, h) || !dec.dout || dec.slab_stride < (long)dec.Hp * 128 || (dec.slab_stride % 4) || !h.D || !h.dP || !h.dW || !h.db || h.ldd < h.Hp ||
+      h.ldp < (long)h.n_planes * h.Gp || h.ldw < (long)h.n_planes * h.Gp || !enc.fD || !enc.fW || (enc.fld % 4) || (enc.fldw % 4) || !enc.zW || (enc.zld % 4) || (enc.zldw % 4) ||
+      enc.zldw < 128 || !e.lat || !e.sig || !e.eps || !e.dlat || !e.stochastic || e.dklz || e.dz_add || (e.ld % 4) || e.ld < 2 * e.Dp ||
+      !sm.seam.counter || !sm.seam.error || sm.seam.target == 0 || sm.seam.shards < 1 || sm.seam.shards > HANDOFF_MAX_SHARDS || (sm.seam.shards & (sm.seam.shards - 1))) {
+    set_error("bn_bwd_seam: bad shapes");
+    return SMX_ERR_INVALID;
+  }
+  h.n_ht = h.Hp / 32; h.n_gt = h.Gp / 32; h.n_ct = (h.B + 31) / 32;
+  h.n_w = h.n_ht * ((h.n_gt + 7) / 8 * 8);
+  h.skip_dd = 1; h.skip_dw = 0; h.diag = 0;
+  if (h.sq_count) *h.sq_count = h.n_ht * h.n_gt * 8;
+  size_t lds = ((size_t)enc.B * (enc.fK + 4) + (size_t)BN_COLS * (enc.fK + 4)) * sizeof(float) + SMX_FOLD_WIMG_BYTES;
+  lds = std::max(lds, (size_t)SMX_HEAD_DW_SMEM_FLOATS * sizeof(float));
+  static_assert(SMX_HEAD_DW_SMEM_FLOATS >= BN_WIDE_BWD_SMEM_FLOATS, "bn_bwd_seam: the column body's view fits the head's");
+  static const bool ok3 = hipFuncSetAttribute(reinterpret_cast<const void*>(&bn_bwd_seam_kernel<3>), hipFuncAttributeMaxDynamicSharedMemorySize, 96 * 1024) == hipSuccess;
+  static const bool ok2 = hipFuncSetAttribute(reinterpret_cast<const void*>(&bn_bwd_seam_kernel<2>), hipFuncAttributeMaxDynamicSharedMemorySize, 96 * 1024) == hipSuccess;
+  if (!ok3 || !ok2 || lds > 96 * 1024) { set_error("bn_bwd_seam: cannot reserve the dynamic LDS"); return SMX_ERR_HIP; }
+  const dim3 grid((unsigned)(dec.Hp + enc.Hp / BN_COLS + (enc.with_metrics ? 1 : 0) + dec.adam_count + (enc.close ? 1 : 0) + h.n_w));
+  if (h.n_planes == 3) hipLaunchKernelGGL(bn_bwd_seam_kernel<3>, grid, dim3(BN_THREADS), lds, st, dec, enc, h, sm);
+  else hipLaunchKernelGGL(bn_bwd_seam_kernel<2>, grid, dim3(BN_THREADS), lds, st, dec, enc, h, sm);
   SMX_HIP(hipGetLastError());
   return SMX_OK;
 }
diff --git a/sisua_amd/csrc/smx_handoff.h b/sisua_amd/csrc/smx_handoff.h
--- /dev/null
+++ b/sisua_amd/csrc/smx_handoff.h
@@ -0,0 +1,73 @@
+#pragma once
+#include <hip/hip_runtime.h>
+
+namespace smx {
+
+constexpr int HANDOFF_MAX_WAITERS = 16;
+constexpr int HANDOFF_SHARD_STRIDE = 32;
+constexpr int HANDOFF_MAX_SHARDS = 8;
+constexpr size_t HANDOFF_STATE_BYTES = (size_t)HANDOFF_MAX_SHARDS * HANDOFF_SHARD_STRIDE * 4 + 16;
+
+struct HandoffSeam {
+  unsigned* counter = nullptr;
+  unsigned* error = nullptr;
+  unsigned target = 0;
+  int shards = 1;
+  long long timeout_ticks = 0;
+};
+
+typedef float handoff_f4 __attribute__((ext_vector_type(4)));
+typedef unsigned handoff_u4 __attribute__((ext_vector_type(4)));
+
+__device__ inline __amdgpu_buffer_rsrc_t handoff_rsrc(const void* p, long bytes) {
+  return __builtin_amdgcn_make_buffer_rsrc(const_cast<void*>(p), 0, (int)(bytes > 0x7FFFFFFFL ? 0x7FFFFFFFL : bytes), 0x00020000);
+}
+__device__ inline void handoff_store(float* p, float v) { __hip_atomic_store(p, v, __ATOMIC_RELAXED, __HIP_MEMORY_SCOPE_AGENT); }
+__device__ inline void handoff_store4(__amdgpu_buffer_rsrc_t rs, unsigned byte_off, handoff_f4 v) {
+  __builtin_amdgcn_raw_buffer_store_b128(__builtin_bit_cast(handoff_u4, v), rs, (int)byte_off, 0, 16);
+}
+__device__ inline float handoff_load(const float* p) { return __hip_atomic_load(p, __ATOMIC_RELAXED, __HIP_MEMORY_SCOPE_AGENT); }
+__device__ inline handoff_f4 handoff_load4(__amdgpu_buffer_rsrc_t rs, unsigned byte_off) {
+  return __builtin_bit_cast(handoff_f4, __builtin_amdgcn_raw_buffer_load_b128(rs, (int)byte_off, 0, 16));
+}
+
+__device__ inline void handoff_publish(const HandoffSeam& s, int producer) {
+  asm volatile("s_waitcnt vmcnt(0)" ::: "memory");
+  __syncthreads();
+  if (threadIdx.x == 0) __hip_atomic_fetch_add(s.counter + (producer & (s.shards - 1)) * HANDOFF_SHARD_STRIDE, 1u, __ATOMIC_RELAXED, __HIP_MEMORY_SCOPE_AGENT);
+}
+
+template <bool ACQUIRE>
+__device__ inline bool handoff_wait(const HandoffSeam& s, int* ok_lds) {
+  if (threadIdx.x < 64) {
+    int ok = 1;
+    const int l = (int)threadIdx.x;
+    const long long t0 = wall_clock64();
+    for (;;) {
+      unsigned got = l < s.shards ? __hip_atomic_load(s.counter + l * HANDOFF_SHARD_STRIDE, __ATOMIC_RELAXED, __HIP_MEMORY_SCOPE_AGENT) : 0u;
+#pragma unroll
+      for (int o = 1; o < HANDOFF_MAX_SHARDS; o <<= 1) got += __shfl_xor(got, o, 64);
+      got = __builtin_amdgcn_readfirstlane(got);
+      if ((int)(got - s.target) >= 0) break;
+      __builtin_amdgcn_s_sleep(2);
+      if (wall_clock64() - t0 > s.timeout_ticks) {
+        if (l == 0) __hip_atomic_store(s.error, 1u, __ATOMIC_RELAXED, __HIP_MEMORY_SCOPE_AGENT);
+        ok = 0;
+        break;
+      }
+    }
+    if (ACQUIRE && ok) {
+      __builtin_amdgcn_fence(__ATOMIC_ACQUIRE, "agent");
+      asm volatile("s_waitcnt vmcnt(0)" ::: "memory");
+    } else {
+      __builtin_amdgcn_fence(__ATOMIC_ACQUIRE, "wavefront");
+    }
+    if (l == 0) *ok_lds = ok;
+  }
+  __syncthreads();
+  const bool ok = *ok_lds != 0;
+  __builtin_amdgcn_fence(__ATOMIC_ACQUIRE, "wavefront");
+  return ok;
+}
+
+}
diff --git a/sisua_amd/csrc/smx_internal.h b/sisua_amd/csrc/smx_internal.h
--- a/sisua_amd/csrc/smx_internal.h
+++ b/sisua_amd/csrc/smx_internal.h
@@ -6,6 +6,7 @@
 
 #include "smx_device.h"
 #include "smx_act.h"
+#include "smx_handoff.h"
 #include "../../include/sisua_hip.h"
 
 namespace smx {
@@ -493,6 +494,13 @@
 bool bn_wide_bwd_dw_supported(const BnBwdArgs& a, const HeadBwdArgs& h);
 int launch_bn_wide_bwd_dw(hipStream_t st, const BnBwdArgs& a, const HeadBwdArgs& h);
 #define SMX_ADAM_SPLIT_LATE_DEFAULT 1.0f
+struct BwdSeamArgs {
+  HandoffSeam seam;
+  int preread = 0;
+  int cons_first = 0;
+};
+bool bn_bwd_seam_supported(const BnBwdArgs& dec, const BnBwdArgs& enc, const HeadBwdArgs& h);
+int launch_bn_bwd_seam(hipStream_t st, const BnBwdArgs& dec, const BnBwdArgs& enc, const HeadBwdArgs& h, const BwdSeamArgs& sm);
 
 struct BigKArgs {
   const float* A = nullptr; long lda = 0;
diff --git a/sisua_amd/csrc/smx_model.h b/sisua_amd/csrc/smx_model.h
--- a/sisua_amd/csrc/smx_model.h
+++ b/sisua_amd/csrc/smx_model.h
@@ -262,6 +262,11 @@
   bool bucket1_in_flight = false;
   bool fold_dz_now = false;
   bool dw_late_now = false;
+  bool seam_pending = false;
+  BnBwdArgs seam_dec; HeadBwdArgs seam_head;
+  unsigned* seam_state = nullptr;
+  unsigned seam_epochs = 0;
+  int32_t seam_steps = 0;
   bool chain_started = false;
   int audit_rows = 0, audit_disc_rows = 0; AuditStacked audit_stk;
   std::map<int, hipGraphExec_t> graphs;
@@ -469,6 +474,7 @@
 int csr_stage(smx_model* m, Pass& ps);
 int check_rows(smx_model* m, const int32_t* ids, size_t n);
 int read_metrics(smx_model* m, smx_metrics* out);
+int seam_error_check(smx_model* m);
 struct CsrRows { const int64_t* indptr; const int32_t* cols; const float* vals; };
 int check_csr_rows(const CsrRows& c, size_t n, int G);
 int csr_host_rows(smx_model* m, const CsrRows& c, size_t r0, size_t n, void* out, float* lgx1, int u16 = 0);
diff --git a/sisua_amd/csrc/smx_model.hip b/sisua_amd/csrc/smx_model.hip
--- a/sisua_amd/csrc/smx_model.hip
+++ b/sisua_amd/csrc/smx_model.hip
@@ -551,6 +551,7 @@
   if (m->pinned) hipHostFree(m->pinned);
   if (m->order_pin) hipHostFree(m->order_pin);
   if (m->metrics_pin) hipHostFree(m->metrics_pin);
+  if (m->seam_state) hipFree(m->seam_state);
   if (m->score_pin) hipHostFree(m->score_pin);
   if (m->ev_order) hipEventDestroy(m->ev_order);
   if (m->pred_stage) hipFree(m->pred_stage);
@@ -872,5 +873,6 @@
 
 int32_t smx_head_dw_late(const smx_model* m) { return (m && m->dw_late_now) ? 1 : 0; }
 int32_t smx_lazy_adam_steps(const smx_model* m) { return m ? m->lazy_steps : 0; }
-
-}
+int32_t smx_bwd_seam_steps(const smx_model* m) { return m ? m->seam_steps : 0; }
+
+}
diff --git a/sisua_amd/csrc/smx_step.hip b/sisua_amd/csrc/smx_step.hip
--- a/sisua_amd/csrc/smx_step.hip
+++ b/sisua_amd/csrc/smx_step.hip
@@ -180,18 +180,34 @@
   return SMX_OK;
 }
 
+static unsigned* seam_error_word(smx_model* m) { return m->seam_state + HANDOFF_MAX_SHARDS * HANDOFF_SHARD_STRIDE; }
+int seam_error_check(smx_model* m) {
+  if (!m->seam_state) return SMX_OK;
+  unsigned e = 0;
+  SMX_HIP(hipStreamSynchronize(m->st));
+  SMX_HIP(hipMemcpy(&e, seam_error_word(m), sizeof(e), hipMemcpyDeviceToHost));
+  if (!e) return SMX_OK;
+  SMX_HIP(hipMemset(seam_error_word(m), 0, sizeof(e)));
+  set_error("BatchNorm-backward seam: the encoder's workgroups gave up waiting for the decoder's d pre-activation inside the fused launch (knob no_bwd_seam runs the two launches)");
+  return SMX_ERR_HIP;
+}
+
 int read_metrics(smx_model* m, smx_metrics* out) {
   if (!out) return SMX_OK;
   const size_t nt = m->tensors.size();
-  if (!m->metrics_pin) SMX_HIP(hipHostMalloc((void**)&m->metrics_pin, (8 + nt + 1) * sizeof(float), hipHostMallocDefault));
+  if (!m->metrics_pin) SMX_HIP(hipHostMalloc((void**)&m->metrics_pin, (8 + nt + 2) * sizeof(float), hipHostMallocDefault));
   float* h = m->metrics_pin;
   float* norms_p = m->metrics_pin + 8;
   unsigned* p2p_err = reinterpret_cast<unsigned*>(m->metrics_pin + 8 + nt);
   *p2p_err = 0u;
+  unsigned* seam_err = p2p_err + 1;
+  *seam_err = 0u;
   SMX_HIP(hipMemcpyAsync(h, m->grads + m->tail_off_metrics, 8 * sizeof(float), hipMemcpyDeviceToHost, m->st));
   SMX_HIP(hipMemcpyAsync(norms_p, m->tensor_norm, nt * sizeof(float), hipMemcpyDeviceToHost, m->st));
   if (m->p2p && m->p2p->error) SMX_HIP(hipMemcpyAsync(p2p_err, m->p2p->error, sizeof(unsigned), hipMemcpyDeviceToHost, m->st));
+  if (m->seam_state) SMX_HIP(hipMemcpyAsync(seam_err, seam_error_word(m), sizeof(unsigned), hipMemcpyDeviceToHost, m->st));
   SMX_HIP(hipStreamSynchronize(m->st));
+  if (*seam_err) SMX_CHECK(seam_error_check(m));
   if (*p2p_err) {
     set_error(*p2p_err == 1u ? "peer-to-peer all-reduce: a wait on a peer's flag timed out (SMX_P2P_TIMEOUT_S)" :
                                "peer-to-peer all-reduce: a peer reported a timed-out wait");
@@ -438,6 +454,7 @@
   ++m->params_epoch;
   smx::DrawCaps caps(m);
   m->lazy_steps = 0;
+  m->seam_steps = 0; m->seam_epochs = 0;
   for (int s = 0; s < n_steps && rc == SMX_OK; ++s) rc = launch_train(m, batch * m->train_draws, use_graph != 0, s, n_steps);
   { const int rf = smx::lazy_flush(m); if (rc == SMX_OK) rc = rf; }
   { const int rj = smx::head_sweep_join(m); if (rc == SMX_OK) rc = rj; }
@@ -461,6 +478,7 @@
 int smx_metrics_history(smx_model* m, int32_t n_steps, float* host) {
   SMX_REQUIRE(m && host && n_steps > 0 && n_steps <= m->mhist_steps, "no such history (steps of the last smx_train_steps call)");
   SMX_HIP(hipStreamSynchronize(m->st));
+  SMX_CHECK(smx::seam_error_check(m));
   SMX_HIP(hipMemcpy(host, m->mhist, (size_t)n_steps * 8 * sizeof(float), hipMemcpyDeviceToHost));
   return SMX_OK;
 }
diff --git a/sisua_amd/engine.py b/sisua_amd/engine.py
--- a/sisua_amd/engine.py
+++ b/sisua_amd/engine.py
@@ -704,6 +704,9 @@
   def head_dw_late(self) -> bool:
     return bool(self.lib.smx_head_dw_late(self._h))
 
+  def bwd_seam_steps(self) -> int:
+    return int(self.lib.smx_bwd_seam_steps(self._h))
+
   def lazy_adam_steps(self) -> int:
     return int(self.lib.smx_lazy_adam_steps(self._h))
 
```

New measurement: 2.201 million, median of 6. 1.03x the previous value.
